# ttanida/rgrg

Measured on AMD Instinct MI355X. Metric: images/sec full 29-region report gen, 512x512 CXR, greedy max_len=128, higher is better.
Workload: dtype bf16; 1 GPU; full_model.generate() batch=32/GPU, 29 regions, greedy max_len=128, bf16 autocast: 16-bit detector, 16-bit decode GEMMs + K/V cache, hipGraph-captured decode step (BASELINE configs[2]); global_batch=32, parallelism=single GPU, weights=seeded random init (rgrg_amd.synth, profile bench), hipGraph_decode=True

## Files before the change

include/rgrg_hip.h:

```cpp
#ifndef RGRG_HIP_H_
#define RGRG_HIP_H_

#include <stdint.h>

#ifdef __cplusplus
extern "C" {
#endif

#define RGRG_OK 0
#define RGRG_EINVAL (-1)
#define RGRG_EHIP (-2)
#define RGRG_ESTATE (-3)

#define RGRG_ACT_NONE 0
#define RGRG_ACT_RELU 1
#define RGRG_ACT_GELU_NEW 2

const char* rgrg_last_error(void);
int rgrg_abi_version(void);
int rgrg_device_arch(int dev, char* buf, int buflen);

int rgrg_linear_f32(const float* A, const float* W, const float* scale, const float* shift, const float* R,
                    float* Y, int M, int N, int K, int ldy, int act, int splitk, float* ws, void* stream);
int rgrg_conv2d_nhwc_f32(const float* X, const float* W, const float* scale, const float* shift, const float* R,
                         float* Y, int B, int H, int Wd, int Cin, int Cout, int KH, int KW, int stride, int pad,
                         int act, int splitk, float* ws, void* stream);

int rgrg_stem_conv7x7_f32(const float* X, const float* Wt, const float* scale, const float* shift, float* Y,
                          int B, int H, int Wd, void* stream);
int rgrg_maxpool3x3s2_nhwc_f32(const float* X, float* Y, int B, int H, int Wd, int C, void* stream);

int rgrg_rpn_proposals_f32(const float* head_out, const float* anchors, float* proposals, int32_t* counts,
                           int32_t* offsets, int B, int HW, int A, int pre_nms, int post_nms, float nms_thresh,
                           float min_size, float img_w, float img_h, void* stream);

int rgrg_roi_align_avgpool_f32(const float* feat, const float* proposals, const int32_t* offsets, float* out,
                               float* pooled, int B, int FH, int FW, int C, int max_props, int R_total,
                               float spatial_scale, void* stream);
int rgrg_roi_align_avgpool_bf16maps(const float* feat, const float* proposals, const int32_t* offsets, uint16_t* out16,
                                    float* pooled, int B, int FH, int FW, int C, int max_props, int R_total,
                                    float spatial_scale, int fp16, void* stream);

int rgrg_top1_per_class_f32(const float* pred, int ldp, const float* proposals, const int32_t* offsets,
                            const float* pooled, uint8_t* class_detected, float* top_scores, float* top_boxes,
                            float* top_feats, int B, int C, int max_props, float img_w, float img_h, void* stream);

int rgrg_bce_with_logits_masked_f32(const float* logits, const uint8_t* mask, const uint8_t* target, float pos_weight,
                                    int n, float* loss, void* stream);
int rgrg_preprocess_u8_f32(const uint8_t* src, int h, int w, int src_stride, int new_h, int new_w, float mean, float std,
                           float* dst, void* stream);
int rgrg_select_regions_f32(const float* logits, const uint8_t* class_detected, float thr, uint8_t* selected,
                            int32_t* sel_rows, int32_t* n_selected, int n, void* stream);
int rgrg_gather_rows_f32(const float* src, const int32_t* rows, float* dst, int n_rows, int D, void* stream);

typedef struct rgrg_decoder_layer_weights {
    const float *ln1_g, *ln1_b, *ln2_g, *ln2_b;
    const float *c_attn_w, *c_attn_b;
    const float *attn_proj_w, *attn_proj_b;
    const float *c_fc_w, *c_fc_b;
    const float *mlp_proj_w, *mlp_proj_b;
} rgrg_decoder_layer_weights;

typedef struct rgrg_decoder_weights {
    int n_layer, d_model, n_head, vocab;
    const float* wte;
    const float *lnf_g, *lnf_b;
    const float *fst0_w, *fst0_b, *fst2_w, *fst2_b;
    const float *ukv_w, *ukv_b;
    const rgrg_decoder_layer_weights* layers;
} rgrg_decoder_weights;

typedef struct rgrg_decoder rgrg_decoder;

int rgrg_decoder_create(const rgrg_decoder_weights* w, int max_seqs, int max_len, rgrg_decoder** out);
int rgrg_decoder_create_with_cache(const rgrg_decoder_weights* w, int max_seqs, int max_len, void* kv_cache, size_t kv_cache_bytes,
                                   rgrg_decoder** out);
size_t rgrg_decoder_kv_cache_bytes(int n_layer, int max_seqs, int max_len);
void rgrg_decoder_destroy(rgrg_decoder* d);
int rgrg_decoder_generate(rgrg_decoder* d, const float* feats, int S, int max_length, int64_t* out_ids,
                          int out_ld, int* out_len, int use_graph, void* stream);
int rgrg_decoder_sample(rgrg_decoder* d, const float* feats, int S, int max_length, float temperature, int top_k, float top_p,
                        uint64_t seed, int64_t* out_ids, int out_ld, float* out_logprobs, int* out_len, int use_graph,
                        void* stream);
int rgrg_sample_logits_f32(const float* logits, int64_t ld, int S, int V, float temperature, int top_k, float top_p,
                           uint64_t seed, int step, int row0, int* out_tok, float* out_logprob, void* stream);
int rgrg_decoder_beam_search(rgrg_decoder* d, const float* feats, int S, int num_beams, int max_length,
                             int early_stopping, float length_penalty, int num_return_sequences, int64_t* out_ids,
                             int out_ld, int* out_len, void* stream);
int rgrg_decoder_set_precision(rgrg_decoder* d, int mode);
int rgrg_decoder_set_kv_format(rgrg_decoder* d, int fmt);
int rgrg_decoder_kv_format_in_use(rgrg_decoder* d, int rows);
int rgrg_decoder_set_lm_positions(rgrg_decoder* d, const int64_t* pos, int64_t n);
int rgrg_decoder_lm_forward(rgrg_decoder* d, const float* feats, const int64_t* input_ids, const float* attention_mask,
                            int S, int T, float* logits_out, float* loss_out, void* stream);
int rgrg_decoder_lm_loss_grad(rgrg_decoder* d, const float* feats, const int64_t* input_ids, const float* attention_mask,
                              int S, int T, float loss_scale, float dropout_p, uint64_t dropout_seed, float* loss_out,
                              float* grad_ukv_w, float* grad_ukv_b, float* grad_fst0_w, float* grad_fst0_b, float* grad_fst2_w,
                              float* grad_fst2_b, void* stream);
int rgrg_decoder_time_train_gemms(rgrg_decoder* d, int S, int T, int iters, float* ms_per_step, double* flops_per_step,
                                  int* launches_per_step);
int rgrg_dropout_mask_f32(uint64_t seed, uint32_t stream_id, float p, int64_t n, int row_len, float* out, void* stream);
int rgrg_decoder_forward_cached(rgrg_decoder* d, const float* feats, const int64_t* input_ids, const int64_t* position_ids,
                                const float* attention_mask,
                                int S, int T, int past_len, float* logits_out, void* stream);
int rgrg_decoder_cache_plane(rgrg_decoder* d, int layer, int kv, void** ptr, int* max_seqs, int* slots, int* is_bf16);
int rgrg_decoder_take_id_error(rgrg_decoder* d, int* pending);
int rgrg_decoder_refresh_trainable(rgrg_decoder* d, void* stream);
int rgrg_transpose_pad_f32(const float* src, float* dst, int rows, int cols, int rows_padded, void* stream);
int rgrg_colsum_f32(const float* src, float* out, int rows, int cols, void* stream);
int rgrg_relu_backward_f32(float* d, const float* h, int64_t n, void* stream);
int rgrg_bce_with_logits_masked_backward_f32(const float* logits, const uint8_t* mask, const uint8_t* target, float pos_weight,
                                             int n, float scale, float* dlogits, int ld, void* stream);
int rgrg_adamw_step_f32(float* param, const float* grad, float* exp_avg, float* exp_avg_sq, int64_t n, float lr, float beta1,
                        float beta2, float eps, float weight_decay, int step, float grad_scale, void* stream);
int rgrg_adamw_multi_step_f32(const void* items, int n_items, float lr, float beta1, float beta2, float eps,
                              float weight_decay, int step, float grad_scale, void* stream);
int rgrg_f32_to_bf16(const float* src, uint16_t* dst, int64_t n, int fp16, void* stream);
int rgrg_bf16_to_f32(const uint16_t* src, float* dst, int64_t n, int fp16, void* stream);
int rgrg_conv2d_nhwc_bf16(const uint16_t* X16, const uint16_t* Wb, const float* shift, const uint16_t* R16, float* Y,
                          uint16_t* Y16, int B, int H, int Wd, int Cin, int Cout, int KH, int KW, int stride, int pad,
                          int act, int fp16, void* stream);
int rgrg_linear_bf16w_f32(const float* A, const uint16_t* Wb, const float* shift, const float* R, float* Y, int M,
                          int N, int K, int ldy, int act, int fp16, void* stream);
int rgrg_linear_bf16_f32(const uint16_t* A16, const uint16_t* Wb, const float* shift, const float* R, float* Y,
                         uint16_t* Y16, int M, int N, int K, int ldy, int act, int fp16, void* stream);
int rgrg_debug_linear_bf16_tile(const uint16_t* A16, const uint16_t* Wb, const float* shift, const float* R, float* Y,
                                int M, int N, int K, int ldy, int act, int tile, int lda, int ldw, int fp16, void* stream);
int rgrg_debug_linear_bf16_train(const uint16_t* A16, const uint16_t* Wb, const float* shift, const float* R, float* Y,
                                 uint16_t* Y16, uint16_t* Ypre16, const uint16_t* G16, int M, int N, int K, int ldy, int act,
                                 int tile, int fp16, void* stream);
int rgrg_debug_linear_bf16_argmax(const uint16_t* A16, const uint16_t* Wb, const float* shift, int M, int N, int K,
                                  float* cand_val, int* cand_idx, int fp16, void* stream);
int rgrg_debug_ln_fold16(const float* w, const float* gain, const float* beta, const float* bias, uint16_t* wb, float* colsum,
                         float* shift, int N, int K, int fp16, void* stream);
int rgrg_debug_linear_bf16_ln(const uint16_t* A16, const uint16_t* Wb, const float* shift, const float* R, float* Y,
                              uint16_t* Yb16, float* stats_out, const float* ln_stats, const float* ln_colsum, int M, int N,
                              int K, int ldy, int act, int fp16, void* stream);
int rgrg_debug_linear_bf16_ln_kv(const uint16_t* A16, const uint16_t* Wb, const float* shift, float* Y, const float* ln_stats,
                                 const float* ln_colsum, uint16_t* kcache, uint16_t* vcache, const int* step_dev, int M, int H,
                                 int T_slots, int K, int ldy, int fp16, void* stream);
int rgrg_debug_linear_bf16_ln_kp(const uint16_t* A16, const uint16_t* Wb, const float* shift, const float* R, float* Y,
                                 uint16_t* Y16, uint16_t* Yb16, float* stats_out, const float* ln_stats, const float* ln_colsum,
                                 int M, int N, int K, int ldy, int act, int fp16, int kp, void* stream);
int rgrg_debug_attn_decode(const float* qkv, int ld_qkv, void* kcache, void* vcache, const int* step_dev, float* out,
                           uint16_t* out16, int S, int H, int T_slots, const int* src, const float* kmask, int kv16, int fp16,
                           int ni, int frag_out, int max_workgroups, void* stream);
int rgrg_debug_attn_decode_qonly(const float* q, int ld_q, const void* kcache, const void* vcache, const int* step_dev, float* out,
                                 uint16_t* out16, int S, int H, int T_slots, int fp16, int max_workgroups, void* stream);
int rgrg_debug_attn_decode_kv8(const float* qkv, int ld_qkv, uint8_t* kcache, uint8_t* vcache, const int* step_dev, float* out,
                               uint16_t* out16, int S, int H, int T_slots, const int* src, const float* kmask, int fp16,
                               int max_workgroups, void* stream);
int rgrg_debug_attn_prefill(const float* qkv, const float* ukv, int ld_ukv, int kcol, const float* am, float* out, uint16_t* out16,
                            float* lse, int S, int H, int T, int variant, uint64_t seed, uint32_t stream_id, float p, int fp16,
                            void* stream);
int rgrg_debug_attn_backward_f32(const float* qkv, const float* ukv, int ld_ukv, int kcol, const float* am, const float* d_att,
                                 const float* att, const float* lse, float* delta, float* d_qkv, float* d_ukv, uint16_t* d_qkv16,
                                 int S, int H, int T, uint64_t seed, uint32_t stream_id, float p, int fp16, float ukv_scale,
                                 void* stream);
int rgrg_debug_attn_train16(int backward, const uint16_t* qkv16, const uint16_t* ukv16, int ld_ukv, int kcol, const float* am,
                            uint16_t* att16, float* lse, const uint16_t* d_att16, uint16_t* d_qkv16, float* d_ukv, int S, int H,
                            int T, uint64_t seed, uint32_t stream_id, float p, float ukv_scale, int fp16, void* stream);
int rgrg_box_match_f32(const float* gt, const int* gt_count, int G, const float* boxes, int64_t box_image_stride,
                       const int* box_count, int B, int N, float high, float low, int allow_low_quality, int* matched,
                       int* ws_best_per_gt, void* stream);
int rgrg_balanced_sample(const int* matched, const int64_t* gt_labels, int G, const int* box_count, const float* keys,
                         uint64_t seed, int stage, int B, int n, int batch, int max_pos, uint32_t* ws_keys, uint8_t* mask,
                         int* list, int* count, void* stream);
int rgrg_rpn_loss_sampled_f32(const float* rpn_out, int ld, int anchors_per_cell, const int* matched, const float* gt, int G,
                              const float* anchors, const uint8_t* mask, const int* list, const int* count, int B, int A,
                              int batch, float* out2, void* stream);
int rgrg_roi_add_gt_f32(const float* props, const int* counts, int P, const float* gt, const int* gt_count, int G, int B,
                        float* boxes, int* box_count, void* stream);
int rgrg_roi_gather_samples_f32(const float* boxes, const int* matched, const float* gt, const int64_t* gt_labels,
                                const int* gt_count, int G, const int* list, const int* count, int B, int N, int K, float wx,
                                float wy, float ww, float wh, float* props_s, int* offsets, int64_t* labels_flat,
                                float* reg_targets, void* stream);
int rgrg_fastrcnn_loss_f32(const float* pred, int ld, int num_classes, const int64_t* labels, const float* reg_targets, int N,
                           float* out2, void* stream);

int rgrg_decoder_copy_last_logits(rgrg_decoder* d, float* dst, int S, void* stream);
int rgrg_decoder_time_step_parts(rgrg_decoder* d, int S, int nkeys, int iters, int one_range, float* ms_gemm, float* ms_attn,
                                 double* gemm_flops, double* gemm_weight_bytes, double* kv_bytes, int* gemm_launches);
int rgrg_decoder_trace_step(rgrg_decoder* d, int S, int nkeys, int iters, float* recs, int max_recs, int* n_out);
int rgrg_decoder_attention_only(rgrg_decoder* d, int S, int nkeys, int iters, void* stream);
int rgrg_decoder_row_limit(rgrg_decoder* d);
int rgrg_debug_chain(int n, int mode, int blocks, float* us_per_kernel);

#ifdef __cplusplus
}
#endif
#endif
```

rgrg_amd/_hip.py:

```python
from __future__ import annotations

import ctypes as C
import os
from typing import Optional

from . import build as _build

c_float_p = C.c_void_p
_i, _f, _p = C.c_int, C.c_float, C.c_void_p

ACT_NONE, ACT_RELU, ACT_GELU_NEW = 0, 1, 2
ABI_VERSION = 25


class RgrgHipError(RuntimeError):
    pass


class DecoderLayerWeights(C.Structure):
    _fields_ = [(n, _p) for n in ("ln1_g", "ln1_b", "ln2_g", "ln2_b", "c_attn_w", "c_attn_b", "attn_proj_w",
                                  "attn_proj_b", "c_fc_w", "c_fc_b", "mlp_proj_w", "mlp_proj_b")]


class DecoderWeights(C.Structure):
    _fields_ = [("n_layer", _i), ("d_model", _i), ("n_head", _i), ("vocab", _i), ("wte", _p), ("lnf_g", _p),
                ("lnf_b", _p), ("fst0_w", _p), ("fst0_b", _p), ("fst2_w", _p), ("fst2_b", _p), ("ukv_w", _p),
                ("ukv_b", _p), ("layers", C.POINTER(DecoderLayerWeights))]


SIGNATURES = {
    "rgrg_last_error": (C.c_char_p, []),
    "rgrg_abi_version": (_i, []),
    "rgrg_device_arch": (_i, [_i, C.c_char_p, _i]),
    "rgrg_linear_f32": (_i, [_p, _p, _p, _p, _p, _p, _i, _i, _i, _i, _i, _i, _p, _p]),
    "rgrg_conv2d_nhwc_f32": (_i, [_p, _p, _p, _p, _p, _p, _i, _i, _i, _i, _i, _i, _i, _i, _i, _i, _i, _p, _p]),
    "rgrg_stem_conv7x7_f32": (_i, [_p, _p, _p, _p, _p, _i, _i, _i, _p]),
    "rgrg_maxpool3x3s2_nhwc_f32": (_i, [_p, _p, _i, _i, _i, _i, _p]),
    "rgrg_rpn_proposals_f32": (_i, [_p, _p, _p, _p, _p, _i, _i, _i, _i, _i, _f, _f, _f, _f, _p]),
    "rgrg_roi_align_avgpool_f32": (_i, [_p, _p, _p, _p, _p, _i, _i, _i, _i, _i, _i, _f, _p]),
    "rgrg_roi_align_avgpool_bf16maps": (_i, [_p, _p, _p, _p, _p, _i, _i, _i, _i, _i, _i, _f, _i, _p]),
    "rgrg_top1_per_class_f32": (_i, [_p, _i, _p, _p, _p, _p, _p, _p, _p, _i, _i, _i, _f, _f, _p]),
    "rgrg_select_regions_f32": (_i, [_p, _p, _f, _p, _p, _p, _i, _p]),
    "rgrg_bce_with_logits_masked_f32": (_i, [_p, _p, _p, C.c_float, _i, _p, _p]),
    "rgrg_preprocess_u8_f32": (_i, [_p, _i, _i, _i, _i, _i, C.c_float, C.c_float, _p, _p]),
    "rgrg_gather_rows_f32": (_i, [_p, _p, _p, _i, _i, _p]),
    "rgrg_decoder_create": (_i, [C.POINTER(DecoderWeights), _i, _i, C.POINTER(_p)]),
    "rgrg_decoder_create_with_cache": (_i, [C.POINTER(DecoderWeights), _i, _i, _p, C.c_size_t, C.POINTER(_p)]),
    "rgrg_decoder_kv_cache_bytes": (C.c_size_t, [_i, _i, _i]),
    "rgrg_decoder_destroy": (None, [_p]),
    "rgrg_decoder_generate": (_i, [_p, _p, _i, _i, _p, _i, C.POINTER(_i), _i, _p]),
    "rgrg_decoder_sample": (_i, [_p, _p, _i, _i, _f, _i, _f, C.c_uint64, _p, _i, _p, C.POINTER(_i), _i, _p]),
    "rgrg_sample_logits_f32": (_i, [_p, C.c_int64, _i, _i, _f, _i, _f, C.c_uint64, _i, _i, _p, _p, _p]),
    "rgrg_decoder_beam_search": (_i, [_p, _p, _i, _i, _i, _i, _f, _i, _p, _i, C.POINTER(_i), _p]),
    "rgrg_decoder_set_precision": (_i, [_p, _i]),
    "rgrg_decoder_set_kv_format": (_i, [_p, _i]),
    "rgrg_decoder_kv_format_in_use": (_i, [_p, _i]),
    "rgrg_decoder_lm_forward": (_i, [_p, _p, _p, _p, _i, _i, _p, _p, _p]),
    "rgrg_decoder_lm_loss_grad": (_i, [_p, _p, _p, _p, _i, _i, C.c_float, C.c_float, C.c_uint64, _p, _p, _p, _p, _p, _p, _p, _p]),
    "rgrg_dropout_mask_f32": (_i, [C.c_uint64, C.c_uint32, C.c_float, C.c_int64, _i, _p, _p]),
    "rgrg_decoder_refresh_trainable": (_i, [_p, _p]),
    "rgrg_decoder_take_id_error": (_i, [_p, C.POINTER(_i)]),
    "rgrg_decoder_forward_cached": (_i, [_p, _p, _p, _p, _p, _i, _i, _i, _p, _p]),
    "rgrg_decoder_cache_plane": (_i, [_p, _i, _i, C.POINTER(C.c_void_p), C.POINTER(_i), C.POINTER(_i), C.POINTER(_i)]),
    "rgrg_transpose_pad_f32": (_i, [_p, _p, _i, _i, _i, _p]),
    "rgrg_colsum_f32": (_i, [_p, _p, _i, _i, _p]),
    "rgrg_relu_backward_f32": (_i, [_p, _p, C.c_int64, _p]),
    "rgrg_bce_with_logits_masked_backward_f32": (_i, [_p, _p, _p, C.c_float, _i, C.c_float, _p, _i, _p]),
    "rgrg_adamw_step_f32": (_i, [_p, _p, _p, _p, C.c_int64, C.c_float, C.c_float, C.c_float, C.c_float, C.c_float, _i, C.c_float, _p]),
    "rgrg_adamw_multi_step_f32": (_i, [_p, _i, C.c_float, C.c_float, C.c_float, C.c_float, C.c_float, _i, C.c_float, _p]),
    "rgrg_f32_to_bf16": (_i, [_p, _p, C.c_int64, _i, _p]),
    "rgrg_bf16_to_f32": (_i, [_p, _p, C.c_int64, _i, _p]),
    "rgrg_conv2d_nhwc_bf16": (_i, [_p, _p, _p, _p, _p, _p, _i, _i, _i, _i, _i, _i, _i, _i, _i, _i, _i, _p]),
    "rgrg_linear_bf16w_f32": (_i, [_p, _p, _p, _p, _p, _i, _i, _i, _i, _i, _i, _p]),
    "rgrg_linear_bf16_f32": (_i, [_p, _p, _p, _p, _p, _p, _i, _i, _i, _i, _i, _i, _p]),
    "rgrg_debug_linear_bf16_tile": (_i, [_p, _p, _p, _p, _p, _i, _i, _i, _i, _i, _i, _i, _i, _i, _p]),
    "rgrg_debug_linear_bf16_train": (_i, [_p, _p, _p, _p, _p, _p, _p, _p, _i, _i, _i, _i, _i, _i, _i, _p]),
    "rgrg_debug_linear_bf16_argmax": (_i, [_p, _p, _p, _i, _i, _i, _p, _p, _i, _p]),
    "rgrg_debug_ln_fold16": (_i, [_p, _p, _p, _p, _p, _p, _p, _i, _i, _i, _p]),
    "rgrg_debug_linear_bf16_ln": (_i, [_p, _p, _p, _p, _p, _p, _p, _p, _p, _i, _i, _i, _i, _i, _i, _p]),
    "rgrg_debug_linear_bf16_ln_kp": (_i, [_p, _p, _p, _p, _p, _p, _p, _p, _p, _p, _i, _i, _i, _i, _i, _i, _i, _p]),
    "rgrg_debug_attn_decode": (_i, [_p, _i, _p, _p, _p, _p, _p, _i, _i, _i, _p, _p, _i, _i, _i, _i, _i, _p]),
    "rgrg_debug_linear_bf16_ln_kv": (_i, [_p, _p, _p, _p, _p, _p, _p, _p, _p, _i, _i, _i, _i, _i, _i, _p]),
    "rgrg_debug_attn_decode_qonly": (_i, [_p, _i, _p, _p, _p, _p, _p, _i, _i, _i, _i, _i, _p]),
    "rgrg_debug_attn_decode_kv8": (_i, [_p, _i, _p, _p, _p, _p, _p, _i, _i, _i, _p, _p, _i, _i, _p]),
    "rgrg_debug_attn_prefill": (_i, [_p, _p, _i, _i, _p, _p, _p, _p, _i, _i, _i, _i, C.c_uint64, C.c_uint32, _f, _i, _p]),
    "rgrg_debug_attn_backward_f32": (_i, [_p, _p, _i, _i, _p, _p, _p, _p, _p, _p, _p, _p, _i, _i, _i, C.c_uint64, C.c_uint32, _f,
                                          _i, _f, _p]),
    "rgrg_debug_attn_train16": (_i, [_i, _p, _p, _i, _i, _p, _p, _p, _p, _p, _p, _i, _i, _i, C.c_uint64, C.c_uint32, _f, _f, _i, _p]),
    "rgrg_decoder_copy_last_logits": (_i, [_p, _p, _i, _p]),
    "rgrg_box_match_f32": (_i, [_p, _p, _i, _p, C.c_int64, _p, _i, _i, _f, _f, _i, _p, _p, _p]),
    "rgrg_balanced_sample": (_i, [_p, _p, _i, _p, _p, C.c_uint64, _i, _i, _i, _i, _i, _p, _p, _p, _p, _p]),
    "rgrg_rpn_loss_sampled_f32": (_i, [_p, _i, _i, _p, _p, _i, _p, _p, _p, _p, _i, _i, _i, _p, _p]),
    "rgrg_roi_add_gt_f32": (_i, [_p, _p, _i, _p, _p, _i, _i, _p, _p, _p]),
    "rgrg_roi_gather_samples_f32": (_i, [_p, _p, _p, _p, _p, _i, _p, _p, _i, _i, _i, _f, _f, _f, _f, _p, _p, _p, _p, _p]),
    "rgrg_fastrcnn_loss_f32": (_i, [_p, _i, _i, _p, _p, _i, _p, _p]),
    "rgrg_decoder_trace_step": (_i, [_p, _i, _i, _i, _p, _i, C.POINTER(_i)]),
    "rgrg_decoder_attention_only": (_i, [_p, _i, _i, _i, _p]),
    "rgrg_decoder_row_limit": (_i, [_p]),
    "rgrg_decoder_set_lm_positions": (_i, [_p, _p, C.c_int64]),
    "rgrg_decoder_time_step_parts": (_i, [_p, _i, _i, _i, _i, C.POINTER(_f), C.POINTER(_f), C.POINTER(C.c_double),
                                          C.POINTER(C.c_double), C.POINTER(C.c_double), C.POINTER(_i)]),
    "rgrg_decoder_time_train_gemms": (_i, [_p, _i, _i, _i, C.POINTER(_f), C.POINTER(C.c_double), C.POINTER(_i)]),
    "rgrg_debug_chain": (_i, [_i, _i, _i, C.POINTER(_f)]),
}

_lib: Optional[C.CDLL] = None


def library_path() -> str:
    return _build.LIB_PATH


def load() -> C.CDLL:
    global _lib
    if _lib is not None:
        return _lib
    path = library_path()
    if _build.is_stale():
        try:
            _build.build_library()
        except Exception as e:
            if not os.path.exists(path):
                raise RgrgHipError(f"librgrg_hip.so is missing and could not be built: {e}") from e
    try:
        lib = C.CDLL(path)
    except OSError as e:
        raise RgrgHipError(f"cannot load {path}: {e} (the RGRG HIP path has no CPU fallback)") from e
    for name, (res, args) in SIGNATURES.items():
        fn = getattr(lib, name)
        fn.restype = res
        fn.argtypes = args
    got = lib.rgrg_abi_version()
    if got != ABI_VERSION:
        raise RgrgHipError(f"{path} has ABI version {got}, this package expects {ABI_VERSION}: rebuild it "
                           "(python -m rgrg_amd.build)")
    _lib = lib
    return lib


def autocast_mode() -> int:
    import torch
    if not torch.is_autocast_enabled("cuda"):
        return 0
    dt = torch.get_autocast_dtype("cuda")
    return 1 if dt == torch.bfloat16 else (2 if dt == torch.float16 else 0)


def check(rc: int, what: str = "") -> None:
    if rc != 0:
        msg = load().rgrg_last_error()
        raise RgrgHipError(f"{what} failed (code {rc}): {msg.decode() if msg else '?'}")


def ptr(t) -> Optional[int]:
    if t is None:
        return None
    assert t.is_contiguous(), "rgrg_hip expects dense tensors"
    return t.data_ptr()
```

rgrg_amd/csrc/decoder.hip:

```cpp
#include <math.h>
#include <stdlib.h>

#include <algorithm>
#include <type_traits>
#include <cmath>
#include <vector>

#include "decoder_internal.h"

namespace rgrg {

int skinny_max_rows() {
    static int v = -1;
    if (v < 0) { const char* e = getenv("RGRG_SKINNY_MAX_ROWS"); v = e ? atoi(e) : SKINNY_MAX_ROWS;
        if (v > SKINNY_MAX_ROWS) v = SKINNY_MAX_ROWS; if (v < 32) v = 32; }
    return v;
}

__global__ __launch_bounds__(256) void pack_weights_kernel(const float* __restrict__ W, float* __restrict__ P, int N,
                                                           int K, int NT) {
    const size_t total = (size_t)NT * (K / 8) * 64;
    for (size_t o = (size_t)blockIdx.x * blockDim.x + threadIdx.x; o < total; o += (size_t)gridDim.x * blockDim.x) {
        const int l = (int)(o & 63);
        const size_t t = o >> 6;
// ... 77 lines not shown
#pragma unroll
            for (int j = 0; j < 4; ++j) c16 = __builtin_amdgcn_mfma_f32_32x32x2f32(x[j], w[c][j], c16, 0, 0, 0);
        }
#pragma unroll
        for (int r = 0; r < 16; ++r) acc[mt][r] = c16[r];
    }
    float* red = smem;
#pragma unroll
    for (int mt = 0; mt < MT; ++mt) {
        __syncthreads();
#pragma unroll
        for (int r = 0; r < 16; ++r) red[(wave * 16 + r) * 64 + lane] = acc[mt][r];
        __syncthreads();
        const int row0 = mt * 32;
#pragma unroll
        for (int q = 0; q < 2; ++q) {
            const int idx = tid + 512 * q;
            const int r = idx >> 6, l = idx & 63;
            float v = red[r * 64 + l];
#pragma unroll
            for (int w2 = 1; w2 < SK_WAVES; ++w2) v += red[(w2 * 16 + r) * 64 + l];
            const int lrow = (r & 3) + 8 * (r >> 2) + 4 * (l >> 5);
            const int col = nt * 32 + (l & 31);
            if (a.KS == 1) skinny_store(a, row0 + lrow, col, v);
            else a.part[(((size_t)mt * a.KS + ks) * PAD_ROWS + lrow) * (a.NT * 32) + col] = v;
        }
    }
}

__global__ __launch_bounds__(512) void rgrg_skinny_gemm_f32_wide(const SkinnyArgs a) {
    extern __shared__ __attribute__((aligned(16))) float smem[];
    constexpr int PW = 16, KC = 8, KWG = PW * SK_WAVES * KC, LDX = KWG + 4, XQ = KWG / 64;
    float* red = smem + a.M * LDX;
    const int tid = threadIdx.x, lane = tid & 63, wave = tid >> 6;
    const int chunks = a.K / KC;
    {
        f32x4 xr[XQ];
#pragma unroll
        for (int q = 0; q < XQ; ++q) {
            const int idx = tid + 512 * q;
            const int row = idx / (KWG / 4), c4 = idx - row * (KWG / 4);
            xr[q] = *reinterpret_cast<const f32x4*>(a.X + (size_t)row * a.K + c4 * 4);
        }
#pragma unroll
        for (int q = 0; q < XQ; ++q) {
            const int idx = tid + 512 * q;
            const int row = idx / (KWG / 4), c4 = idx - row * (KWG / 4);
            if (row < a.M) *reinterpret_cast<f32x4*>(&smem[row * LDX + c4 * 4]) = xr[q];
        }
    }
    __syncthreads();
    const float* xa = &smem[(lane & 31) * LDX + wave * PW * KC + (lane >> 5) * 4];
    const f32x4* wbase = reinterpret_cast<const f32x4*>(a.P) + ((size_t)wave * PW) * 64 + lane;
    f32x4 wa[8], wb[8];
    auto load8 = [&](f32x4(&w)[8], int nt, int half) {
        const f32x4* wp = wbase + ((size_t)nt * chunks + half * 8) * 64;
#pragma unroll
        for (int c = 0; c < 8; ++c) w[c] = __builtin_nontemporal_load(wp + (size_t)c * 64);
    };
    int nt = blockIdx.x;
    if (nt < a.NT) { load8(wa, nt, 0); load8(wb, nt, 1); }
    for (; nt < a.NT; nt += gridDim.x) {
        const int nxt = nt + gridDim.x;
        f32x16 acc;
#pragma unroll
        for (int r = 0; r < 16; ++r) acc[r] = 0.f;
#pragma unroll
        for (int c = 0; c < 8; ++c) {
            const f32x4 x = *reinterpret_cast<const f32x4*>(xa + c * KC);
#pragma unroll
            for (int j = 0; j < 4; ++j) acc = __builtin_amdgcn_mfma_f32_32x32x2f32(x[j], wa[c][j], acc, 0, 0, 0);
        }
        if (nxt < a.NT) load8(wa, nxt, 0);
#pragma unroll
        for (int c = 0; c < 8; ++c) {
            const f32x4 x = *reinterpret_cast<const f32x4*>(xa + (8 + c) * KC);
#pragma unroll
            for (int j = 0; j < 4; ++j) acc = __builtin_amdgcn_mfma_f32_32x32x2f32(x[j], wb[c][j], acc, 0, 0, 0);
        }
        if (nxt < a.NT) load8(wb, nxt, 1);
        __syncthreads();
#pragma unroll
        for (int r = 0; r < 16; ++r) red[(wave * 16 + r) * 64 + lane] = acc[r];
        __syncthreads();
#pragma unroll
        for (int q = 0; q < 2; ++q) {
            const int idx = tid + 512 * q;
            const int r = idx >> 6, l = idx & 63;
            float v = red[r * 64 + l];
#pragma unroll
            for (int w2 = 1; w2 < SK_WAVES; ++w2) v += red[(w2 * 16 + r) * 64 + l];
            const int row = (r & 3) + 8 * (r >> 2) + 4 * (l >> 5);
            const int col = nt * 32 + (l & 31);
            skinny_store(a, row, col, v);
        }
    }
}


#include "skinny_direct.inc"

constexpr int WIDE_MAX_ROWS = 31;
constexpr size_t WIDE_LDS = (size_t)(WIDE_MAX_ROWS * (16 * SK_WAVES * 8 + 4) + SK_WAVES * 16 * 64) * sizeof(float);
static_assert(WIDE_LDS <= 160 * 1024, "wide skinny GEMM must fit the 160 KiB LDS");

template <int PW, int MT>
static int launch_skinny(const SkinnyArgs& a, hipStream_t st) {
    constexpr size_t lds_x = (size_t)32 * (PW * SK_WAVES * 8 + 4) * sizeof(float);
    constexpr size_t lds_r = (size_t)SK_WAVES * 16 * 64 * sizeof(float);
    constexpr size_t lds = lds_x > lds_r ? lds_x : lds_r;
    hipLaunchKernelGGL((rgrg_skinny_gemm_f32<PW, MT>), dim3(a.NT, a.KS), dim3(64 * SK_WAVES), lds, st, a);
    RGRG_LAUNCH_CHECK();
    return RGRG_OK;
}

template <int PW>
static int launch_skinny_mt(const SkinnyArgs& a, hipStream_t st) {
    const int mt = (a.M + PAD_ROWS - 1) / PAD_ROWS;
    if (mt <= 1) return launch_skinny<PW, 1>(a, st);
    if (mt == 2) return launch_skinny<PW, 2>(a, st);
    if (mt == 3) return launch_skinny<PW, 3>(a, st);
    if (mt == 4) return launch_skinny<PW, 4>(a, st);
    set_error("skinny GEMM: %d rows exceed 4 row tiles", a.M);
    return RGRG_EINVAL;
}

static int launch_skinny_any(const SkinnyArgs& a, hipStream_t st) {
    const int pw = a.K / (8 * a.KS * SK_WAVES);
    if (pw == 16 && a.KS == 1 && a.NT > 512 && a.M <= WIDE_MAX_ROWS) {
        hipLaunchKernelGGL(rgrg_skinny_gemm_f32_wide, dim3(256), dim3(64 * SK_WAVES), WIDE_LDS, st, a);
        RGRG_LAUNCH_CHECK();
        return RGRG_OK;
    }
    if (pw == 4) return launch_skinny_mt<4>(a, st);
    if (pw == 8) return launch_skinny_mt<8>(a, st);
    if (pw == 16) return launch_skinny_mt<16>(a, st);
    set_error("skinny GEMM: unsupported shape K=%d KS=%d (chunks per wave %d)", a.K, a.KS, pw);
    return RGRG_EINVAL;
}

__global__ __launch_bounds__(256) void skinny_reduce_kernel(const SkinnyArgs a) {
    const int ldp = a.NT * 32;
    const int total = a.M * a.N;
    for (int i = blockIdx.x * blockDim.x + threadIdx.x; i < total; i += gridDim.x * blockDim.x) {
        const int row = i / a.N, col = i - row * a.N;
        float v = 0.f;
        const float* pt = a.part + ((size_t)(row >> 5) * a.KS * PAD_ROWS + (row & 31)) * ldp + col;
        for (int ks = 0; ks < a.KS; ++ks) v += pt[(size_t)ks * PAD_ROWS * ldp];
        skinny_store(a, row, col, v);
    }
}


__global__ __launch_bounds__(256) void embed_ln_kernel(const float* __restrict__ wte, const long long* __restrict__ ids,
                                                       int ld_ids, const int* __restrict__ step, const float* __restrict__ g,
                                                       const float* __restrict__ b, float* __restrict__ x,
                                                       float* __restrict__ xn, int D, const int* __restrict__ tok_override,
                                                       unsigned short* __restrict__ xn16, int f16, const int* __restrict__ pos_override,
                                                       float* __restrict__ stats) {
    __shared__ float sh[4];
    const int s = blockIdx.x, tid = threadIdx.x;
    const int t = pos_override ? pos_override[s] : *step;
    const long long tok = tok_override ? (long long)tok_override[s] : ids[(size_t)s * ld_ids + *step];
    const f32x4 v = reinterpret_cast<const f32x4*>(wte + (size_t)tok * D)[tid] + reinterpret_cast<const f32x4*>(wte + (size_t)t * D)[tid];
    reinterpret_cast<f32x4*>(x + (size_t)s * D)[tid] = v;
    if (stats) {
        store_16x4(xn16 + (size_t)s * D + 4 * tid, v, f16);
        const float s1 = block_sum_256((v[0] + v[1]) + (v[2] + v[3]), sh);
        const float s2 = block_sum_256((v[0] * v[0] + v[1] * v[1]) + (v[2] * v[2] + v[3] * v[3]), sh);
        if (tid < 16) reinterpret_cast<float2*>(stats)[(size_t)s * 16 + tid] = tid ? make_float2(0.f, 0.f) : make_float2(s1, s2);
        return;
    }
    const f32x4 o = ln_row(v, g, b, sh, D);
    if (xn16) store_16x4(xn16 + (size_t)s * D + 4 * tid, o, f16);
    else reinterpret_cast<f32x4*>(xn + (size_t)s * D)[tid] = o;
}

__global__ __launch_bounds__(256) void ln_rows_kernel(const float* __restrict__ x, const float* __restrict__ g,
                                                      const float* __restrict__ b, float* __restrict__ xn, int D,
                                                      unsigned short* __restrict__ xn16, int f16, int rows) {
    const int lane = threadIdx.x & 63, row = blockIdx.x * 4 + (threadIdx.x >> 6);
    if (row >= rows) return;
    const f32x4* xr = reinterpret_cast<const f32x4*>(x + (size_t)row * D);
    f32x4 v[4], gg[4], bb[4];
#pragma unroll
    for (int j = 0; j < 4; ++j) v[j] = xr[j * 64 + lane];
#pragma unroll
    for (int j = 0; j < 4; ++j) {
        gg[j] = reinterpret_cast<const f32x4*>(g)[j * 64 + lane];
        bb[j] = reinterpret_cast<const f32x4*>(b)[j * 64 + lane];
    }
    __builtin_amdgcn_sched_barrier(0);
    float s = 0.f;
#pragma unroll
    for (int j = 0; j < 4; ++j) s += (v[j][0] + v[j][1]) + (v[j][2] + v[j][3]);
    const float mean = wave_sum_dpp(s) / (float)D;
    float q = 0.f;
#pragma unroll
    for (int j = 0; j < 4; ++j) {
#pragma unroll
        for (int e = 0; e < 4; ++e) { v[j][e] -= mean; q += v[j][e] * v[j][e]; }
    }
    const float rstd = 1.0f / sqrtf(wave_sum_dpp(q) / (float)D + LN_EPS);
#pragma unroll
    for (int j = 0; j < 4; ++j) {
        f32x4 o;
#pragma unroll
        for (int e = 0; e < 4; ++e) o[e] = v[j][e] * rstd * gg[j][e] + bb[j][e];
        if (xn16) store_16x4(xn16 + (size_t)row * D + 4 * (j * 64 + lane), o, f16);
        else reinterpret_cast<f32x4*>(xn + (size_t)row * D)[j * 64 + lane] = o;
    }
}
int launch_ln_rows(const float* x, const float* g, const float* b, float* xn, int D, unsigned short* xn16, int f16, int rows,
                   hipStream_t st) {
    hipLaunchKernelGGL(ln_rows_kernel, dim3((rows + 3) / 4), dim3(256), 0, st, x, g, b, xn, D, xn16, f16, rows);
    RGRG_LAUNCH_CHECK();
    return RGRG_OK;
}


__device__ __forceinline__ float group16_sum_dpp(float v) {
    v += dpp_get<0xB1, 0xf>(v);
    v += dpp_get<0x4E, 0xf>(v);
    v += dpp_get<0x141, 0xf>(v);
    v += dpp_get<0x140, 0xf>(v);
    return v;
}

template <bool HAS_SRC, int NI, bool HAS_MASK = false>
__device__ __forceinline__ void attn_chunk(const float* __restrict__ kc, const float* __restrict__ vc, const int* __restrict__ srow, int s,
                                           int hd, int H, int T, int base, int nkeys, int slot, int wave, int g, int d4,
                                           const f32x4& q4, const f32x4& k4, const f32x4& v4, float& m, float& l, f32x4& acc,
                                           const float* __restrict__ kmask = nullptr) {
    int rowi[NI];
#pragma unroll
    for (int i = 0; i < NI; ++i) rowi[i] = HAS_SRC ? srow[min(base + (i * 4 + wave) * 4 + g, nkeys - 1)] : s;
    f32x4 kk[NI], vv[NI];
    float mk[NI];
#pragma unroll
    for (int i = 0; i < NI; ++i) {
        const int jc = min(base + (i * 4 + wave) * 4 + g, nkeys - 1);
        const size_t off = (((size_t)rowi[i] * H + hd) * T + jc) * 64 + d4 * 4;
        kk[i] = *reinterpret_cast<const f32x4*>(kc + off);
        vv[i] = *reinterpret_cast<const f32x4*>(vc + off);
        mk[i] = HAS_MASK ? kmask[(size_t)s * T + jc] : 0.f;
    }
    __builtin_amdgcn_sched_barrier(0);
    {
#pragma clang fp contract(off)
    float sc[NI];
#pragma unroll
    for (int i = 0; i < NI; ++i) {
        const int j = base + (i * 4 + wave) * 4 + g;
        if (j == slot) { kk[i] = k4; vv[i] = v4; }
        const float dot = group16_sum_dpp(fmaf(q4[0], kk[i][0], q4[1] * kk[i][1]) + fmaf(q4[2], kk[i][2], q4[3] * kk[i][3]));
        sc[i] = HAS_MASK ? dot / 8.0f + mk[i] : dot / 8.0f;
    }
    float ex[NI];
    bool up[NI];
    float mp = m;
#pragma unroll
    for (int i = 0; i < NI; ++i) {
        const bool valid = base + (i * 4 + wave) * 4 + g < nkeys;
        up[i] = valid && sc[i] > mp;
        ex[i] = valid ? expf(-fabsf(sc[i] - mp)) : 0.f;
        mp = up[i] ? sc[i] : mp;
    }
#pragma unroll
    for (int i = 0; i < NI; ++i) {
        const bool valid = base + (i * 4 + wave) * 4 + g < nkeys;
        const float scale = up[i] ? ex[i] : 1.f;
        const float p = up[i] ? 1.f : ex[i];
        l = fmaf(l, scale, p);
#pragma unroll
        for (int e = 0; e < 4; ++e) acc[e] = fmaf(p, valid ? vv[i][e] : 0.f, acc[e] * scale);
    }
    m = mp;
    }
}

template <bool HAS_SRC, int ATT_NI, bool HAS_MASK = false>
__global__ __launch_bounds__(256) void attn_decode_kernel(const float* __restrict__ qkv, int ld_qkv,
                                                          float* __restrict__ kc, float* __restrict__ vc,
                                                          const int* __restrict__ step, float* __restrict__ out,
                                                          int S, int H, int T, const int* __restrict__ src, int frag_out,
                                                          const float* __restrict__ kmask = nullptr) {
    __shared__ float pm[16], pl[16];
    __shared__ __attribute__((aligned(16))) float pacc[16][64];
    const int lane = threadIdx.x & 63, wave = threadIdx.x >> 6;
    const int s = blockIdx.x / H, hd = blockIdx.x - s * H;
    const int t = *step, nkeys = t + 2, slot = t + 1;
    const int g = lane >> 4, d4 = lane & 15;
    const float* row = qkv + (size_t)s * ld_qkv;
    const int D = H * 64;
    const int* srow = HAS_SRC ? src + (size_t)s * T : nullptr;
    constexpr int ATT_CHUNK = 16 * ATT_NI;
    const f32x4 q4 = *reinterpret_cast<const f32x4*>(row + hd * 64 + d4 * 4);
    const f32x4 k4 = *reinterpret_cast<const f32x4*>(row + D + hd * 64 + d4 * 4);
    const f32x4 v4 = *reinterpret_cast<const f32x4*>(row + 2 * D + hd * 64 + d4 * 4);
    float m = -INFINITY, l = 0.f;
    f32x4 acc = {0.f, 0.f, 0.f, 0.f};
#define ATT_CHUNK_CALL(NI_, BASE_) attn_chunk<HAS_SRC, NI_, HAS_MASK>(kc, vc, srow, s, hd, H, T, BASE_, nkeys, slot, wave, g, d4, q4, k4, v4, m, l, acc, kmask)
    if constexpr (ATT_NI == 9) {
        int base = 0;
        for (; nkeys - base > ATT_CHUNK; base += ATT_CHUNK) ATT_CHUNK_CALL(9, base);
        switch ((nkeys - base + 15) >> 4) {
            case 1: ATT_CHUNK_CALL(1, base); break;
            case 2: ATT_CHUNK_CALL(2, base); break;
            case 3: ATT_CHUNK_CALL(3, base); break;
            case 4: ATT_CHUNK_CALL(4, base); break;
            case 5: ATT_CHUNK_CALL(5, base); break;
            case 6: ATT_CHUNK_CALL(6, base); break;
            case 7: ATT_CHUNK_CALL(7, base); break;
            case 8: ATT_CHUNK_CALL(8, base); break;
            default: ATT_CHUNK_CALL(9, base); break;
        }
    } else {
        for (int base = 0; base < nkeys; base += ATT_CHUNK) ATT_CHUNK_CALL(ATT_NI, base);
    }
#undef ATT_CHUNK_CALL
    if (wave == 0 && g == 0) {
        *reinterpret_cast<f32x4*>(kc + (((size_t)s * H + hd) * T + slot) * 64 + d4 * 4) = k4;
        *reinterpret_cast<f32x4*>(vc + (((size_t)s * H + hd) * T + slot) * 64 + d4 * 4) = v4;
    }
    const int grp = wave * 4 + g;
    if (d4 == 0) { pm[grp] = m; pl[grp] = l; }
    *reinterpret_cast<f32x4*>(&pacc[grp][d4 * 4]) = acc;
    __syncthreads();
// ... 67 lines not shown
            vn16 = kv16_pack_round<F16>(r.v0, r.v1);
        }
    }
    float sc[NI];
    float cmax = -INFINITY;
#pragma unroll
    for (int i = 0; i < NI; ++i) {
        const int j = base + i * 8 + g;
        if constexpr (!QONLY) {
            if (j == slot) { kk[i] = kn16; vv[i] = vn16; }
        }
        float dot = 0.f;
#pragma unroll
        for (int e = 0; e < 4; ++e)
            dot += q[2 * e] * pair_lo<F16>(kk[i][e]) + q[2 * e + 1] * pair_hi<F16>(kk[i][e]);
        dot += dpp_get<0xB1, 0xf>(dot);
        dot += dpp_get<0x4E, 0xf>(dot);
        dot += dpp_get<0x141, 0xf>(dot);
        sc[i] = j < nkeys ? dot / 8.0f : -INFINITY;
        cmax = fmaxf(cmax, sc[i]);
    }
    const float m_new = fmaxf(m, cmax);
    const float scale = (m == -INFINITY) ? 0.f : expf(m - m_new);
    const bool any = m_new != -INFINITY;
    l *= scale;
#pragma unroll
    for (int e = 0; e < 8; ++e) acc[e] *= scale;
#pragma unroll
    for (int i = 0; i < NI; ++i) {
        const int j = base + i * 8 + g;
        const float pj = (j < nkeys && any) ? expf(sc[i] - m_new) : 0.f;
        l += pj;
#pragma unroll
        for (int e = 0; e < 4; ++e) {
            const unsigned u = j < nkeys ? vv[i][e] : 0u;
            acc[2 * e] += pj * pair_lo<F16>(u);
            acc[2 * e + 1] += pj * pair_hi<F16>(u);
        }
    }
    m = m_new;
}

template <bool HAS_SRC, bool F16, bool QONLY = false>
__global__ __launch_bounds__(256) void attn_decode_kv16_wave_kernel(const float* __restrict__ qkv, int ld_qkv,
                                                                    u16* __restrict__ kc, u16* __restrict__ vc,
                                                                    const int* __restrict__ step, float* __restrict__ out,
                                                                    int S, int H, int T, const int* __restrict__ src,
                                                                    u16* __restrict__ out16) {
    const int lane = threadIdx.x & 63;
    const int t = *step, nkeys = t + 2, slot = t + 1;
    const int g = lane >> 3, d8 = lane & 7;
    const int D = H * 64;
    const __amdgpu_buffer_rsrc_t rk = dx_rsrc(kc), rv = dx_rsrc(vc);
    for (int item = blockIdx.x * 4 + (threadIdx.x >> 6); item < S * H; item += gridDim.x * 4) {
    const int s = item / H, hd = item - s * H;
    const float* row = qkv + (size_t)s * ld_qkv;
    const int* srow = HAS_SRC ? src + (size_t)s * T : nullptr;
    Kv16Row r;
    r.q0 = *reinterpret_cast<const f32x4*>(row + hd * 64 + d8 * 8);
    r.q1 = *reinterpret_cast<const f32x4*>(row + hd * 64 + d8 * 8 + 4);
    if constexpr (!QONLY) {
        r.k0 = *reinterpret_cast<const f32x4*>(row + D + hd * 64 + d8 * 8);
        r.k1 = *reinterpret_cast<const f32x4*>(row + D + hd * 64 + d8 * 8 + 4);
        r.v0 = *reinterpret_cast<const f32x4*>(row + 2 * D + hd * 64 + d8 * 8);
        r.v1 = *reinterpret_cast<const f32x4*>(row + 2 * D + hd * 64 + d8 * 8 + 4);
    }
    float m = -INFINITY, l = 0.f, acc[8], q[8];
    u32x4 kn16, vn16;
#pragma unroll
    for (int e = 0; e < 8; ++e) acc[e] = 0.f;
#define KV16_CHUNK(NI_, FIRST_, BASE_) \
    kv16_wave_chunk<NI_, HAS_SRC, FIRST_, F16, QONLY>(rk, rv, srow, s, hd, H, T, BASE_, nkeys, slot, g, d8, r, q, kn16, vn16, m, l, acc)
#define KV16_TAIL(FIRST_, BASE_, REM_)                                                                   \
    switch (((REM_) + 7) >> 3) {                                                                         \
        case 1: KV16_CHUNK(1, FIRST_, BASE_); break;                                                     \
        case 2: KV16_CHUNK(2, FIRST_, BASE_); break;                                                     \
        case 3: KV16_CHUNK(3, FIRST_, BASE_); break;                                                     \
        case 4: KV16_CHUNK(4, FIRST_, BASE_); break;                                                     \
        case 5: KV16_CHUNK(5, FIRST_, BASE_); break;                                                     \
        case 6: KV16_CHUNK(6, FIRST_, BASE_); break;                                                     \
        case 7: KV16_CHUNK(7, FIRST_, BASE_); break;                                                     \
        case 8: KV16_CHUNK(8, FIRST_, BASE_); break;                                                     \
        default: KV16_CHUNK(9, FIRST_, BASE_); break;                                                    \
    }
    if (nkeys > 72) {
        KV16_CHUNK(9, true, 0);
        int base = 72;
        for (; nkeys - base > 72; base += 72) KV16_CHUNK(9, false, base);
        KV16_TAIL(false, base, nkeys - base)
    } else {
        KV16_TAIL(true, 0, nkeys)
    }
#undef KV16_TAIL
#undef KV16_CHUNK
    if constexpr (!QONLY) {
        if (g == 0) {
            const size_t o = (((size_t)s * H + hd) * T + slot) * 64 + d8 * 8;
            *reinterpret_cast<u32x4*>(kc + o) = kn16;
            *reinterpret_cast<u32x4*>(vc + o) = vn16;
        }
    }
    float M = fmaxf(m, dpp_get<0x128, 0xf>(m));
    M = fmaxf(M, __shfl_xor(M, 16, 64));
    M = fmaxf(M, __shfl_xor(M, 32, 64));
    const float wgt = (m == -INFINITY) ? 0.f : expf(m - M);
    l *= wgt;
    l += dpp_get<0x128, 0xf>(l);
    l += __shfl_xor(l, 16, 64);
    l += __shfl_xor(l, 32, 64);
#pragma unroll
    for (int e = 0; e < 8; ++e) {
        float o = acc[e] * wgt;
        o += dpp_get<0x128, 0xf>(o);
        o += __shfl_xor(o, 16, 64);
        o += __shfl_xor(o, 32, 64);
        acc[e] = o / l;
    }
    if (g == 0) {
        const size_t o = (size_t)s * D + hd * 64 + d8 * 8;
        if (out16) {
            u32x4 pk;
#pragma unroll
            for (int i = 0; i < 4; ++i) pk[i] = to16<F16>(acc[2 * i]) | (to16<F16>(acc[2 * i + 1]) << 16);
            *reinterpret_cast<u32x4*>(out16 + o) = pk;
        } else {
            *reinterpret_cast<f32x4*>(out + o) = f32x4{acc[0], acc[1], acc[2], acc[3]};
            *reinterpret_cast<f32x4*>(out + o + 4) = f32x4{acc[4], acc[5], acc[6], acc[7]};
        }
    }
    }
}

template <typename KV>
__global__ __launch_bounds__(256) void kv_slot0_kernel(const float* __restrict__ ukv, int ld, KV* __restrict__ kv_all,
                                                       size_t layer_stride, size_t kv_stride, int S, int H, int T,
                                                       int L, int row_mul, int f16) {
    const int D = H * 64;
    const size_t total = (size_t)L * 2 * S * D;
    for (size_t i = (size_t)blockIdx.x * blockDim.x + threadIdx.x; i < total; i += (size_t)gridDim.x * blockDim.x) {
        const int d = (int)(i % D);
        size_t r = i / D;
        const int s = (int)(r % S);
        r /= S;
        const int kv = (int)(r & 1), l = (int)(r >> 1);
        const int hd = d >> 6, e = d & 63;
        const float val = ukv[(size_t)s * ld + ((size_t)l * 2 + kv) * D + d];
        const size_t o = (size_t)l * layer_stride + (size_t)kv * kv_stride + (((size_t)s * row_mul * H + hd) * T) * 64 + e;
        if constexpr (sizeof(KV) == 1) kv_all[o] = (KV)f32_to_e4m3_bits(val);
        else if constexpr (sizeof(KV) == 2) kv_all[o] = (KV)to16_rt(val, f16);
        else kv_all[o] = val;
    }
}

constexpr int ARGMAX_U = 13;
__global__ __launch_bounds__(256) void argmax_update_kernel(const float* __restrict__ cand_val, const int* __restrict__ cand_idx,
                                                            int NT, long long* __restrict__ ids, int ld_ids,
                                                            int* __restrict__ finished, int* __restrict__ step,
                                                            int* __restrict__ done_len, int* __restrict__ sync, int S) {
    __shared__ float bv[4];
    __shared__ int bi[4];
    const int row = blockIdx.x, tid = threadIdx.x, lane = tid & 63, wave = tid >> 6;
    const int t = *step;
    const float* cv = cand_val + (size_t)row * NT;
    const int* cx = cand_idx + (size_t)row * NT;
    float v[ARGMAX_U];
    int ci[ARGMAX_U];
#pragma unroll
    for (int u = 0; u < ARGMAX_U; ++u) {
        const int i = min(tid + 256 * u, NT - 1);
        v[u] = cv[i];
        ci[u] = cx[i];
    }
    float best = -INFINITY;
    int idx = 0x7fffffff;
#pragma unroll
    for (int u = 0; u < ARGMAX_U; ++u)
        if (tid + 256 * u < NT && (v[u] > best || (v[u] == best && ci[u] < idx))) { best = v[u]; idx = ci[u]; }
    for (int i = tid + 256 * ARGMAX_U; i < NT; i += 256) {
        const float w = cv[i];
        const int wi = cx[i];
        if (w > best || (w == best && wi < idx)) { best = w; idx = wi; }
    }
    for (int o = 32; o > 0; o >>= 1) {
        const float ov = __shfl_xor(best, o, 64);
        const int oi = __shfl_xor(idx, o, 64);
        if (ov > best || (ov == best && oi < idx)) { best = ov; idx = oi; }
    }
    if (lane == 0) { bv[wave] = best; bi[wave] = idx; }
    __syncthreads();
    if (tid == 0) {
        for (int w = 1; w < 4; ++w)
            if (bv[w] > best || (bv[w] == best && bi[w] < idx)) { best = bv[w]; idx = bi[w]; }
        const StepBook bk{ids, ld_ids, finished, step, done_len, sync, S};
        record_step_token(bk, row, t, idx == 0x7fffffff ? 0 : idx);
    }
}

__global__ __launch_bounds__(256) void logits_candidates_kernel(const float* __restrict__ logits, int ld, int V, int NT,
                                                                float* __restrict__ cand_val, int* __restrict__ cand_idx) {
    const int row = blockIdx.y, lane = threadIdx.x & 63, wave = threadIdx.x >> 6;
    const float* x = logits + (size_t)row * ld;
    const int sub = lane & 7, tw = lane >> 3;
    constexpr int UN = 4;
    for (int t0 = (blockIdx.x * 4 + wave) * 8 * UN; t0 < NT; t0 += gridDim.x * 4 * 8 * UN) {
        f32x4 v[UN];
#pragma unroll
        for (int u = 0; u < UN; ++u) {
            const int nt = min(t0 + u * 8 + tw, NT - 1);
            v[u] = *reinterpret_cast<const f32x4*>(x + nt * 32 + sub * 4);
        }
#pragma unroll
        for (int u = 0; u < UN; ++u) {
            const int nt = t0 + u * 8 + tw;
            const int c0 = min(nt, NT - 1) * 32 + sub * 4;
            float bv = -INFINITY;
            int bi = c0;
#pragma unroll
            for (int e = 0; e < 4; ++e) {
                const float val = (c0 + e < V) ? v[u][e] : -INFINITY;
                if (val > bv) { bv = val; bi = c0 + e; }
            }
#define CAND_STEP(CTRL)                                                                                     \
    {                                                                                                       \
        const float ov = dpp_get<CTRL, 0xf>(bv);                                                            \
        const int oi = __builtin_amdgcn_update_dpp(0, bi, CTRL, 0xf, 0xf, false);                           \
        if (ov > bv || (ov == bv && oi < bi)) { bv = ov; bi = oi; }                                         \
    }
            CAND_STEP(0xB1) CAND_STEP(0x4E) CAND_STEP(0x141)
#undef CAND_STEP
            if (sub == 0 && nt < NT) {
                cand_val[(size_t)row * NT + nt] = bv;
                cand_idx[(size_t)row * NT + nt] = bi;
            }
        }
    }
}

__global__ __launch_bounds__(256) void decode_reset_kernel(long long* __restrict__ ids, int ld_ids, int* __restrict__ finished,
                                                           int* __restrict__ step, int* __restrict__ done_len,
                                                           int* __restrict__ sync, int S, int L) {
    const size_t total = (size_t)S * L;
    for (size_t i = (size_t)blockIdx.x * blockDim.x + threadIdx.x; i < total; i += (size_t)gridDim.x * blockDim.x)
        ids[(i / L) * ld_ids + (i % L)] = (i % L) == 0 ? BOS_ID : PAD_ID;
    if (blockIdx.x == 0) {
        for (int s = threadIdx.x; s < S; s += 256) finished[s] = 0;
        if (threadIdx.x == 0) { *step = 0; *done_len = 0; }
        if (threadIdx.x < 2) sync[threadIdx.x] = 0;
    }
}

__global__ __launch_bounds__(256) void ln_fold16_kernel(const float* __restrict__ w, const float* __restrict__ gain,
                                                        const float* __restrict__ beta, const float* __restrict__ b,
                                                        unsigned short* __restrict__ wb, float* __restrict__ cs,
                                                        float* __restrict__ c2, int N, int K, int f16) {
    const int lane = threadIdx.x & 63, n = blockIdx.x * 4 + (threadIdx.x >> 6);
    if (n >= N) return;
    float a = 0.f, c = 0.f;
    for (int k = lane; k < K; k += 64) {
        const float wv = w[(size_t)n * K + k];
        float gw = gain[k] * wv;
        asm("" : "+v"(gw));
        const unsigned short r = (unsigned short)to16_rt(gw, f16);
        wb[(size_t)n * K + k] = r;
        a += from16_rt(r, f16);
        c += beta[k] * wv;
    }
    a = wave_sum(a);
    c = wave_sum(c);
    if (lane == 0) { cs[n] = a; c2[n] = (b ? b[n] : 0.f) + c; }
}

int dmalloc(rgrg_decoder* d, void** p, size_t bytes, bool zero) {
    RGRG_HIP(hipMalloc(p, bytes));
    d->allocs.push_back(*p);
    if (zero) RGRG_HIP(hipMemset(*p, 0, bytes));
    return RGRG_OK;
}

static int pick_ks(int NT, int chunks) {
    int ks = 1;
    if (NT >= 64) return ks;
    while (NT * ks < 256 && chunks % (ks * 2 * SK_WAVES * 4) == 0) ks *= 2;
    return ks;
}

static int make_lin(rgrg_decoder* d, Lin& l, const float* w, const float* b, int N, int K, bool pack,
                    bool direct = false, const float* ln_g = nullptr, const float* ln_b = nullptr) {
    l.w = w; l.b = b; l.N = N; l.K = K;
    if (direct) {
        if (!(K == DK_SLICE || (K == 4 * DK_SLICE && !ln_g && N == DK_SLICE))) { set_error("decoder: N=%d K=%d unsupported by the fused plan", N, K); return RGRG_EINVAL; }
        l.direct = true; l.ntile = 16; l.KS = K / DK_SLICE; l.NT = (N + 15) / 16; l.lnf = ln_g != nullptr;
        int rc = dmalloc(d, (void**)&l.packed, (size_t)l.NT * 16 * K * sizeof(float), false);
        if (rc) return rc;
        hipLaunchKernelGGL(pack_weights16_scaled_kernel, dim3(2048), dim3(256), 0, d->stream, w, ln_g, l.packed, N, K, l.NT);
        RGRG_LAUNCH_CHECK();
        if (l.lnf) {
            if ((rc = dmalloc(d, (void**)&l.c1, (size_t)N * sizeof(float), false)) ||
                (rc = dmalloc(d, (void**)&l.c2, (size_t)N * sizeof(float), false)))
                return rc;
            hipLaunchKernelGGL(ln_fold_vectors_kernel, dim3((N + 3) / 4), dim3(256), 0, d->stream, w, ln_g, ln_b, b, l.c1, l.c2, N, K);
            RGRG_LAUNCH_CHECK();
        }
        return RGRG_OK;
    }
    l.ntile = 32;
    l.KS = pick_ks((N + 31) / 32, K / 8);
    l.NT = (N + l.ntile - 1) / l.ntile;
    const int kc = 8;
    const int pw = K / (kc * l.KS * SK_WAVES);
    const bool ok = (K % (kc * l.KS * SK_WAVES) == 0) && (pw == 4 || pw == 8 || pw == 16);
    if (!ok) {
        set_error("decoder: no skinny GEMM instance for N=%d K=%d (ntile %d, KS %d, %d chunks per wave)", N, K, l.ntile, l.KS, pw);
        return RGRG_EINVAL;
    }
    if (pack) {
        const size_t bytes = (size_t)l.NT * l.ntile * K * sizeof(float);
        int rc = dmalloc(d, (void**)&l.packed, bytes, false);
        if (rc) return rc;
        hipLaunchKernelGGL(pack_weights_kernel, dim3(2048), dim3(256), 0, d->stream, w, l.packed, N, K, l.NT);
        RGRG_LAUNCH_CHECK();
    }
    return RGRG_OK;
}

template <int PW, int MT>
static int skinny_attr1() {
    constexpr size_t lds_x = (size_t)32 * (PW * SK_WAVES * 8 + 4) * sizeof(float);
    RGRG_HIP(hipFuncSetAttribute(reinterpret_cast<const void*>(&rgrg_skinny_gemm_f32<PW, MT>),
                                 hipFuncAttributeMaxDynamicSharedMemorySize, (int)(lds_x > 65536 ? lds_x : 65536)));
    return RGRG_OK;
}
template <int PW>
static int skinny_attr() {
    int rc;
    if ((rc = skinny_attr1<PW, 1>())) return rc;
    if ((rc = skinny_attr1<PW, 2>())) return rc;
    if ((rc = skinny_attr1<PW, 3>())) return rc;
    return skinny_attr1<PW, 4>();
}
static int init_skinny_attrs() {
    int rc;
    RGRG_HIP(hipFuncSetAttribute(reinterpret_cast<const void*>(&rgrg_lm_head_wave_f32<DX_COMBINE4>),
                                 hipFuncAttributeMaxDynamicSharedMemorySize, (int)LMH_LDS));
    if ((rc = skinny_attr<4>())) return rc;
    if ((rc = skinny_attr<8>())) return rc;
    RGRG_HIP(hipFuncSetAttribute(reinterpret_cast<const void*>(&rgrg_skinny_gemm_f32_wide),
                                 hipFuncAttributeMaxDynamicSharedMemorySize, (int)WIDE_LDS));
    return skinny_attr<16>();
// ... 113 lines not shown
        const dim3 wgrid(a.max_wgs > 0 ? std::min(wgs, a.max_wgs) : wgs), wblk(256);
        if (a.q_only && (a.fmt == KV_E4M3 || a.src)) {
            set_error("decode attention: the q-only variant exists for the 16-bit K/V cache without an ancestor table (%s)",
                      a.src ? "beam search" : "e4m3 K/V cache");
            return RGRG_EINVAL;
        }
        if (a.fmt == KV_E4M3)
            return launch_attn_decode_kv8(a.qkv, a.ld_qkv, static_cast<uint8_t*>(a.kc), static_cast<uint8_t*>(a.vc), a.step, a.out, a.out16,
                                          a.S, a.H, a.T, a.src, a.f16, (int)wgrid.x, a.st);
#define KV16_LAUNCH(...) hipLaunchKernelGGL((attn_decode_kv16_wave_kernel<__VA_ARGS__>), wgrid, wblk, 0, a.st, a.qkv, a.ld_qkv, \
                                                  static_cast<u16*>(a.kc), static_cast<u16*>(a.vc), a.step, a.out, a.S, a.H, a.T, a.src, a.out16)
        if (a.q_only) { if (a.f16) KV16_LAUNCH(false, true, true); else KV16_LAUNCH(false, false, true); }
        else if (a.src) { if (a.f16) KV16_LAUNCH(true, true); else KV16_LAUNCH(true, false); }
        else { if (a.f16) KV16_LAUNCH(false, true); else KV16_LAUNCH(false, false); }
#undef KV16_LAUNCH
    } else {
        if (a.q_only) { set_error("decode attention: the q-only variant exists for the 16-bit K/V cache only"); return RGRG_EINVAL; }
        const dim3 grid(a.S * a.H), blk(256);
        const int ni = a.ni ? a.ni : (a.S * a.H <= 4096 ? 9 : 2);
        if (ni != 9 && ni != 2) { set_error("decode attention: %d keys per group, the kernel is built for 9 and 2", ni); return RGRG_EINVAL; }
#define ATT_LAUNCH(SRC_, NI_, MASK_) hipLaunchKernelGGL((attn_decode_kernel<SRC_, NI_, MASK_>), grid, blk, 0, a.st, a.qkv, a.ld_qkv, static_cast<float*>(a.kc), \
                                                       static_cast<float*>(a.vc), a.step, a.out, a.S, a.H, a.T, a.src, a.frag_out, a.kmask)
        if (a.kmask) {
            if (ni == 9) ATT_LAUNCH(false, 9, true); else ATT_LAUNCH(false, 2, true);
        } else if (ni == 9) { if (a.src) ATT_LAUNCH(true, 9, false); else ATT_LAUNCH(false, 9, false); }
        else { if (a.src) ATT_LAUNCH(true, 2, false); else ATT_LAUNCH(false, 2, false); }
#undef ATT_LAUNCH
    }
    RGRG_LAUNCH_CHECK();
    return RGRG_OK;
}

static int launch_attention(rgrg_decoder* d, int l, int S, const int* src, unsigned short* att16, int frag_out = 0, int r0 = 0,
                            bool q_only = false) {
    const int D = d->D;
    AttnDecodeLaunch a{};
    a.q_only = q_only;
    a.ld_qkv = 3 * D; a.step = d->step; a.S = S; a.H = d->H; a.T = d->T; a.src = src; a.kmask = d->key_mask_cur;
    a.frag_out = frag_out; a.st = d->stream; a.plane_elems = d->kv_kv_stride;
    a.fmt = kv_format(d, S);
    if (a.fmt != KV_F32) {
        static const int cap = [] { const char* e = getenv("RGRG_ATTN_WGS_PER_CU"); return e ? atoi(e) : 0; }();
        const size_t esz = a.fmt == KV_E4M3 ? 1 : sizeof(u16);
        unsigned char* kcr = reinterpret_cast<unsigned char*>(d->kv) + ((size_t)l * d->kv_layer_stride + (size_t)r0 * d->H * d->T * 64) * esz;
        a.f16 = d->f16(); a.max_wgs = cap > 0 ? cap * 256 : 0;
        a.qkv = d->qkv + (size_t)r0 * 3 * D; a.kc = kcr; a.vc = kcr + d->kv_kv_stride * esz;
        a.out = d->att + (size_t)r0 * D; a.out16 = att16;
    } else {
        float* kc = d->kv + (size_t)l * d->kv_layer_stride;
        a.qkv = d->qkv; a.kc = kc; a.vc = kc + d->kv_kv_stride; a.out = d->att;
    }
    return launch_attn_decode(a);
}

static int direct_linear(rgrg_decoder* d, const Lin& l, DirectArgs a, int mode, int M, bool count, bool cand = false) {
    if (!l.direct) { set_error("direct_linear: layer was not packed for the fused plan"); return RGRG_EINVAL; }
    if (l.lnf && mode == DX_PLAIN && !a.Xf) { set_error("direct_linear: missing operand"); return RGRG_EINVAL; }
    a.P = l.packed; a.bias = l.lnf ? l.c2 : l.b; a.c1 = l.c1;
    a.M = M; a.K = l.K; a.N = l.N; a.NT = l.NT; a.KS = l.KS;
    if (l.KS > 1) a.part_out = d->part;
    if (cand) { a.cand_val = d->cand_val; a.cand_idx = d->cand_idx; }
    const int mt = (M + PAD_ROWS - 1) / PAD_ROWS;
    const int w16 = (d->bf16_gemms && d->w16_fused && mt > 1 && l.packed16 && l.packed16_f16 == d->f16() && (!l.lnf || l.c1_16)) ? (d->f16() ? 2 : 1) : 0;
    if (w16) { a.P = reinterpret_cast<const float*>(l.packed16); if (l.lnf) a.c1 = l.c1_16; }
    const dim3 grid(l.NT, l.KS), blk(64 * SK_WAVES);
    hipStream_t st = d->stream;
    if (l.lnf && mode == DX_COMBINE4 && l.NT > 512 && mt == 1 && l.K == DK_SLICE) {
        hipLaunchKernelGGL((rgrg_lm_head_wave_f32<DX_COMBINE4>), dim3(256), blk, LMH_LDS, st, a);
    } else if (!l.lnf && mode == DX_PLAIN && l.KS == 1 && mt == 1 && l.NT <= 64 && M > 16 && !cand) {
        hipLaunchKernelGGL(rgrg_skinny_direct_half_f32, dim3(l.NT, 2), blk, 0, st, a);
    } else {
#define DX_LAUNCH(MT_, MODE_, LNF_)                                                                                          \
    do {                                                                                                                      \
        if constexpr (MT_ > 1) {                                                                                              \
            if (w16 == 1) { hipLaunchKernelGGL((rgrg_skinny_direct_f32<MT_, MODE_, LNF_, 1>), grid, blk, 0, st, a); break; }  \
            if (w16 == 2) { hipLaunchKernelGGL((rgrg_skinny_direct_f32<MT_, MODE_, LNF_, 2>), grid, blk, 0, st, a); break; }  \
        }                                                                                                                     \
        hipLaunchKernelGGL((rgrg_skinny_direct_f32<MT_, MODE_, LNF_>), grid, blk, 0, st, a);                                  \
    } while (0)
#define DX_MODES(MT_)                                                                        \
    do {                                                                                     \
        if (!l.lnf && mode == DX_PLAIN) DX_LAUNCH(MT_, DX_PLAIN, false);                     \
        else if (l.lnf && mode == DX_PLAIN) DX_LAUNCH(MT_, DX_PLAIN, true);                  \
        else if (l.lnf && mode == DX_COMBINE4) DX_LAUNCH(MT_, DX_COMBINE4, true);            \
        else if (l.lnf && mode == DX_EMBED) DX_LAUNCH(MT_, DX_EMBED, true);                  \
        else if (l.lnf && mode == DX_EMBED_TOK) DX_LAUNCH(MT_, DX_EMBED_TOK, true);          \
        else if (l.lnf && mode == DX_EMBED_TOKPOS) DX_LAUNCH(MT_, DX_EMBED_TOKPOS, true);    \
        else { set_error("direct_linear: unsupported mode %d (lnf %d)", mode, (int)l.lnf); return RGRG_EINVAL; } \
    } while (0)
        if (mt == 1) DX_MODES(1);
        else if (mt == 2) DX_MODES(2);
        else if (mt == 3) DX_MODES(3);
        else if (mt == 4) DX_MODES(4);
        else { set_error("direct_linear: %d rows exceed 4 row tiles", M); return RGRG_EINVAL; }
#undef DX_MODES
#undef DX_LAUNCH
    }
    RGRG_LAUNCH_CHECK();
    if (count) {
        d->gemm_bytes_per_step += (size_t)l.N * l.K * (w16 ? 2 : sizeof(float));
        d->gemm_flops_per_step += 2.0 * M * l.N * l.K;
        d->gemm_launches_per_step += 1;
    }
    return RGRG_OK;
}

static int enqueue_layer_gemms(rgrg_decoder* d, int l, int S, bool count, const int* tok_override, const float* cur, float* nxt,
                               int part) {
    const LayerW& w = d->layers[l];
    const int D = d->D;
    int rc;
    if (part == 0) {
        DirectArgs a{};
        a.xout = nxt; a.Y = d->qkv; a.ldy = 3 * D; a.act = RGRG_ACT_NONE;
        int mode;
        if (l == 0) {
            a.wte = d->wte; a.ids = d->ids; a.ld_ids = d->max_len; a.step = d->step; a.tok_override = tok_override;
            a.pos_override = d->pos_override_cur;
            mode = tok_override ? (d->pos_override_cur ? DX_EMBED_TOKPOS : DX_EMBED_TOK) : DX_EMBED;
        } else {
            a.Xf = cur; a.part = d->part;
            mode = DX_COMBINE4;
        }
        return direct_linear(d, w.c_attn, a, mode, S, count);
    }
    DirectArgs p{};
    p.Xf = d->att; p.Rf = nxt; p.Yf = nxt; p.act = RGRG_ACT_NONE;
    p.zero_acc = d->part;
    if ((rc = direct_linear(d, w.attn_proj, p, DX_PLAIN, S, count))) return rc;
    DirectArgs f{};
    f.Xf = nxt; f.Yf = d->ff; f.act = RGRG_ACT_GELU_NEW;
    if ((rc = direct_linear(d, w.c_fc, f, DX_PLAIN, S, count))) return rc;
    DirectArgs m{};
    m.Xf = d->ff; m.act = RGRG_ACT_NONE;
    return direct_linear(d, w.mlp_proj, m, DX_PLAIN, S, count);
}

static int enqueue_step_fused(rgrg_decoder* d, int S, bool count, const int* tok_override, const int* src, bool beam) {
    if (count) { d->gemm_bytes_per_step = 0; d->gemm_flops_per_step = 0.0; d->gemm_launches_per_step = 0; }
    hipStream_t st = d->stream;
    int rc;
    float* cur = d->x;
    float* nxt = d->x2;
    for (int l = 0; l < d->n_layer; ++l) {
        if ((rc = enqueue_layer_gemms(d, l, S, count, tok_override, cur, nxt, 0))) return rc;
        if ((rc = launch_attention(d, l, S, src, nullptr, 1))) return rc;
        if ((rc = enqueue_layer_gemms(d, l, S, count, tok_override, cur, nxt, 1))) return rc;
        float* tmp = cur; cur = nxt; nxt = tmp;
    }
    DirectArgs h{};
    h.Xf = cur; h.part = d->part; h.Y = d->logits; h.ldy = d->ld_logits; h.act = RGRG_ACT_NONE;
    if ((rc = direct_linear(d, d->lm_head, h, DX_COMBINE4, S, count, !beam))) return rc;
    if (beam) return RGRG_OK;
    hipLaunchKernelGGL(argmax_update_kernel, dim3(S), dim3(256), 0, st, d->cand_val, d->cand_idx, d->lm_head.NT, d->ids,
                       d->max_len, d->finished, d->step, d->done_len, d->sync, S);
    RGRG_LAUNCH_CHECK();
    return RGRG_OK;
}

static int range_bounds(int S, int want, int (&bounds)[MAX_CHAINS + 1]) {
    int nr = want < 1 ? 1 : (want > MAX_CHAINS ? MAX_CHAINS : want);
    const int tiles = (S + 63) / 64;
    for (; nr > 1; --nr) {
        int least = S;
        for (int i = 0; i <= nr; ++i) {
            bounds[i] = std::min(S, ((tiles * i + nr - 1) / nr) * 64);
            if (i) least = std::min(least, bounds[i] - bounds[i - 1]);
        }
        if (least > SKINNY_MAX_ROWS) break;
    }
    if (nr <= 1) { nr = 1; bounds[0] = 0; bounds[1] = S; }
    return nr;
}
template <class F>
static int run_row_ranges(rgrg_decoder* d, int S, int chains, F&& fn) {
    int bounds[MAX_CHAINS + 1];
    const int nr = range_bounds(S, chains < 0 ? -chains : chains, bounds);
    if (nr <= 1) return fn(0, S);
    if (chains > 0) {
        RGRG_HIP(hipEventRecord(d->ev_fork, d->stream));
        for (int i = 1; i < nr; ++i) RGRG_HIP(hipStreamWaitEvent(d->streams_x[i - 1], d->ev_fork, 0));
    }
    int rc = RGRG_OK;
    for (int i = 0; i < nr && !rc; ++i) {
        if (bounds[i + 1] <= bounds[i]) continue;
        if (chains > 0 && i > 0) std::swap(d->stream, d->streams_x[i - 1]);
        rc = fn(bounds[i], bounds[i + 1] - bounds[i]);
        if (chains > 0 && i > 0) std::swap(d->stream, d->streams_x[i - 1]);
    }
    if (chains > 0)
        for (int i = 1; i < nr; ++i) {
            RGRG_HIP(hipEventRecord(d->ev_join[i - 1], d->streams_x[i - 1]));
            RGRG_HIP(hipStreamWaitEvent(d->stream, d->ev_join[i - 1], 0));
        }
    return rc;
}
static int step_chains(const rgrg_decoder* d, int S, bool greedy, bool fold) {
    return (greedy && fold && S >= 512 && (d->chains < 0 || d->streams_x[0])) ? d->chains : 1;
}

static int trace_mark(rgrg_decoder* d, int r0, int tag) {
    if (!d->trace) return RGRG_OK;
    hipEvent_t e;
    RGRG_HIP(hipEventCreate(&e));
    RGRG_HIP(hipEventRecord(e, d->stream));
    d->trace->push_back({e, r0, tag});
    return RGRG_OK;
}

static bool step_ln_fold(const rgrg_decoder* d, int S) {
    return kv_is_bf16(d, S) && d->xn16 && d->ln_fold && d->ln_stat && d->layers[0].c_attn.wb_ln && d->D == 1024;
}
static bool step_qkv_cache(const rgrg_decoder* d, int S, bool plain) {
    const KvFormat f = kv_format(d, S);
    return d->qkv_cache && plain && step_ln_fold(d, S) && (f == KV_BF16 || f == KV_F16) && d->kp_gemms != 1 && d->kp_gemms != 3 && !d->key_mask_cur;
}
static GemmLnFold cons_kv_cache(const rgrg_decoder* d, const GemmLnFold& cons, int l, int r0) {
    GemmLnFold f = cons;
    u16* kcr = reinterpret_cast<u16*>(d->kv) + (size_t)l * d->kv_layer_stride + (size_t)r0 * d->H * d->T * 64;
    f.kv_k = kcr; f.kv_v = kcr + d->kv_kv_stride; f.kv_step = d->step; f.kv_H = d->H; f.kv_T = d->T;
    return f;
}

int enqueue_step(rgrg_decoder* d, int S, bool count, const int* tok_override, const int* src, bool beam) {
    if (S <= decode_row_limit(d)) return enqueue_step_fused(d, S, count, tok_override, src, beam);
    if (count) { d->gemm_bytes_per_step = 0; d->gemm_flops_per_step = 0.0; d->gemm_launches_per_step = 0; }
    d->step_rows = S;
    hipStream_t st = d->stream;
    const int D = d->D;
    int rc;
    unsigned short* xn16 = (kv_is_bf16(d, S) && d->xn16) ? d->xn16 : nullptr;
    unsigned short* att16 = xn16 ? d->att16 : nullptr;
    unsigned short* ff16 = xn16 ? d->ff16 : nullptr;
    const bool fold = step_ln_fold(d, S);
    const bool qc = step_qkv_cache(d, S, !tok_override && !src);
    static const float cons_tag = 0.f;
    GemmLnFold prod{}, cons{};
    prod.Yb16 = xn16; prod.stats_out = d->ln_stat;
    cons.ln_stats = d->ln_stat; cons.ln_colsum = &cons_tag;
    const GemmLnFold* pf = fold ? &prod : nullptr;
    const GemmLnFold* cf = fold ? &cons : nullptr;
    auto run_rows = [&](int r0, int rows) -> int {
        hipStream_t rs = d->stream;
        const size_t o = (size_t)r0 * D;
        float* x = d->x + o; float* xn = d->xn + o;
        unsigned short* xn16r = xn16 ? xn16 + o : nullptr;
        unsigned short* att16r = att16 ? att16 + o : nullptr;
        unsigned short* ff16r = ff16 ? ff16 + 4 * o : nullptr;
        float* statr = d->ln_stat ? d->ln_stat + (size_t)r0 * 32 : nullptr;
        GemmLnFold prod_r = prod, cons_r = cons;
        prod_r.Yb16 = xn16r; prod_r.stats_out = statr; cons_r.ln_stats = statr;
        const GemmLnFold* pfr = fold ? &prod_r : nullptr;
        const GemmLnFold* cfr = fold ? &cons_r : nullptr;
        hipLaunchKernelGGL(embed_ln_kernel, dim3(rows), dim3(256), 0, rs, d->wte, d->ids + (size_t)r0 * d->max_len, d->max_len, d->step,
                           d->layers[0].ln1_g, d->layers[0].ln1_b, x, xn, D, tok_override ? tok_override + r0 : nullptr, xn16r, d->f16(),
                           d->pos_override_cur ? d->pos_override_cur + r0 : nullptr, fold ? statr : (float*)nullptr);
        RGRG_LAUNCH_CHECK();
        int rc2;
        if ((rc2 = trace_mark(d, r0, 1000))) return rc2;
        for (int l = 0; l < d->n_layer; ++l) {
            const LayerW& w = d->layers[l];
            const float* ng = (l + 1 < d->n_layer) ? d->layers[l + 1].ln1_g : d->lnf_g;
            const float* nb = (l + 1 < d->n_layer) ? d->layers[l + 1].ln1_b : d->lnf_b;
            const GemmLnFold cons_kv = qc ? cons_kv_cache(d, cons_r, l, r0) : cons_r;
            if ((rc2 = linear(d, w.c_attn, xn, nullptr, d->qkv + 3 * o, rows, 3 * D, RGRG_ACT_NONE, count, xn16r, nullptr, qc ? &cons_kv : cfr))) return rc2;
            if ((rc2 = trace_mark(d, r0, l * 8 + 0))) return rc2;
            if ((rc2 = launch_attention(d, l, rows, src ? src + (size_t)r0 * d->T : nullptr, att16r, 0, r0, qc))) return rc2;
            if ((rc2 = trace_mark(d, r0, l * 8 + 1))) return rc2;
            if ((rc2 = linear(d, w.attn_proj, d->att + o, x, x, rows, D, RGRG_ACT_NONE, count, att16r, nullptr, pfr))) return rc2;
            if ((rc2 = trace_mark(d, r0, l * 8 + 2))) return rc2;
            if (!fold) {
                if ((rc2 = launch_ln_rows(x, w.ln2_g, w.ln2_b, xn, D, xn16r, d->f16(), rows, rs))) return rc2;
            }
            if ((rc2 = linear(d, w.c_fc, xn, nullptr, d->ff + 4 * o, rows, 4 * D, RGRG_ACT_GELU_NEW, count, xn16r, ff16r, cfr))) return rc2;
            if ((rc2 = trace_mark(d, r0, l * 8 + 3))) return rc2;
            if ((rc2 = linear(d, w.mlp_proj, d->ff + 4 * o, x, x, rows, D, RGRG_ACT_NONE, count, ff16r, nullptr, pfr))) return rc2;
            if ((rc2 = trace_mark(d, r0, l * 8 + 4))) return rc2;
            if (!fold || l + 1 == d->n_layer) {
                if ((rc2 = launch_ln_rows(x, ng, nb, xn, D, xn16r, d->f16(), rows, rs))) return rc2;
                if ((rc2 = trace_mark(d, r0, 1001))) return rc2;
            }
        }
        return RGRG_OK;
    };
    if ((rc = run_row_ranges(d, S, step_chains(d, S, !beam && !tok_override && !src, fold), run_rows))) return rc;
    if (!beam && xn16 && lm_head_cand_path(d, S)) {
        GemmLnFold ce{};
        ce.cand_val = d->cand_val; ce.cand_idx = d->cand_idx;
        if ((rc = linear(d, d->lm_head, d->xn, nullptr, nullptr, S, d->ld_logits, RGRG_ACT_NONE, count, xn16, nullptr, &ce))) return rc;
        if ((rc = trace_mark(d, 0, 1002))) return rc;
        hipLaunchKernelGGL(argmax_update_kernel, dim3(S), dim3(256), 0, st, d->cand_val, d->cand_idx, (d->lm_head.N + 255) / 256, d->ids,
                           d->max_len, d->finished, d->step, d->done_len, d->sync, S);
        RGRG_LAUNCH_CHECK();
        return trace_mark(d, 0, 1003);
    }
    if ((rc = linear(d, d->lm_head, d->xn, nullptr, d->logits, S, d->ld_logits, RGRG_ACT_NONE, count, xn16))) return rc;
    if (beam) return RGRG_OK;
    const int cand_nt = (d->V + 31) / 32;
    hipLaunchKernelGGL(logits_candidates_kernel, dim3(4, S), dim3(256), 0, st, d->logits, d->ld_logits, d->V,
                       cand_nt, d->cand_val, d->cand_idx);
    RGRG_LAUNCH_CHECK();
    hipLaunchKernelGGL(argmax_update_kernel, dim3(S), dim3(256), 0, st, d->cand_val, d->cand_idx, cand_nt, d->ids,
                       d->max_len, d->finished, d->step, d->done_len, d->sync, S);
    RGRG_LAUNCH_CHECK();
    return RGRG_OK;
}

int enqueue_prefill(rgrg_decoder* d, const float* feats, int S, int row_mul) {
    hipStream_t st = d->stream;
    const int D = d->D;
    hipLaunchKernelGGL(decode_reset_kernel, dim3(64), dim3(256), 0, st, d->ids, d->max_len, d->finished, d->step,
                       d->done_len, d->sync, S, d->max_len);
    RGRG_LAUNCH_CHECK();
    RGRG_HIP(hipMemcpyAsync(d->feats, feats, (size_t)S * D * sizeof(float), hipMemcpyDeviceToDevice, st));
    int rc;
    if ((rc = linear(d, d->fst0, d->feats, nullptr, d->h1, S, D, RGRG_ACT_RELU, false))) return rc;
    if ((rc = linear(d, d->fst2, d->h1, nullptr, d->img, S, D, RGRG_ACT_NONE, false))) return rc;
    if ((rc = linear(d, d->ukv, d->img, nullptr, d->ukv_out, S, d->ld_ukv, RGRG_ACT_NONE, false))) return rc;
    const KvFormat fmt = kv_format(d, S * row_mul);
    if (fmt == KV_E4M3)
        hipLaunchKernelGGL(kv_slot0_kernel<uint8_t>, dim3(1024), dim3(256), 0, st, d->ukv_out, d->ld_ukv,
                           reinterpret_cast<uint8_t*>(d->kv), d->kv_layer_stride, d->kv_kv_stride, S, d->H, d->T, d->n_layer, row_mul, 0);
    else if (fmt != KV_F32)
        hipLaunchKernelGGL(kv_slot0_kernel<u16>, dim3(1024), dim3(256), 0, st, d->ukv_out, d->ld_ukv,
                           reinterpret_cast<u16*>(d->kv), d->kv_layer_stride, d->kv_kv_stride, S, d->H, d->T, d->n_layer, row_mul, d->f16());
    else
        hipLaunchKernelGGL(kv_slot0_kernel<float>, dim3(1024), dim3(256), 0, st, d->ukv_out, d->ld_ukv, d->kv,
                           d->kv_layer_stride, d->kv_kv_stride, S, d->H, d->T, d->n_layer, row_mul, 0);
    RGRG_LAUNCH_CHECK();
    return RGRG_OK;
}

}

using namespace rgrg;

extern "C" size_t rgrg_decoder_kv_cache_bytes(int n_layer, int max_seqs, int max_len) {
    return (size_t)n_layer * 2 * (size_t)max_seqs * 16 * (size_t)(max_len + 1) * 64 * sizeof(float);
}

extern "C" int rgrg_decoder_create(const rgrg_decoder_weights* w, int max_seqs, int max_len, rgrg_decoder** out) {
    return rgrg_decoder_create_with_cache(w, max_seqs, max_len, nullptr, 0, out);
}

extern "C" int rgrg_decoder_create_with_cache(const rgrg_decoder_weights* w, int max_seqs, int max_len, void* kv_cache, size_t kv_cache_bytes,
                                              rgrg_decoder** out) {
    RGRG_CHECK_ARG(w && out && max_seqs > 0 && max_seqs < 65536 && max_len >= 2 && max_len <= 1024);
    RGRG_CHECK_ARG(w->d_model == 1024 && w->n_head == 16 && w->n_layer > 0 && w->vocab > 0 && w->layers);
    int rc = init_gemm_attrs();
    if (rc) return rc;
    if ((rc = init_skinny_attrs())) return rc;
    RGRG_HIP(hipDeviceSynchronize());
    rgrg_decoder* d = new rgrg_decoder();
    d->n_layer = w->n_layer; d->D = w->d_model; d->H = w->n_head; d->V = w->vocab;
    d->max_seqs = max_seqs; d->max_len = max_len; d->T = max_len + 1;
    d->rows = ((max_seqs + PAD_ROWS - 1) / PAD_ROWS) * PAD_ROWS;
    d->wte = w->wte; d->lnf_g = w->lnf_g; d->lnf_b = w->lnf_b;
    const int D = d->D;
#define TRY(x) do { rc = (x); if (rc) { rgrg_decoder_destroy(d); return rc; } } while (0)
    if (hipStreamCreateWithFlags(&d->stream, hipStreamNonBlocking) != hipSuccess ||
        hipEventCreateWithFlags(&d->ev_in, hipEventDisableTiming) != hipSuccess) {
        set_error("decoder: stream/event creation failed");
        delete d;
        return RGRG_EHIP;
    }
    if (const char* e = getenv("RGRG_GEMM_KP")) d->kp_gemms = atoi(e);
    if (const char* e = getenv("RGRG_W16_FUSED")) d->w16_fused = atoi(e) != 0;
    if (const char* e = getenv("RGRG_QKV_CACHE")) d->qkv_cache = atoi(e) != 0;
    if (const char* e = getenv("RGRG_DECODE_CHAINS")) {
        const int v = atoi(e);
        d->chains = (v >= -MAX_CHAINS && v <= MAX_CHAINS && v != 0 && v != -1) ? v : 1;
    }
    if (d->chains > 1) {
        bool ok = hipEventCreateWithFlags(&d->ev_fork, hipEventDisableTiming) == hipSuccess;
        for (int i = 0; ok && i < d->chains - 1; ++i)
            ok = hipStreamCreateWithFlags(&d->streams_x[i], hipStreamNonBlocking) == hipSuccess &&
                 hipEventCreateWithFlags(&d->ev_join[i], hipEventDisableTiming) == hipSuccess;
        if (!ok) {
            set_error("decoder: stream/event creation failed");
            rgrg_decoder_destroy(d);
            return RGRG_EHIP;
        }
    }
    if (hipHostMalloc((void**)&d->h_id_error, sizeof(int), 0) == hipSuccess) *d->h_id_error = 0;
    if (hipHostMalloc((void**)&d->h_done, 3 * sizeof(int), 0) != hipSuccess ||
        hipEventCreateWithFlags(&d->ev_poll[0], hipEventDisableTiming) != hipSuccess ||
        hipEventCreateWithFlags(&d->ev_poll[1], hipEventDisableTiming) != hipSuccess) {
        set_error("decoder: hipHostMalloc failed");
        delete d;
        return RGRG_EHIP;
    }
    TRY(make_lin(d, d->fst0, w->fst0_w, w->fst0_b, D, D, true));
    TRY(make_lin(d, d->fst2, w->fst2_w, w->fst2_b, D, D, true));
    TRY(make_lin(d, d->ukv, w->ukv_w, w->ukv_b, w->n_layer * 2 * D, D, true));
    TRY(make_lin(d, d->lm_head, w->wte, nullptr, w->vocab, D, true, true, w->lnf_g, w->lnf_b));
    d->layers.resize(w->n_layer);
    for (int l = 0; l < w->n_layer; ++l) {
        const rgrg_decoder_layer_weights& s = w->layers[l];
        LayerW& t = d->layers[l];
        t.ln1_g = s.ln1_g; t.ln1_b = s.ln1_b; t.ln2_g = s.ln2_g; t.ln2_b = s.ln2_b;
        TRY(make_lin(d, t.c_attn, s.c_attn_w, s.c_attn_b, 3 * D, D, true, true, s.ln1_g, s.ln1_b));
        TRY(make_lin(d, t.attn_proj, s.attn_proj_w, s.attn_proj_b, D, D, true, true));
        TRY(make_lin(d, t.c_fc, s.c_fc_w, s.c_fc_b, 4 * D, D, true, true, s.ln2_g, s.ln2_b));
        TRY(make_lin(d, t.mlp_proj, s.mlp_proj_w, s.mlp_proj_b, D, 4 * D, true, true));
    }
    const size_t R = d->rows;
    d->ld_logits = d->lm_head.NT * d->lm_head.ntile;
    d->ld_ukv = d->ukv.N;
    TRY(dmalloc(d, (void**)&d->feats, R * D * 4, true));
    TRY(dmalloc(d, (void**)&d->h1, R * D * 4, true));
    TRY(dmalloc(d, (void**)&d->img, R * D * 4, true));
    TRY(dmalloc(d, (void**)&d->ukv_out, R * d->ld_ukv * 4, true));
    TRY(dmalloc(d, (void**)&d->x, R * D * 4, true));
    TRY(dmalloc(d, (void**)&d->x2, R * D * 4, true));
    TRY(dmalloc(d, (void**)&d->xn, R * D * 4, true));
    TRY(dmalloc(d, (void**)&d->qkv, R * 3 * D * 4, true));
    TRY(dmalloc(d, (void**)&d->att, R * D * 4, true));
    TRY(dmalloc(d, (void**)&d->ff, R * 4 * D * 4, true));
    TRY(dmalloc(d, (void**)&d->logits, R * d->ld_logits * 4, true));
    TRY(dmalloc(d, (void**)&d->part, (size_t)(SKINNY_MAX_ROWS / PAD_ROWS) * 8 * PAD_ROWS * D * 4, true));
    d->kv_kv_stride = (size_t)d->max_seqs * d->H * d->T * 64;
    d->kv_layer_stride = 2 * d->kv_kv_stride;
    if (kv_cache) {
        if (kv_cache_bytes < (size_t)d->n_layer * d->kv_layer_stride * 4) {
            set_error("decoder: the caller's K/V cache holds %zu bytes, %zu needed", kv_cache_bytes, (size_t)d->n_layer * d->kv_layer_stride * 4);
            rgrg_decoder_destroy(d);
            return RGRG_EINVAL;
        }
        d->kv = static_cast<float*>(kv_cache);
    } else {
        TRY(dmalloc(d, (void**)&d->kv, (size_t)d->n_layer * d->kv_layer_stride * 4, true));
    }
    TRY(dmalloc(d, (void**)&d->ids, R * max_len * sizeof(long long), true));
    TRY(dmalloc(d, (void**)&d->next, R * 4, true));
    TRY(dmalloc(d, (void**)&d->finished, R * 4, true));
    TRY(dmalloc(d, (void**)&d->step, 4, true));
    TRY(dmalloc(d, (void**)&d->done_len, 4, true));
    TRY(dmalloc(d, (void**)&d->sync, 64, true));
    TRY(dmalloc(d, (void**)&d->id_error, 8, true));
    TRY(dmalloc(d, (void**)&d->cand_val, R * d->lm_head.NT * 4, true));
    TRY(dmalloc(d, (void**)&d->cand_idx, R * d->lm_head.NT * 4, true));
    TRY(dmalloc(d, (void**)&d->src_a, R * d->T * 4, true));
    TRY(dmalloc(d, (void**)&d->src_b, R * d->T * 4, true));
    TRY(dmalloc(d, (void**)&d->beam_tok, R * 4, true));
    TRY(dmalloc(d, (void**)&d->row_pos, R * 4, true));
    TRY(dmalloc(d, (void**)&d->beam_parent, R * 4, true));
    TRY(dmalloc(d, (void**)&d->beam_scores, R * 4, true));
    TRY(dmalloc(d, (void**)&d->row_max, R * 4, true));
    TRY(dmalloc(d, (void**)&d->row_logsum, R * 4, true));
    TRY(dmalloc(d, (void**)&d->top_val, R * BEAM_K * 4, true));
    TRY(dmalloc(d, (void**)&d->top_tok, R * BEAM_K * 4, true));
    TRY(dmalloc(d, (void**)&d->cand_score, R * BEAM_K * 4, true));
    TRY(dmalloc(d, (void**)&d->cand_tok, R * BEAM_K * 4, true));
    TRY(dmalloc(d, (void**)&d->cand_beam, R * BEAM_K * 4, true));
    d->gemm_ws_floats = (d->max_seqs > 32) ? (size_t)16 * R * 4 * D : 0;
    d->gemm_ws = nullptr;
    if (d->gemm_ws_floats) TRY(dmalloc(d, (void**)&d->gemm_ws, d->gemm_ws_floats * 4, false));
#undef TRY
    if (hipDeviceSynchronize() != hipSuccess) {
        set_error("decoder: weight packing failed");
        rgrg_decoder_destroy(d);
        return RGRG_EHIP;
    }
    *out = d;
    return RGRG_OK;
}

extern "C" void rgrg_decoder_destroy(rgrg_decoder* d) {
    if (!d) return;
    for (auto& g : d->graphs) (void)hipGraphExecDestroy(g.exec);
    for (void* p : d->allocs) (void)hipFree(p);
    d->tf.free();
    d->tr.free();
    if (d->tr.a16_scratch) (void)hipFree(d->tr.a16_scratch);
    if (d->h_done) (void)hipHostFree(d->h_done);
    for (hipEvent_t e : d->ev_poll)
        if (e) (void)hipEventDestroy(e);
    if (d->h_id_error) (void)hipHostFree(d->h_id_error);
    if (d->ev_in) (void)hipEventDestroy(d->ev_in);
    if (d->ev_fork) (void)hipEventDestroy(d->ev_fork);
    for (int i = 0; i < MAX_CHAINS - 1; ++i) {
        if (d->ev_join[i]) (void)hipEventDestroy(d->ev_join[i]);
        if (d->streams_x[i]) (void)hipStreamDestroy(d->streams_x[i]);
    }
    if (d->stream) (void)hipStreamDestroy(d->stream);
    delete d;
}

namespace rgrg {
int decode_begin(rgrg_decoder* d, void* stream) {
    RGRG_HIP(hipEventRecord(d->ev_in, as_stream(stream)));
    RGRG_HIP(hipStreamWaitEvent(d->stream, d->ev_in, 0));
    d->logits_valid = false;
    return RGRG_OK;
}
int run_decode_loop(rgrg_decoder* d, const float* feats, int S, int limit, int graph_key, int (*step)(rgrg_decoder*, int, bool),
                    int use_graph, int64_t* out_ids, int out_ld, float* out_logprobs, int* out_len) {
    int rc = enqueue_prefill(d, feats, S);
    if (rc) return rc;

    hipGraphExec_t exec = nullptr;
    if (use_graph) {
        for (auto& g : d->graphs)
            if (g.S == S && g.key2 == graph_key) exec = g.exec;
        if (!exec) {
            hipGraph_t graph = nullptr;
            RGRG_HIP(hipStreamBeginCapture(d->stream, hipStreamCaptureModeThreadLocal));
            rc = step(d, S, true);
            hipError_t e = hipStreamEndCapture(d->stream, &graph);
            if (rc) return rc;
            if (e != hipSuccess) { set_error("hipStreamEndCapture: %s", hipGetErrorString(e)); return RGRG_EHIP; }
            RGRG_HIP(hipGraphInstantiate(&exec, graph, nullptr, nullptr, 0));
            (void)hipGraphDestroy(graph);
            d->graphs.push_back({S, exec, graph_key, 0});
        }
    }
    const int steps = limit - 1;
    int done = 0;
    int polls = 0;
    d->h_done[1] = d->h_done[2] = 0;
    for (int t = 0; t < steps; ++t) {
        if (exec) {
            RGRG_HIP(hipGraphLaunch(exec, d->stream));
        } else {
            rc = step(d, S, t == 0);
            if (rc) return rc;
        }
        if ((t & 15) == 15 && t + 1 < steps) {
            if (polls > 0) {
                const int prev = (polls - 1) & 1;
                RGRG_HIP(hipEventSynchronize(d->ev_poll[prev]));
                if (d->h_done[1 + prev]) break;
            }
            const int cur = polls & 1;
            RGRG_HIP(hipMemcpyAsync(d->h_done + 1 + cur, d->done_len, sizeof(int), hipMemcpyDeviceToHost, d->stream));
            RGRG_HIP(hipEventRecord(d->ev_poll[cur], d->stream));
            ++polls;
        }
    }
    RGRG_HIP(hipMemcpyAsync(d->h_done, d->done_len, sizeof(int), hipMemcpyDeviceToHost, d->stream));
    RGRG_HIP(hipMemcpy2DAsync(out_ids, (size_t)out_ld * sizeof(int64_t), d->ids, (size_t)d->max_len * sizeof(long long),
                              (size_t)limit * sizeof(int64_t), S, hipMemcpyDeviceToDevice, d->stream));
    if (out_logprobs)
        RGRG_HIP(hipMemcpy2DAsync(out_logprobs, (size_t)out_ld * sizeof(float), d->sample_lp, (size_t)d->max_len * sizeof(float),
                                  (size_t)limit * sizeof(float), S, hipMemcpyDeviceToDevice, d->stream));
    RGRG_HIP(hipStreamSynchronize(d->stream));
    done = *d->h_done;
    *out_len = (done > 0 && done < limit) ? done : limit;
    d->logits_valid = true;
    return RGRG_OK;
}
}

static int greedy_step(rgrg_decoder* d, int S, bool count) { return enqueue_step(d, S, count); }

extern "C" int rgrg_decoder_generate(rgrg_decoder* d, const float* feats, int S, int max_length, int64_t* out_ids,
                                     int out_ld, int* out_len, int use_graph, void* stream) {
    RGRG_CHECK_ARG(d && feats && out_ids && out_len && S > 0 && S <= d->max_seqs);
    int limit = (max_length > 0) ? max_length : d->max_len;
    RGRG_CHECK_ARG(limit >= 2 && limit <= d->max_len && out_ld >= limit);
    int rc = decode_begin(d, stream);
    if (rc) return rc;
    if ((rc = run_decode_loop(d, feats, S, limit, 0, greedy_step, use_graph, out_ids, out_ld, nullptr, out_len))) return rc;
    d->logits_stale_rows = lm_head_cand_path(d, S) ? S : 0;
    return RGRG_OK;
}

namespace rgrg {
__global__ __launch_bounds__(256) void key_mask_kernel(const float* __restrict__ am, int L, int S, int T, float* __restrict__ kmask) {
    const int i = blockIdx.x * 256 + threadIdx.x;
    if (i >= S * T) return;
    const int s = i / T, j = i - s * T;
    kmask[i] = (j >= 1 && j <= L) ? (1.0f - am[(size_t)s * L + (j - 1)]) * -10000.0f : 0.f;
}
__global__ void set_int_kernel(int* p, int v) {
    if (threadIdx.x == 0 && blockIdx.x == 0) *p = v;
}
__global__ __launch_bounds__(256) void forward_cached_tokens_kernel(const long long* __restrict__ ids, const long long* __restrict__ pos_ids,
                                                                    int T, int j, int S, int V, int* __restrict__ tok,
                                                                    int* __restrict__ row_pos, int* __restrict__ step, int position) {
    const int s = blockIdx.x * 256 + threadIdx.x;
    if (s < S) {
        const long long t = ids[(size_t)s * T + j];
        tok[s] = (int)(t < 0 ? 0 : (t >= V ? V - 1 : t));
        if (pos_ids) {
            const long long q = pos_ids[(size_t)s * T + j];
            row_pos[s] = (int)(q < 0 ? 0 : (q >= V ? V - 1 : q));
        }
    }
    if (s == 0) *step = position;
}
}

extern "C" int rgrg_decoder_forward_cached(rgrg_decoder* d, const float* feats, const int64_t* input_ids, const int64_t* position_ids,
                                           const float* attention_mask, int S, int T, int past_len, float* logits_out, void* stream) {
    RGRG_CHECK_ARG(d && input_ids && logits_out && S > 0 && S <= d->max_seqs && T >= 1 && past_len >= 0);
    RGRG_CHECK_ARG(past_len == 0 || feats == nullptr);
    RGRG_CHECK_ARG(past_len + T <= d->max_len);
    if (attention_mask && kv_is_bf16(d, S)) {
        set_error("rgrg_decoder_forward_cached: attention_mask is not supported in precision mode %d for %d sequences (more than the "
                  "%d rows of the fp32-cache path): call rgrg_decoder_set_precision(d, 0) first", d->bf16_gemms, S, decode_row_limit(d));
        return RGRG_EINVAL;
    }
    hipStream_t caller = as_stream(stream), st = d->stream;
    RGRG_HIP(hipEventRecord(d->ev_in, caller));
    RGRG_HIP(hipStreamWaitEvent(st, d->ev_in, 0));
    int rc;
    d->logits_stale_rows = 0;
    d->logits_valid = false;
    if (past_len == 0 && feats && (rc = enqueue_prefill(d, feats, S))) return rc;
    if (attention_mask) {
        if (!d->key_mask && (rc = dmalloc(d, (void**)&d->key_mask, (size_t)d->rows * d->T * sizeof(float), true))) return rc;
        hipLaunchKernelGGL(key_mask_kernel, dim3((S * d->T + 255) / 256), dim3(256), 0, st, attention_mask, past_len + T, S, d->T, d->key_mask);
        RGRG_LAUNCH_CHECK();
    }
    for (int j = 0; j < T; ++j) {
        hipLaunchKernelGGL(forward_cached_tokens_kernel, dim3((S + 255) / 256), dim3(256), 0, st,
                           reinterpret_cast<const long long*>(input_ids), reinterpret_cast<const long long*>(position_ids), T, j, S, d->V,
                           d->beam_tok, d->row_pos, d->step, past_len + j);
        RGRG_LAUNCH_CHECK();
        d->pos_override_cur = position_ids ? d->row_pos : nullptr;
        d->key_mask_cur = attention_mask ? d->key_mask : nullptr;
        rc = enqueue_step(d, S, false, d->beam_tok, nullptr, true);
        d->pos_override_cur = nullptr;
        d->key_mask_cur = nullptr;
        if (rc) return rc;
        RGRG_HIP(hipMemcpy2DAsync(logits_out + (size_t)j * d->V, (size_t)T * d->V * sizeof(float), d->logits,
                                  (size_t)d->ld_logits * sizeof(float), (size_t)d->V * sizeof(float), S, hipMemcpyDeviceToDevice, st));
    }
    hipLaunchKernelGGL(set_int_kernel, dim3(1), dim3(64), 0, st, d->step, past_len + T);
    RGRG_LAUNCH_CHECK();
    RGRG_HIP(hipEventRecord(d->ev_in, st));
    RGRG_HIP(hipStreamWaitEvent(caller, d->ev_in, 0));
    d->logits_valid = true;
    return RGRG_OK;
}

extern "C" int rgrg_decoder_cache_plane(rgrg_decoder* d, int layer, int kv, void** ptr, int* max_seqs, int* slots, int* is_bf16) {
    RGRG_CHECK_ARG(d && ptr && layer >= 0 && layer < d->n_layer && (kv == 0 || kv == 1));
    *ptr = d->kv + (size_t)layer * d->kv_layer_stride + (size_t)kv * d->kv_kv_stride;
    if (max_seqs) *max_seqs = d->max_seqs;
    if (slots) *slots = d->T;
    if (is_bf16) *is_bf16 = 0;
    return RGRG_OK;
}

extern "C" int rgrg_decoder_take_id_error(rgrg_decoder* d, int* pending) {
    RGRG_CHECK_ARG(d && pending);
    RGRG_HIP(hipStreamSynchronize(d->stream));
    *pending = (d->h_id_error && *d->h_id_error) ? 1 : 0;
    if (*pending) {
        *d->h_id_error = 0;
        RGRG_HIP(hipMemsetAsync(d->id_error, 0, 2 * sizeof(int), d->stream));
    }
    return RGRG_OK;
}

extern "C" int rgrg_decoder_refresh_trainable(rgrg_decoder* d, void* stream) {
    RGRG_CHECK_ARG(d);
    hipStream_t caller = as_stream(stream), st = d->stream;
    RGRG_HIP(hipEventRecord(d->ev_in, caller));
    RGRG_HIP(hipStreamWaitEvent(st, d->ev_in, 0));
    Lin* ls[] = {&d->fst0, &d->fst2, &d->ukv};
    for (Lin* l : ls) {
        if (l->packed) {
            hipLaunchKernelGGL(pack_weights_kernel, dim3(2048), dim3(256), 0, st, l->w, l->packed, l->N, l->K, l->NT);
            RGRG_LAUNCH_CHECK();
        }
        if (l->wT) {
            int rc = launch_transpose_pad(l->w, l->wT, l->N, l->K, pad256(l->N), st);
            if (rc) return rc;
        }
    }
    RGRG_HIP(hipEventRecord(d->ev_in, st));
    RGRG_HIP(hipStreamWaitEvent(caller, d->ev_in, 0));
    return RGRG_OK;
}

extern "C" int rgrg_debug_attn_decode(const float* qkv, int ld_qkv, void* kcache, void* vcache, const int* step_dev, float* out,
                                      uint16_t* out16, int S, int H, int T_slots, const int* src, const float* kmask, int kv16,
                                      int fp16, int ni, int frag_out, int max_workgroups, void* stream) {
    RGRG_CHECK_ARG(qkv && kcache && vcache && step_dev && S > 0 && H > 0 && T_slots >= 2 && ld_qkv >= 3 * H * 64);
    RGRG_CHECK_ARG(out || (kv16 && out16));
    RGRG_CHECK_ARG(kv16 || (!out16 && max_workgroups == 0));
    RGRG_CHECK_ARG(!kv16 || (ni == 0 && frag_out == 0));
    AttnDecodeLaunch a{};
    a.qkv = qkv; a.ld_qkv = ld_qkv; a.kc = kcache; a.vc = vcache; a.plane_elems = (size_t)S * H * T_slots * 64;
    a.step = step_dev; a.out = out; a.out16 = out16; a.S = S; a.H = H; a.T = T_slots; a.src = src; a.kmask = kmask;
    a.fmt = kv16 ? (fp16 ? KV_F16 : KV_BF16) : KV_F32; a.f16 = fp16 ? 1 : 0; a.ni = ni; a.frag_out = frag_out ? 1 : 0; a.max_wgs = max_workgroups;
    a.st = as_stream(stream);
    return launch_attn_decode(a);
}

extern "C" int rgrg_debug_attn_decode_qonly(const float* q, int ld_q, const void* kcache, const void* vcache, const int* step_dev, float* out,
                                            uint16_t* out16, int S, int H, int T_slots, int fp16, int max_workgroups, void* stream) {
    RGRG_CHECK_ARG(q && kcache && vcache && step_dev && S > 0 && H > 0 && T_slots >= 2 && ld_q >= H * 64 && (out || out16));
    AttnDecodeLaunch a{};
    a.qkv = q; a.ld_qkv = ld_q; a.kc = const_cast<void*>(kcache); a.vc = const_cast<void*>(vcache);
    a.plane_elems = (size_t)S * H * T_slots * 64; a.step = step_dev; a.out = out; a.out16 = out16; a.S = S; a.H = H; a.T = T_slots;
    a.fmt = fp16 ? KV_F16 : KV_BF16; a.f16 = fp16 ? 1 : 0; a.max_wgs = max_workgroups; a.st = as_stream(stream); a.q_only = true;
    return launch_attn_decode(a);
}

extern "C" int rgrg_debug_attn_decode_kv8(const float* qkv, int ld_qkv, uint8_t* kcache, uint8_t* vcache, const int* step_dev, float* out,
                                          uint16_t* out16, int S, int H, int T_slots, const int* src, const float* kmask, int fp16,
                                          int max_workgroups, void* stream) {
    RGRG_CHECK_ARG(qkv && kcache && vcache && step_dev && S > 0 && H > 0 && T_slots >= 2 && ld_qkv >= 3 * H * 64 && (out || out16));
    AttnDecodeLaunch a{};
    a.qkv = qkv; a.ld_qkv = ld_qkv; a.kc = kcache; a.vc = vcache; a.plane_elems = (size_t)S * H * T_slots * 64;
    a.step = step_dev; a.out = out; a.out16 = out16; a.S = S; a.H = H; a.T = T_slots; a.src = src; a.kmask = kmask;
    a.fmt = KV_E4M3; a.f16 = fp16 ? 1 : 0; a.max_wgs = max_workgroups; a.st = as_stream(stream);
    return launch_attn_decode(a);
}

extern "C" int rgrg_debug_ln_fold16(const float* w, const float* gain, const float* beta, const float* bias, uint16_t* wb,
                                    float* colsum, float* shift, int N, int K, int fp16, void* stream) {
    RGRG_CHECK_ARG(w && gain && beta && wb && colsum && shift && N > 0 && K > 0);
    hipLaunchKernelGGL(ln_fold16_kernel, dim3((N + 3) / 4), dim3(256), 0, as_stream(stream), w, gain, beta, bias, wb, colsum, shift, N, K,
                       fp16 ? 1 : 0);
    RGRG_LAUNCH_CHECK();
    return RGRG_OK;
}

static int set_precision_impl(rgrg_decoder* d, int mode);
extern "C" int rgrg_decoder_set_precision(rgrg_decoder* d, int mode) {
    RGRG_CHECK_ARG(d && mode >= 0 && mode <= 2);
    if (mode == d->bf16_gemms) return RGRG_OK;
    const int prev = d->bf16_gemms;
    const int rc = set_precision_impl(d, mode);
    if (rc) {
        auto stale = [](Lin& l) { l.wb_f16 = -1; l.wb_ln_f16 = -1; l.wTb_f16 = -1; };
        stale(d->lm_head); stale(d->ukv); stale(d->fst2);
        for (auto& w : d->layers) { stale(w.c_attn); stale(w.attn_proj); stale(w.c_fc); stale(w.mlp_proj); }
        d->bf16_gemms = 0;
        (void)prev;
        for (auto& g : d->graphs) (void)hipGraphExecDestroy(g.exec);
        d->graphs.clear();
    }
    return rc;
}
static int set_precision_impl(rgrg_decoder* d, int mode) {
    d->logits_valid = false;
    const int prev = d->bf16_gemms;
    d->bf16_gemms = mode;
    if (mode) {
        int rc = init_gemm_bf16_attrs();
        if (rc) { d->bf16_gemms = prev; return rc; }
        auto mk = [&](Lin& l) -> int {
            if (l.wb && l.wb_f16 == d->f16()) return RGRG_OK;
            if (!l.wb) {
                int r = dmalloc(d, &l.wb, (size_t)l.N * l.K * 2, false);
                if (r) return r;
            }
            l.wb_f16 = d->f16();
            return convert_f32_to_bf16(l.w, l.wb, (size_t)l.N * l.K, d->stream, d->f16());
        };
        int rc2;
        RGRG_HIP(hipStreamSynchronize(d->stream));
        if (!d->xn16) {
            if ((rc2 = dmalloc(d, (void**)&d->xn16, (size_t)d->rows * d->D * 2, false)) ||
                (rc2 = dmalloc(d, (void**)&d->att16, (size_t)d->rows * d->D * 2, false)) ||
                (rc2 = dmalloc(d, (void**)&d->ff16, (size_t)d->rows * 4 * d->D * 2, false)))
                return rc2;
        }
        if ((rc2 = mk(d->lm_head))) return rc2;
        for (auto& w : d->layers) {
            if ((rc2 = mk(w.c_attn)) || (rc2 = mk(w.attn_proj)) || (rc2 = mk(w.c_fc)) || (rc2 = mk(w.mlp_proj))) return rc2;
        }
        if (d->w16_fused && d->rows > PAD_ROWS) {
            auto mk16 = [&](Lin& l) -> int {
                if (!l.direct || !l.packed || (l.packed16 && l.packed16_f16 == d->f16())) return RGRG_OK;
                const size_t n = (size_t)l.NT * 16 * l.K;
                int r;
                if (!l.packed16 && (r = dmalloc(d, &l.packed16, n * 2, false))) return r;
                if (l.lnf && !l.c1_16 && (r = dmalloc(d, (void**)&l.c1_16, (size_t)l.NT * 16 * sizeof(float), false))) return r;
                if ((r = convert_f32_to_bf16(l.packed, l.packed16, n, d->stream, d->f16()))) return r;
                if (l.lnf)
                    hipLaunchKernelGGL(packed16_colsum_kernel, dim3(l.NT), dim3(64), 0, d->stream, (const unsigned short*)l.packed16, l.c1_16, l.NT * 16, l.K,
                                       d->f16());
                l.packed16_f16 = d->f16();
                return RGRG_OK;
            };
            if ((rc2 = mk16(d->lm_head))) return rc2;
            for (auto& w : d->layers) {
                if ((rc2 = mk16(w.c_attn)) || (rc2 = mk16(w.attn_proj)) || (rc2 = mk16(w.c_fc)) || (rc2 = mk16(w.mlp_proj))) return rc2;
            }
        }
        if (const char* e = getenv("RGRG_LN_FOLD")) d->ln_fold = atoi(e) != 0;
        if (d->ln_fold && d->D == 1024) {
            auto mkln = [&](Lin& l, const float* g, const float* be) -> int {
                if (l.wb_ln && l.wb_ln_f16 == d->f16()) return RGRG_OK;
                int r;
                if (!l.wb_ln && ((r = dmalloc(d, &l.wb_ln, (size_t)l.N * l.K * 2, false)) ||
                                 (r = dmalloc(d, (void**)&l.cs16, (size_t)l.N * sizeof(float), false)) ||
                                 (r = dmalloc(d, (void**)&l.c2_16, (size_t)l.N * sizeof(float), false))))
                    return r;
                l.wb_ln_f16 = d->f16();
                hipLaunchKernelGGL(ln_fold16_kernel, dim3((l.N + 3) / 4), dim3(256), 0, d->stream, l.w, g, be, l.b,
                                   reinterpret_cast<unsigned short*>(l.wb_ln), l.cs16, l.c2_16, l.N, l.K, d->f16());
                RGRG_LAUNCH_CHECK();
                return RGRG_OK;
            };
            if (!d->ln_stat && (rc2 = dmalloc(d, (void**)&d->ln_stat, (size_t)d->rows * 32 * sizeof(float), true))) return rc2;
            if (!d->sk_ws) {
                const size_t tiles = (size_t)((d->rows + 63) / 64) * (d->D / 64);
                const size_t small_rows = (size_t)((std::min(d->rows, 256) + 127) / 128) * 2;
                const size_t slabs = std::max(tiles * 4, small_rows * (size_t)(4 * d->D / 64) * 2), tickets = std::max(tiles, small_rows * (size_t)(4 * d->D / 64));
                if ((rc2 = dmalloc(d, (void**)&d->sk_ws, slabs * 4096 * sizeof(float), false)) ||
                    (rc2 = dmalloc(d, (void**)&d->sk_cnt, tickets * sizeof(unsigned), true)))
                    return rc2;
                const char* e1 = getenv("RGRG_SK_MLP");
                const char* e2 = getenv("RGRG_SK_ATTN");
                d->sk_mlp = e1 ? atoi(e1) : -1;
                d->sk_attn = e2 ? atoi(e2) : -1;
                if (d->sk_mlp == 0) d->sk_mlp = 1;
                if (d->sk_attn == 0) d->sk_attn = 1;
                if (d->sk_mlp > 4) d->sk_mlp = 4;
                if (d->sk_attn > 4) d->sk_attn = 4;
            }
            for (auto& w : d->layers) {
                if ((rc2 = mkln(w.c_attn, w.ln1_g, w.ln1_b)) || (rc2 = mkln(w.c_fc, w.ln2_g, w.ln2_b))) return rc2;
            }
        }
        RGRG_HIP(hipStreamSynchronize(d->stream));
    }
    for (auto& g : d->graphs) (void)hipGraphExecDestroy(g.exec);
    d->graphs.clear();
    return RGRG_OK;
}

extern "C" int rgrg_decoder_set_kv_format(rgrg_decoder* d, int fmt) {
    RGRG_CHECK_ARG(d && (fmt == 0 || fmt == 1));
    if (fmt == d->kv8) return RGRG_OK;
    RGRG_HIP(hipStreamSynchronize(d->stream));
    d->kv8 = fmt;
    d->logits_valid = false;
    for (auto& g : d->graphs) (void)hipGraphExecDestroy(g.exec);
    d->graphs.clear();
    return RGRG_OK;
}

extern "C" int rgrg_decoder_kv_format_in_use(rgrg_decoder* d, int rows) { return d && rows > 0 ? (int)kv_format(d, rows) : -1; }

extern "C" int rgrg_decoder_copy_last_logits(rgrg_decoder* d, float* dst, int S, void* stream) {
    RGRG_CHECK_ARG(d && dst && S > 0 && S <= d->max_seqs);
    if (!d->logits_valid) {
        set_error("decoder: no logits of a completed step to copy - the last generate / beam / cached call failed, or a timing hook or a "
                  "precision change has reused the decoder's work space since");
        return RGRG_EINVAL;
    }
    if (d->logits_stale_rows > 0) {
        const int rows = d->logits_stale_rows;
        RGRG_CHECK_ARG(S <= rows);
        int rc = linear(d, d->lm_head, d->xn, nullptr, d->logits, rows, d->ld_logits, RGRG_ACT_NONE, false, d->xn16);
        if (rc) return rc;
        RGRG_HIP(hipStreamSynchronize(d->stream));
        d->logits_stale_rows = 0;
    }
    RGRG_HIP(hipMemcpy2DAsync(dst, (size_t)d->V * 4, d->logits, (size_t)d->ld_logits * 4, (size_t)d->V * 4, S,
                              hipMemcpyDeviceToDevice, as_stream(stream)));
    RGRG_HIP(hipStreamSynchronize(as_stream(stream)));
    return RGRG_OK;
}

extern "C" int rgrg_decoder_row_limit(rgrg_decoder* d) { return d ? decode_row_limit(d) : -1; }

extern "C" int rgrg_decoder_attention_only(rgrg_decoder* d, int S, int nkeys, int iters, void* stream) {
    RGRG_CHECK_ARG(d && S > decode_row_limit(d) && S <= d->rows && nkeys >= 2 && nkeys <= d->T && iters > 0);
    hipStream_t keep = d->stream;
    d->stream = as_stream(stream);
    hipLaunchKernelGGL(set_int_kernel, dim3(1), dim3(64), 0, d->stream, d->step, nkeys - 2);
    int rc = RGRG_OK;
    unsigned short* att16 = (kv_is_bf16(d, S) && d->xn16) ? d->att16 : nullptr;
    const bool qc = step_qkv_cache(d, S, true);
    for (int it = 0; it < iters && !rc; ++it)
        for (int l = 0; l < d->n_layer && !rc; ++l) rc = launch_attention(d, l, S, nullptr, att16, 0, 0, qc);
    hipLaunchKernelGGL(set_int_kernel, dim3(1), dim3(64), 0, d->stream, d->step, 0);
    d->stream = keep;
    return rc;
}

extern "C" int rgrg_decoder_trace_step(rgrg_decoder* d, int S, int nkeys, int iters, float* recs, int max_recs, int* n_out) {
    RGRG_CHECK_ARG(d && S > decode_row_limit(d) && S <= d->rows && nkeys >= 2 && nkeys <= d->T && recs && n_out && iters >= 0);
    d->logits_valid = false;
    std::vector<rgrg_decoder::TraceMark> marks;
    hipEvent_t base;
    RGRG_HIP(hipEventCreate(&base));
    int rc = RGRG_OK;
    for (int it = 0; it <= iters && !rc; ++it) {
        hipLaunchKernelGGL(set_int_kernel, dim3(1), dim3(64), 0, d->stream, d->step, nkeys - 2);
        if (it == iters) { d->trace = &marks; RGRG_HIP(hipEventRecord(base, d->stream)); }
        rc = enqueue_step(d, S, false);
    }
    d->trace = nullptr;
    (void)hipStreamSynchronize(d->stream);
    int n = 0;
    for (auto& m : marks) {
        float ms = 0.f;
        if (!rc && n < max_recs && hipEventElapsedTime(&ms, base, m.ev) == hipSuccess) {
            recs[3 * n] = (float)m.r0; recs[3 * n + 1] = (float)m.tag; recs[3 * n + 2] = ms;
            ++n;
        }
        (void)hipEventDestroy(m.ev);
    }
    (void)hipEventDestroy(base);
    hipLaunchKernelGGL(set_int_kernel, dim3(1), dim3(64), 0, d->stream, d->step, 0);
    (void)hipStreamSynchronize(d->stream);
    *n_out = n;
    return rc;
}

extern "C" int rgrg_decoder_time_step_parts(rgrg_decoder* d, int S, int nkeys, int iters, int one_range, float* ms_gemm, float* ms_attn,
                                            double* gemm_flops, double* gemm_weight_bytes, double* kv_bytes,
                                            int* gemm_launches) {
    RGRG_CHECK_ARG(d && S > 0 && S <= d->max_seqs && nkeys >= 2 && nkeys <= d->T && iters > 0 && ms_gemm && ms_attn);
// ... 104 lines not shown
```

rgrg_amd/csrc/decoder_internal.h:

```cpp
#pragma once
#include <vector>

#include "internal.h"

namespace rgrg {

constexpr int MAX_CHAINS = 4;
constexpr int PAD_ROWS = 32;
constexpr int SKINNY_MAX_ROWS = 128;
constexpr int BOS_ID = 50256, EOS_ID = 50256, PAD_ID = 50256;
constexpr int BEAM_K = 32;
enum KvFormat { KV_F32 = 0, KV_BF16 = 1, KV_F16 = 2, KV_E4M3 = 3 };
constexpr int KV8_CHUNK_KEYS = 144;

struct StepBook {
    long long* ids;
    int ld_ids;
    int *finished, *step, *done_len, *sync;
    int S;
};
#ifdef __HIPCC__
__device__ __forceinline__ int record_step_token(const StepBook& bk, int row, int t, int tok, bool* was_finished = nullptr) {
    int fin = bk.finished[row];
    if (was_finished) *was_finished = fin != 0;
    if (fin) tok = PAD_ID;
    bk.ids[(size_t)row * bk.ld_ids + t + 1] = tok;
    if (tok == EOS_ID) fin = 1;
    bk.finished[row] = fin;
    const unsigned mine = fin ? 0u : 0x10000u;
    const unsigned old = atomicAdd(reinterpret_cast<unsigned*>(bk.sync), 1u + mine);
    if ((old & 0xffffu) == (unsigned)(bk.S - 1)) {
        const unsigned unfinished = (old >> 16) + (mine >> 16);
        if (unfinished == 0 && *bk.done_len == 0) *bk.done_len = t + 2;
        *bk.step = t + 1;
        bk.sync[0] = 0;
    }
    return tok;
}
#endif

struct Lin {
    const float* w = nullptr;
    const float* b = nullptr;
    float* packed = nullptr;
    void* wb = nullptr;
    float* wT = nullptr;
    void* wTb = nullptr;
    int wb_f16 = 0, wTb_f16 = 0;
    void* wb_ln = nullptr;
    float *cs16 = nullptr, *c2_16 = nullptr;
    int wb_ln_f16 = -1;
    int N = 0, K = 0, NT = 0, KS = 1, ntile = 32;
    bool direct = false, lnf = false;
    float *c1 = nullptr, *c2 = nullptr;
    void* packed16 = nullptr;
    float* c1_16 = nullptr;
    int packed16_f16 = -1;
};

struct LayerW {
    const float *ln1_g, *ln1_b, *ln2_g, *ln2_b;
    Lin c_attn, attn_proj, c_fc, mlp_proj;
};

struct GraphEntry {
    int S;
    hipGraphExec_t exec;
    int key2 = 0, key3 = 0;
};

}

struct rgrg_decoder {
    int n_layer, D, H, V, max_seqs, rows, T, max_len;
    const float* wte;
    const float *lnf_g, *lnf_b;
    rgrg::Lin fst0, fst2, ukv, lm_head;
    std::vector<rgrg::LayerW> layers;
    float *feats, *h1, *img, *ukv_out, *x, *x2, *xn, *qkv, *att, *ff, *logits, *part, *kv, *cand_val, *gemm_ws;
    size_t gemm_ws_floats;
    int* cand_idx;
    size_t kv_layer_stride, kv_kv_stride;
    int ld_logits, ld_ukv;
    long long* ids;
    int *next, *finished, *step, *done_len, *sync;
    int *src_a, *src_b, *beam_tok, *beam_parent, *cand_tok, *cand_beam, *top_tok;
    float *beam_scores, *row_max, *row_logsum, *top_val, *cand_score;
    float *wide_val = nullptr, *wide_score = nullptr;
    int* wide_tok = nullptr;
    size_t wide_cap = 0;
    void* sample_prm = nullptr;
    float* sample_lp = nullptr;
    int* h_done;
    hipEvent_t ev_poll[2] = {nullptr, nullptr};
    int* id_error = nullptr;
    int* h_id_error = nullptr;
    hipStream_t stream;
    hipEvent_t ev_in;
    std::vector<rgrg::GraphEntry> graphs;
    std::vector<void*> allocs;
    size_t gemm_bytes_per_step = 0;
    double gemm_flops_per_step = 0.0;
    struct TfWork {
        float *x = nullptr, *xn = nullptr, *qkv = nullptr, *att = nullptr, *ff = nullptr, *logits = nullptr, *ws = nullptr,
              *row_loss = nullptr;
        int* row_valid = nullptr;
        size_t rows = 0, ws_floats = 0;
        const long long* pos = nullptr;
        int pos_rows = 1;
        void free() {
            float** fs[] = {&x, &xn, &qkv, &att, &ff, &logits, &ws, &row_loss};
            for (float** f : fs) { if (*f) (void)hipFree(*f); *f = nullptr; }
            if (row_valid) (void)hipFree(row_valid);
            row_valid = nullptr;
            rows = 0;
            ws_floats = 0;
        }
    } tf;
    struct TrWork {
        float *xs = nullptr, *qkv = nullptr, *ffpre = nullptr, *ff = nullptr, *dx = nullptr, *dbig = nullptr, *dxn = nullptr,
              *logits = nullptr, *dukv = nullptr, *t1 = nullptr, *t2 = nullptr, *dimg = nullptr, *dh1 = nullptr, *row_lse = nullptr,
              *att = nullptr, *lse = nullptr, *delta = nullptr;
        int* count = nullptr;
        size_t rows = 0, seqs = 0;
        unsigned short *xn16 = nullptr, *att16 = nullptr, *ff16 = nullptr, *ffpre16 = nullptr, *dx16 = nullptr, *dff16 = nullptr,
                       *dqkv16 = nullptr, *dl16 = nullptr;
        unsigned short *qkv16 = nullptr, *datt16 = nullptr, *ukv16 = nullptr;
        bool a16 = false;
        bool h16 = false;
        size_t chunk = 0;
        bool seen_a16 = false, seen_a32 = false, seen_h16 = false, seen_h32 = false, seen_h16_a32 = false;
        bool have_wT = false;
        void* a16_scratch = nullptr;
        size_t a16_bytes = 0;
        void free() {
            float** fs[] = {&xs, &qkv, &ffpre, &ff, &dx, &dbig, &dxn, &logits, &dukv, &t1, &t2, &dimg, &dh1, &row_lse, &att, &lse, &delta};
            for (float** f : fs) { if (*f) (void)hipFree(*f); *f = nullptr; }
            if (count) (void)hipFree(count);
            count = nullptr;
            unsigned short** hs[] = {&xn16, &att16, &ff16, &ffpre16, &dx16, &dff16, &dqkv16, &dl16, &qkv16, &datt16, &ukv16};
            for (unsigned short** h : hs) { if (*h) (void)hipFree(*h); *h = nullptr; }
            rows = seqs = 0;
            chunk = 0;
        }
    } tr;
    int bf16_gemms = 0;
    int f16() const { return bf16_gemms == 2 ? 1 : 0; }
    unsigned short *xn16 = nullptr, *att16 = nullptr, *ff16 = nullptr;
    float* sk_ws = nullptr;
    unsigned* sk_cnt = nullptr;
    int sk_attn = 0, sk_mlp = 0;
    int step_rows = 0;
    float* ln_stat = nullptr;
    bool ln_fold = true;
    float* key_mask = nullptr;
    const float* key_mask_cur = nullptr;
    struct TraceMark { hipEvent_t ev; int r0; int tag; };
    std::vector<TraceMark>* trace = nullptr;
    bool w16_fused = true;
    bool qkv_cache = true;
    int kp_gemms = 2;
    int gemm_launches_per_step = 0;
    const int* pos_override_cur = nullptr;
    int* row_pos = nullptr;
    int logits_stale_rows = 0;
    bool logits_valid = false;
    hipStream_t streams_x[rgrg::MAX_CHAINS - 1] = {};
    hipEvent_t ev_fork = nullptr, ev_join[rgrg::MAX_CHAINS - 1] = {};
    int kv8 = 0;
    int chains = 4;
};

namespace rgrg {

inline int pad256(int n) { return (n + 255) / 256 * 256; }

int dmalloc(rgrg_decoder* d, void** p, size_t bytes, bool zero);
int skinny_max_rows();
int linear(rgrg_decoder* d, const Lin& l, const float* X, const float* R, float* Y, int M, int ldy, int act,
           bool count, const unsigned short* X16 = nullptr, unsigned short* Y16 = nullptr, const GemmLnFold* ln = nullptr);
int launch_ln_rows(const float* x, const float* g, const float* b, float* xn, int D, unsigned short* xn16, int f16, int rows,
                   hipStream_t st);
int enqueue_step(rgrg_decoder* d, int S, bool count, const int* tok_override = nullptr, const int* src = nullptr,
                 bool beam = false);
int enqueue_prefill(rgrg_decoder* d, const float* feats, int S, int row_mul = 1);
int decode_begin(rgrg_decoder* d, void* stream);
int launch_attn_decode_kv8(const float* qkv, int ld_qkv, uint8_t* kc, uint8_t* vc, const int* step, float* out, unsigned short* out16,
                           int S, int H, int T, const int* src, int f16, int workgroups, hipStream_t st);
int run_decode_loop(rgrg_decoder* d, const float* feats, int S, int limit, int graph_key, int (*step)(rgrg_decoder*, int, bool),
                    int use_graph, int64_t* out_ids, int out_ld, float* out_logprobs, int* out_len);

}
```

rgrg_amd/csrc/gemm_bf16.hip:

```cpp
#include "internal.h"

namespace rgrg {

typedef short bf16x8 __attribute__((ext_vector_type(8)));
typedef short bf16x4 __attribute__((ext_vector_type(4)));
typedef unsigned short u16;

struct GemmBf16Params {
    const float* A;
    const u16* A16;
    const u16* Wb;
    const float* shift;
    const float* R;
    float* Y;
    u16* Y16;
    int M, N, K, ldy, act;
    int lda = 0, ldw = 0;
    int cH = 0, cW = 0, cCin = 0, cKH = 0, cKW = 0, cStride = 1, cPad = 0, cOH = 0, cOW = 0;
    const u16* R16 = nullptr;
    int f16 = 0;
    u16* Yb16 = nullptr;
    float* stats_out = nullptr;
    const float* ln_stats = nullptr;
    const float* ln_colsum = nullptr;
    u16 *kv_k = nullptr, *kv_v = nullptr;
    const int* kv_step = nullptr;
    int kv_H = 0, kv_T = 0;
    u16* Ypre16 = nullptr;
    const u16* G16 = nullptr;
    int gm = 0;
    int ksplit = 0;
    float* sk_ws = nullptr;
    unsigned* sk_cnt = nullptr;
    float* cand_val = nullptr;
    int* cand_idx = nullptr;
    int dbg = 0;
};

constexpr float LN_EPS16 = 1e-5f;

constexpr int BK16 = 64;
constexpr int LDB = (BK16 * 2 + 16) / 2;

template <bool F16>
__device__ __forceinline__ f32x16 mfma16(const bf16x8& a, const bf16x8& b, const f32x16& c) {
    if constexpr (F16) return __builtin_amdgcn_mfma_f32_32x32x16_f16(__builtin_bit_cast(f16x8, a), __builtin_bit_cast(f16x8, b), c, 0, 0, 0);
    else return __builtin_amdgcn_mfma_f32_32x32x16_bf16(a, b, c, 0, 0, 0);
}

template <int BM, int BN, int THREADS, bool A16, bool F16>
__global__ __launch_bounds__(THREADS) void gemm_bf16w_kernel(const GemmBf16Params p, const int mtiles, const int ntiles) {
    constexpr int WAVES = THREADS / 64, WN = WAVES / 2;
    constexpr int TM = BM / 2, TN = BN / WN;
    constexpr int MI = TM / 32, NI = TN / 32;
    constexpr int AL = BM * 8 / THREADS, BL = BN * 8 / THREADS;
    constexpr int RSTEP = THREADS / 8;
    constexpr int NS = 4;
    extern __shared__ __attribute__((aligned(16))) u16 smem16[];
    u16* As = smem16;
    u16* Bs = smem16 + 2 * BM * LDB;
    const int tid = threadIdx.x, lane = tid & 63, wave = tid >> 6;
    const int wm = wave / WN, wn = wave % WN;
    const int total = mtiles * ntiles;
    int t = blockIdx.x;
    if ((total & 7) == 0) t = (t & 7) * (total >> 3) + (t >> 3);
    const int tn = t / mtiles, tm = t - tn * mtiles;
    const int m0 = tm * BM, n0 = tn * BN;
    const int kchunk = tid & 7, lrow = tid >> 3;
    const int nk = p.K / BK16;

    const float* aptr[AL];
    const u16* aptr16[AL];
    const u16* bptr[BL];
#pragma unroll
    for (int i = 0; i < AL; ++i) {
        const int m = min(m0 + lrow + RSTEP * i, p.M - 1);
        aptr[i] = A16 ? nullptr : p.A + (size_t)m * p.K + kchunk * 4;
        aptr16[i] = A16 ? p.A16 + (size_t)m * p.K + kchunk * 8 : nullptr;
    }
#pragma unroll
    for (int i = 0; i < BL; ++i) {
        const int n = min(n0 + lrow + RSTEP * i, p.N - 1);
        bptr[i] = p.Wb + (size_t)n * p.K + kchunk * 8;
    }

    f32x4 ra[NS][AL][2];
    bf16x8 ra16[NS][AL];
    bf16x8 rb[NS][BL];
#define RGRG_LOAD_TILE(S, KT)                                                                    \
    {                                                                                            \
        const int koff = (KT) * BK16;                                                            \
        _Pragma("unroll") for (int i = 0; i < AL; ++i) {                                         \
            if constexpr (A16) {                                                                 \
                ra16[S][i] = *reinterpret_cast<const bf16x8*>(aptr16[i] + koff);                 \
            } else {                                                                             \
                ra[S][i][0] = *reinterpret_cast<const f32x4*>(aptr[i] + koff);                   \
                ra[S][i][1] = *reinterpret_cast<const f32x4*>(aptr[i] + koff + 32);              \
            }                                                                                    \
        }                                                                                        \
        _Pragma("unroll") for (int i = 0; i < BL; ++i)                                           \
            rb[S][i] = *reinterpret_cast<const bf16x8*>(bptr[i] + koff);                         \
    }
#define RGRG_STORE_ITEM(S, BUF, I)                                                               \
    {                                                                                            \
        if ((I) < AL) {                                                                          \
            constexpr int i = (I) < AL ? (I) : 0;                                                \
            if constexpr (A16) {                                                                 \
                *reinterpret_cast<bf16x8*>(&As[((BUF) * BM + lrow + RSTEP * i) * LDB + kchunk * 8]) = ra16[S][i]; \
            } else {                                                                             \
                bf16x4 lo, hi;                                                                   \
                _Pragma("unroll") for (int e = 0; e < 4; ++e) {                                  \
                    lo[e] = (short)to16<F16>(ra[S][i][0][e]);                                    \
                    hi[e] = (short)to16<F16>(ra[S][i][1][e]);                                    \
                }                                                                                \
                u16* dst = &As[((BUF) * BM + lrow + RSTEP * i) * LDB + kchunk * 4];              \
                *reinterpret_cast<bf16x4*>(dst) = lo;                                            \
                *reinterpret_cast<bf16x4*>(dst + 32) = hi;                                       \
            }                                                                                    \
        } else {                                                                                 \
            constexpr int i = (I) >= AL ? (I) - AL : 0;                                          \
            *reinterpret_cast<bf16x8*>(&Bs[((BUF) * BN + lrow + RSTEP * i) * LDB + kchunk * 8]) = rb[S][i]; \
        }                                                                                        \
    }
#define RGRG_STORE_TILE(S, BUF) \
    { RGRG_STORE_ITEM(S, BUF, 0) RGRG_STORE_ITEM(S, BUF, 1) RGRG_STORE_ITEM(S, BUF, 2) RGRG_STORE_ITEM(S, BUF, 3) }
    static_assert(AL + BL == BK16 / 16, "one staging item per 16-wide K step");

    f32x16 acc[MI][NI];
#pragma unroll
    for (int mi = 0; mi < MI; ++mi)
#pragma unroll
        for (int ni = 0; ni < NI; ++ni)
#pragma unroll
            for (int r = 0; r < 16; ++r) acc[mi][ni][r] = 0.f;

#pragma unroll
    for (int s = 0; s < NS; ++s) RGRG_LOAD_TILE(s, s)
    __builtin_amdgcn_sched_barrier(0);
    RGRG_STORE_TILE(0, 0)
    __syncthreads();

    const int frow = lane & 31, fk = (lane >> 5) * 8;
    for (int kt0 = 0; kt0 < nk; kt0 += NS) {
#pragma unroll
        for (int s = 0; s < NS; ++s) {
            const int kt = kt0 + s;
            {
                const int buf = kt & 1;
                RGRG_LOAD_TILE(s, min(kt + NS, nk - 1))
                __builtin_amdgcn_sched_barrier(0);
                const u16* Ab = &As[(buf * BM + wm * TM + frow) * LDB + fk];
                const u16* Bb = &Bs[(buf * BN + wn * TN + frow) * LDB + fk];
                bf16x8 a[2][MI], b[2][NI];
#pragma unroll
                for (int mi = 0; mi < MI; ++mi) a[0][mi] = *reinterpret_cast<const bf16x8*>(Ab + mi * 32 * LDB);
#pragma unroll
                for (int ni = 0; ni < NI; ++ni) b[0][ni] = *reinterpret_cast<const bf16x8*>(Bb + ni * 32 * LDB);
#define RGRG_KSTEP(KS)                                                                                       \
    {                                                                                                        \
        if ((KS) + 1 < BK16 / 16) {                                                                          \
            _Pragma("unroll") for (int mi = 0; mi < MI; ++mi) a[((KS) + 1) & 1][mi] =                        \
                *reinterpret_cast<const bf16x8*>(Ab + mi * 32 * LDB + ((KS) + 1) * 16);                      \
            _Pragma("unroll") for (int ni = 0; ni < NI; ++ni) b[((KS) + 1) & 1][ni] =                        \
                *reinterpret_cast<const bf16x8*>(Bb + ni * 32 * LDB + ((KS) + 1) * 16);                      \
        }                                                                                                    \
        _Pragma("unroll") for (int mi = 0; mi < MI; ++mi) _Pragma("unroll") for (int ni = 0; ni < NI; ++ni)  \
            acc[mi][ni] = mfma16<F16>(a[(KS) & 1][mi], b[(KS) & 1][ni], acc[mi][ni]);                        \
        RGRG_STORE_ITEM((s + 1) % NS, buf ^ 1, KS)                                                           \
    }
                RGRG_KSTEP(0) RGRG_KSTEP(1) RGRG_KSTEP(2) RGRG_KSTEP(3)
#undef RGRG_KSTEP
                __syncthreads();
            }
        }
    }
#undef RGRG_LOAD_TILE
#undef RGRG_STORE_TILE
#undef RGRG_STORE_ITEM
    const int ccol = lane & 31, crow4 = 4 * (lane >> 5);
#pragma unroll
    for (int mi = 0; mi < MI; ++mi)
#pragma unroll
        for (int ni = 0; ni < NI; ++ni) {
            const int col = n0 + wn * TN + ni * 32 + ccol;
            const int colc = min(col, p.N - 1);
            const int rbase = m0 + wm * TM + mi * 32 + crow4;
            const float sh = p.shift ? p.shift[colc] : 0.f;
            float rv[16];
// ... 358 lines not shown
                        }
                    }
#pragma unroll
                    for (int r = 0; r < 16; ++r) vv[r] = apply_act_fast(acc[mi][ni][r] + sh + rv[r], p.act);
                }
            } else {
#pragma unroll
                for (int r = 0; r < 16; ++r) vv[r] = apply_act_fast(acc[mi][ni][r] + sh + rv[r], p.act);
            }
            bool to_cache = false;
            if constexpr (KVC) to_cache = n0 + wn * (BN / 2) + ni * 32 >= p.kv_H * 64;
            if (to_cache) {
                const int Dm = p.kv_H * 64, c = col - Dm, isv = c >= Dm ? 1 : 0, ch = c - isv * Dm;
                u16* plane = isv ? p.kv_v : p.kv_k;
                const size_t o0 = ((size_t)(ch >> 6) * p.kv_T + kv_slot) * 64 + (ch & 63);
                if (kv_slot < p.kv_T) {
#pragma unroll
                    for (int r = 0; r < 16; ++r) {
                        const int row = rbase + (r & 3) + 8 * (r >> 2);
                        if (row < p.M) plane[(size_t)row * p.kv_H * p.kv_T * 64 + o0] = (u16)to16<F16>(vv[r]);
                    }
                }
            } else if (col < p.N) {
#pragma unroll
                for (int r = 0; r < 16; ++r) {
                    const int dr = (r & 3) + 8 * (r >> 2);
                    const float v = vv[r];
                    if (rbase + dr < p.M) {
                        const size_t o = (size_t)rbase * p.ldy + col + (size_t)(dr * p.ldy);
                        if (p.Y16) p.Y16[o] = (u16)to16<F16>(v);
                        else if (p.N > 8192) __builtin_nontemporal_store(v, &p.Y[o]);
                        else p.Y[o] = v;
                        if constexpr (LNF == 1) p.Yb16[o] = (u16)to16<F16>(v);
                    }
                }
            }
            if constexpr (LNF == 1) {
                float a1[16], a2[16];
#pragma unroll
                for (int r = 0; r < 16; ++r) { a1[r] = vv[r]; a2[r] = vv[r] * vv[r]; }
#define RGRG_BFLY(H, BIT)                                                                         \
                {                                                                                         \
                    const bool up = (lane & (BIT)) != 0;                                                  \
                    _Pragma("unroll") for (int i = 0; i < (H); ++i) {                                     \
                        const float s1 = up ? a1[i] : a1[i + (H)], s2 = up ? a2[i] : a2[i + (H)];         \
                        const float k1 = up ? a1[i + (H)] : a1[i], k2 = up ? a2[i + (H)] : a2[i];         \
                        a1[i] = k1 + __shfl_xor(s1, (BIT), 64);                                           \
                        a2[i] = k2 + __shfl_xor(s2, (BIT), 64);                                           \
                    }                                                                                     \
                }
                RGRG_BFLY(8, 16) RGRG_BFLY(4, 8) RGRG_BFLY(2, 4) RGRG_BFLY(1, 2)
#undef RGRG_BFLY
                a1[0] += __shfl_xor(a1[0], 1, 64);
                a2[0] += __shfl_xor(a2[0], 1, 64);
                blk1[mi] += a1[0];
                blk2[mi] += a2[0];
            }
        }
    if constexpr (LNF == 1) {
        float2* xch = reinterpret_cast<float2*>(glds_smem + NST * STAGE);
        const int r = (lane >> 1) & 15, lrow = (r & 3) + 8 * (r >> 2) + 4 * (lane >> 5);
        if constexpr (NI == 1) {
            if (wn == 1 && !(lane & 1)) {
#pragma unroll
                for (int mi = 0; mi < MI; ++mi) xch[(wave * MI + mi) * 32 + lrow] = make_float2(blk1[mi], blk2[mi]);
            }
            __syncthreads();
        }
        if (!(lane & 1) && (NI == 2 || wn == 0)) {
#pragma unroll
            for (int mi = 0; mi < MI; ++mi) {
                float s1 = blk1[mi], s2 = blk2[mi];
                if constexpr (NI == 1) {
                    const float2 o = xch[((wave + 1) * MI + mi) * 32 + lrow];
                    s1 += o.x; s2 += o.y;
                }
                const int row = m0 + wm * (BM / 2) + mi * 32 + lrow;
                const int slot = NI == 2 ? (n0 + wn * 64) / 64 : n0 / 64;
                if (row < p.M) *reinterpret_cast<float2*>(p.stats_out + ((size_t)row * 16 + slot) * 2) = make_float2(s1, s2);
            }
        }
    }
}

template <int TAG>
__device__ __forceinline__ void pp_dma4(const u16* base, unsigned char* dst, const int (&v)[4], int soff) {
    const __amdgpu_buffer_rsrc_t r = bf16_rsrc(base);
#pragma unroll
    for (int j = 0; j < 4; ++j) __builtin_amdgcn_raw_ptr_buffer_load_lds(r, (lds_ptr_t)(dst + j * 8192), 16, v[j], soff, 0, 0);
}
template <int TAG>
__device__ __forceinline__ void pp_dma2(const u16* base, unsigned char* dst, int v0, int v1, int soff) {
    const __amdgpu_buffer_rsrc_t r = bf16_rsrc(base);
    __builtin_amdgcn_raw_ptr_buffer_load_lds(r, (lds_ptr_t)dst, 16, v0, soff, 0, 0);
    __builtin_amdgcn_raw_ptr_buffer_load_lds(r, (lds_ptr_t)(dst + 1024), 16, v1, soff, 0, 0);
}
template <bool F16>
__global__ __launch_bounds__(512) void gemm_bf16_pp_kernel(const GemmBf16Params p, const int mtiles, const int ntiles) {
    constexpr int BM = 256, BN = 256, BK = 64, MI = 4, NI = 2;
    constexpr int STAGE = (BM + BN) * 128, WOFF = BM * 128;
    constexpr int TAG = F16 ? 901 : 900;
    extern __shared__ __attribute__((aligned(16))) unsigned char pp_smem[];
    const int tid = threadIdx.x, lane = tid & 63;
    const int wave = __builtin_amdgcn_readfirstlane(tid >> 6);
    const int g = wave >> 2, wq = wave & 3;
    int t = blockIdx.x;
    {
        const int total = mtiles * ntiles, q = total >> 3, r = total & 7, x = t & 7, i = t >> 3;
        t = (x < r ? x * (q + 1) : r * (q + 1) + (x - r) * q) + i;
    }
    int tn, tm;
    if (p.gm <= 0 || p.gm >= mtiles) {
        tn = t / mtiles; tm = t - tn * mtiles;
    } else {
        const int gsz = p.gm * ntiles, gi = t / gsz, r = t - gi * gsz;
        const int rows = min(p.gm, mtiles - gi * p.gm);
        tn = r / rows; tm = gi * p.gm + (r - tn * rows);
    }
    const int m0 = tm * BM, n0 = tn * BN;
    const int nk = p.K / BK;
    const int lda = p.lda ? p.lda : p.K, ldw = p.ldw ? p.ldw : p.K;
    const u16* abase = p.A16 + (size_t)m0 * lda;
    const u16* wbase = p.Wb + (size_t)n0 * ldw;
    const int lrow = lane >> 3, lch = lane & 7;
    auto src_off = [&](int row0, int limit, int ld) { const int row = row0 + lrow; return min(row, limit) * ld * 2 + ((lch ^ ((row >> 1) & 7)) << 4); };
    const int ra0 = (g == 0 ? 192 : 0) + wq * 16, ra1 = (g == 0 ? 128 : 64) + wq * 16;
    const int rw0 = (g == 0 ? 0 : 128) + wq * 16, rw1 = rw0 + 64;
    const int va00 = src_off(ra0, p.M - 1 - m0, lda), va01 = src_off(ra0 + 8, p.M - 1 - m0, lda);
    const int va10 = src_off(ra1, p.M - 1 - m0, lda), va11 = src_off(ra1 + 8, p.M - 1 - m0, lda);
    const int vw00 = src_off(rw0, p.N - 1 - n0, ldw), vw01 = src_off(rw0 + 8, p.N - 1 - n0, ldw);
    const int vw10 = src_off(rw1, p.N - 1 - n0, ldw), vw11 = src_off(rw1 + 8, p.N - 1 - n0, ldw);
    unsigned char* const da0 = pp_smem + ra0 * 128;
    unsigned char* const da1 = pp_smem + ra1 * 128;
    unsigned char* const dw0 = pp_smem + WOFF + rw0 * 128;
    unsigned char* const dw1 = pp_smem + WOFF + rw1 * 128;
    const int frow = lane & 31, fh = lane >> 5, fsw = (frow >> 1) & 7;
    int foff[4];
#pragma unroll
    for (int ks = 0; ks < 4; ++ks) foff[ks] = frow * 128 + (((2 * ks + fh) ^ fsw) << 4);
    const unsigned char* const fa_base = pp_smem + g * (128 * 128);
    const unsigned char* const fb_base = pp_smem + WOFF + wq * (64 * 128);

    f32x16 acc[MI][NI];
#pragma unroll
    for (int mi = 0; mi < MI; ++mi)
#pragma unroll
        for (int ni = 0; ni < NI; ++ni)
#pragma unroll
            for (int r = 0; r < 16; ++r) acc[mi][ni][r] = 0.f;
    bf16x8 fa[4][2], fb[4][NI];
    float esh[NI];
#pragma unroll
    for (int ni = 0; ni < NI; ++ni) esh[ni] = p.shift ? p.shift[min(n0 + wq * 64 + ni * 32 + (lane & 31), p.N - 1)] : 0.f;
    const int dbg = __builtin_amdgcn_readfirstlane(p.dbg);
    if (dbg) {
#pragma unroll
        for (int ks = 0; ks < 4; ++ks)
#pragma unroll
            for (int i = 0; i < 2; ++i) { fa[ks][i] = bf16x8{1, 2, 3, 4, 5, 6, 7, 8}; fb[ks][i] = bf16x8{8, 7, 6, 5, 4, 3, 2, 1}; }
    }

#define PP_READ_A(ST_, H_)                                                                                       \
    if (!(dbg & 1)) {                                                                                            \
        const unsigned char* sa_ = fa_base + (ST_) * STAGE + (H_) * (64 * 128);                                  \
        _Pragma("unroll") for (int ks = 0; ks < 4; ++ks)                                                         \
            _Pragma("unroll") for (int m2 = 0; m2 < 2; ++m2)                                                     \
                fa[ks][m2] = *reinterpret_cast<const bf16x8*>(sa_ + m2 * 4096 + foff[ks]);                       \
    }
#define PP_READ_W(ST_)                                                                                           \
    if (!(dbg & 1)) {                                                                                            \
        const unsigned char* sw_ = fb_base + (ST_) * STAGE;                                                      \
        _Pragma("unroll") for (int ks = 0; ks < 4; ++ks)                                                         \
            _Pragma("unroll") for (int ni = 0; ni < NI; ++ni)                                                    \
                fb[ks][ni] = *reinterpret_cast<const bf16x8*>(sw_ + ni * 4096 + foff[ks]);                       \
    }
#define PP_MUL(H_)                                                                                               \
    if (!(dbg & 4)) {                                                                                            \
        __builtin_amdgcn_s_setprio(1);                                                                           \
        _Pragma("unroll") for (int ks = 0; ks < 4; ++ks)                                                         \
            _Pragma("unroll") for (int m2 = 0; m2 < 2; ++m2)                                                     \
                _Pragma("unroll") for (int ni = 0; ni < NI; ++ni)                                                \
                    acc[(H_) * 2 + m2][ni] = mfma16<F16>(fa[ks][m2], fb[ks][ni], acc[(H_) * 2 + m2][ni]);        \
        __builtin_amdgcn_s_setprio(0);                                                                           \
    }
#define PP_BAR()                                  \
    {                                             \
        __builtin_amdgcn_sched_barrier(0);        \
        __builtin_amdgcn_s_barrier();             \
        __builtin_amdgcn_sched_barrier(0);        \
    }
#define PP_END_READ(FIRST_, DO_, TA_, WAIT_)                                                                                  \
    {                                                                                                                          \
        if ((DO_) && !(dbg & 2)) {                                                                                             \
            pp_dma2<TAG>(abase, ((FIRST_) ? da0 : da1) + ((TA_) & 1) * STAGE, (FIRST_) ? va00 : va10, (FIRST_) ? va01 : va11, (TA_) * (BK * 2)); \
            if (!(FIRST_)) {                                                                                                   \
                pp_dma2<TAG>(wbase, dw0 + ((TA_) & 1) * STAGE, vw00, vw01, (TA_) * (BK * 2));                                  \
                pp_dma2<TAG>(wbase, dw1 + ((TA_) & 1) * STAGE, vw10, vw11, (TA_) * (BK * 2));                                  \
            }                                                                                                                  \
        }                                                                                                                      \
        asm volatile("s_waitcnt lgkmcnt(0)" ::: "memory");                                                                     \
        if (dbg & 2) wait_vmcnt<0>(); else wait_vmcnt<WAIT_>();                                                                \
        PP_BAR()                                                                                                               \
    }

    {
        int vpa[4], vpw[4];
#pragma unroll
        for (int j = 0; j < 4; ++j) {
            vpa[j] = src_off((j * 8 + wave) * 8, p.M - 1 - m0, lda);
            vpw[j] = src_off((j * 8 + wave) * 8, p.N - 1 - n0, ldw);
        }
        unsigned char* const dst = pp_smem + wave * 1024;
        pp_dma4<TAG>(wbase, dst + WOFF, vpw, 0);
        pp_dma4<TAG>(abase, dst, vpa, 0);
        pp_dma4<TAG>(wbase, dst + STAGE + WOFF, vpw, BK * 2);
        pp_dma4<TAG>(abase, dst + STAGE, vpa, BK * 2);
    }
    wait_vmcnt<8>();
    PP_BAR()

#define PP_TILE_G0(D0_, W0_, D2_, W2_)                                              \
    {                                                                               \
        const int cur = kt & 1;                                                     \
        PP_READ_A(cur, 0) PP_READ_W(cur)                                            \
        PP_END_READ(true, D0_, kt + 1, W0_)                                         \
        PP_MUL(0)                                                                   \
        PP_BAR()                                                                    \
        PP_READ_A(cur, 1)                                                           \
        PP_END_READ(false, D2_, kt + 2, W2_)                                        \
        PP_MUL(1)                                                                   \
        PP_BAR()                                                                    \
    }
#define PP_TILE_G1(FIRSTKT_, D1_, W1_, D3_, W3_)                                    \
    {                                                                               \
        const int cur = kt & 1;                                                     \
        if (!(FIRSTKT_)) PP_MUL(1)                                                  \
        PP_BAR()                                                                    \
        PP_READ_A(cur, 0) PP_READ_W(cur)                                            \
        PP_END_READ(true, D1_, kt + 2, W1_)                                         \
        PP_MUL(0)                                                                   \
        PP_BAR()                                                                    \
        PP_READ_A(cur, 1)                                                           \
        PP_END_READ(false, D3_, kt + 2, W3_)                                        \
    }
    if (g == 0) {
        int kt = 0;
        PP_TILE_G0(0, 0, 1, 6)
        for (kt = 1; kt < nk - 2; ++kt) PP_TILE_G0(1, 8, 1, 8)
        PP_TILE_G0(1, 8, 0, 2)
        ++kt;
        PP_TILE_G0(0, 0, 0, 0)
    } else {
        int kt = 0;
        PP_TILE_G1(true, 1, 2, 1, 8)
        for (kt = 1; kt < nk - 2; ++kt) PP_TILE_G1(false, 1, 8, 1, 8)
        PP_TILE_G1(false, 0, 6, 0, 0)
        ++kt;
        PP_TILE_G1(false, 0, 0, 0, 0)
        PP_MUL(1)
    }
#undef PP_TILE_G0
#undef PP_TILE_G1
#undef PP_END_READ
#undef PP_MUL
#undef PP_READ_A
#undef PP_READ_W
#undef PP_BAR

    if (dbg & 8) {
        float z = 0.f;
#pragma unroll
        for (int mi = 0; mi < MI; ++mi)
#pragma unroll
            for (int ni = 0; ni < NI; ++ni)
#pragma unroll
                for (int r = 0; r < 16; ++r) z += acc[mi][ni][r];
        if (z == 12345.678f) p.Y[0] = z;
        return;
    }
    if (p.cand_val) {
        __syncthreads();
        float* cv = reinterpret_cast<float*>(pp_smem);
        int* ci = reinterpret_cast<int*>(pp_smem + 4096);
        const int ccol = lane & 31;
#pragma unroll
        for (int mi = 0; mi < MI; ++mi) {
            float bv[16];
            int bi[16];
            const int c0 = n0 + wq * 64 + ccol, c1 = c0 + 32;
#pragma unroll
            for (int r = 0; r < 16; ++r) {
                const float v0 = c0 < p.N ? acc[mi][0][r] + esh[0] : -INFINITY;
                const float v1 = c1 < p.N ? acc[mi][1][r] + esh[1] : -INFINITY;
                const bool hi = v1 > v0;
                bv[r] = hi ? v1 : v0;
                bi[r] = hi ? c1 : c0;
            }
#define PP_CAND_STEP(CNT_, XOR_)                                                                   \
    {                                                                                              \
        const bool up = (lane & (XOR_)) != 0;                                                      \
        _Pragma("unroll") for (int j = 0; j < (CNT_); ++j) {                                       \
            const float keep_v = up ? bv[j + (CNT_)] : bv[j], send_v = up ? bv[j] : bv[j + (CNT_)]; \
            const int keep_i = up ? bi[j + (CNT_)] : bi[j], send_i = up ? bi[j] : bi[j + (CNT_)];   \
            const float ov = __shfl_xor(send_v, (XOR_), 64);                                       \
            const int oi = __shfl_xor(send_i, (XOR_), 64);                                         \
            const bool take = ov > keep_v || (ov == keep_v && oi < keep_i);                        \
            bv[j] = take ? ov : keep_v;                                                            \
// ... 43 lines not shown
            float rv[16], vv[16];
#pragma unroll
            for (int r = 0; r < 16; ++r) rv[r] = 0.f;
            if (p.R) {
#pragma unroll
                for (int r = 0; r < 16; ++r) {
                    const int row = min(rbase + (r & 3) + 8 * (r >> 2), p.M - 1);
                    rv[r] = p.R[(size_t)row * p.ldy + colc];
                }
            }
            if (p.G16) {
#pragma unroll
                for (int r = 0; r < 16; ++r) {
                    const int row = min(rbase + (r & 3) + 8 * (r >> 2), p.M - 1);
                    rv[r] = from16<F16>(p.G16[(size_t)row * p.ldy + colc]);
                }
#pragma unroll
                for (int r = 0; r < 16; ++r) vv[r] = (acc[mi][ni][r] + sh) * gelu_new_grad_fast(rv[r]);
            } else {
                if (p.Ypre16 && col < p.N) {
#pragma unroll
                    for (int r = 0; r < 16; ++r) {
                        const int dr = (r & 3) + 8 * (r >> 2);
                        if (rbase + dr < p.M)
                            p.Ypre16[(size_t)rbase * p.ldy + col + (size_t)(dr * p.ldy)] = (u16)to16<F16>(acc[mi][ni][r] + sh + rv[r]);
                    }
                }
#pragma unroll
                for (int r = 0; r < 16; ++r) vv[r] = apply_act_fast(acc[mi][ni][r] + sh + rv[r], p.act);
            }
            if (col < p.N) {
#pragma unroll
                for (int r = 0; r < 16; ++r) {
                    const int dr = (r & 3) + 8 * (r >> 2);
                    if (rbase + dr < p.M) {
                        const size_t o = (size_t)rbase * p.ldy + col + (size_t)(dr * p.ldy);
                        if (p.Y16) p.Y16[o] = (u16)to16<F16>(vv[r]);
                        else if (p.N > 8192) __builtin_nontemporal_store(vv[r], &p.Y[o]);
                        else p.Y[o] = vv[r];
                    }
                }
            }
        }
}

__global__ __launch_bounds__(256) void f32_to_bf16_kernel(const float* __restrict__ src, u16* __restrict__ dst, size_t n, int f16) {
    for (size_t i = (size_t)blockIdx.x * blockDim.x + threadIdx.x; i < n; i += (size_t)gridDim.x * blockDim.x)
        dst[i] = (u16)to16_rt(src[i], f16);
}

template <int BM, int BN, int THREADS>
static int launch_bf16_cfg(const GemmBf16Params& p, hipStream_t st) {
    constexpr size_t lds = (size_t)(2 * BM + 2 * BN) * LDB * sizeof(u16);
    const int mtiles = (p.M + BM - 1) / BM, ntiles = (p.N + BN - 1) / BN;
#define RGRG_W_LAUNCH(A16_, F16_) hipLaunchKernelGGL((gemm_bf16w_kernel<BM, BN, THREADS, A16_, F16_>), dim3(mtiles * ntiles), dim3(THREADS), lds, st, p, mtiles, ntiles)
    if (p.A16) { if (p.f16) RGRG_W_LAUNCH(true, true); else RGRG_W_LAUNCH(true, false); }
    else { if (p.f16) RGRG_W_LAUNCH(false, true); else RGRG_W_LAUNCH(false, false); }
#undef RGRG_W_LAUNCH
    RGRG_LAUNCH_CHECK();
    return RGRG_OK;
}

template <int BM, int BN, int THREADS>
static int bf16_attr() {
    RGRG_HIP(hipFuncSetAttribute(reinterpret_cast<const void*>(&gemm_bf16w_kernel<BM, BN, THREADS, false, false>),
                                 hipFuncAttributeMaxDynamicSharedMemorySize, 81920));
    RGRG_HIP(hipFuncSetAttribute(reinterpret_cast<const void*>(&gemm_bf16w_kernel<BM, BN, THREADS, true, false>),
                                 hipFuncAttributeMaxDynamicSharedMemorySize, 81920));
    RGRG_HIP(hipFuncSetAttribute(reinterpret_cast<const void*>(&gemm_bf16w_kernel<BM, BN, THREADS, false, true>),
                                 hipFuncAttributeMaxDynamicSharedMemorySize, 81920));
    RGRG_HIP(hipFuncSetAttribute(reinterpret_cast<const void*>(&gemm_bf16w_kernel<BM, BN, THREADS, true, true>),
                                 hipFuncAttributeMaxDynamicSharedMemorySize, 81920));
    return RGRG_OK;
}

template <int BM, int BN, int NST>
static int glds_attr() {
    constexpr int lds = NST * (BM + BN) * 128 + BM * 16;
#define RGRG_G_ATTR(...) RGRG_HIP(hipFuncSetAttribute(reinterpret_cast<const void*>(&gemm_bf16_glds_kernel<BM, BN, NST, __VA_ARGS__>), hipFuncAttributeMaxDynamicSharedMemorySize, lds))
    RGRG_G_ATTR(false, false, 0); RGRG_G_ATTR(true, false, 0); RGRG_G_ATTR(false, true, 0); RGRG_G_ATTR(true, true, 0);
    RGRG_G_ATTR(false, false, 1); RGRG_G_ATTR(false, true, 1); RGRG_G_ATTR(false, false, 2); RGRG_G_ATTR(false, true, 2);
    RGRG_G_ATTR(false, false, 3); RGRG_G_ATTR(false, true, 3);
#undef RGRG_G_ATTR
    return RGRG_OK;
}
template <int BM, int BN>
static int glds_attrs() {
    int rc;
    if ((rc = glds_attr<BM, BN, 2>()) || (rc = glds_attr<BM, BN, 3>())) return rc;
    return glds_attr<BM, BN, 4>();
}

static int gemm_gm_override();
#include "gemm_kp.inc"

constexpr int PP_LDS = 2 * (256 + 256) * 128;

int init_gemm_bf16_attrs() {
    static bool done = false;
    if (done) return RGRG_OK;
    int rc;
    if ((rc = bf16_attr<128, 128, 512>()) || (rc = bf16_attr<64, 64, 256>())) return rc;
    if ((rc = glds_attrs<128, 128>()) || (rc = glds_attrs<64, 64>()) || (rc = glds_attrs<128, 64>()) || (rc = glds_attrs<64, 128>())) return rc;
    RGRG_HIP(hipFuncSetAttribute(reinterpret_cast<const void*>(&gemm_bf16_pp_kernel<false>), hipFuncAttributeMaxDynamicSharedMemorySize, PP_LDS));
    RGRG_HIP(hipFuncSetAttribute(reinterpret_cast<const void*>(&gemm_bf16_pp_kernel<true>), hipFuncAttributeMaxDynamicSharedMemorySize, PP_LDS));
    if ((rc = kp_attr<128, 128, 2>()) || (rc = kp_attr<64, 64, 4>()) || (rc = kp_attr<64, 64, 3>()) || (rc = kp_attr<128, 64, 3>()) || (rc = kp_attr<64, 128, 3>()) || (rc = kp_attr<64, 64, 2>()) || (rc = pr_attrs())) return rc;
    done = true;
    return RGRG_OK;
}

static int gemm_gm_override() {
    static const int v = [] { const char* e = getenv("RGRG_GEMM_GM"); return e ? atoi(e) : 0; }();
    return v;
}

template <int BM, int BN, int NST>
static int launch_glds_cfg(const GemmBf16Params& p0, hipStream_t st) {
    GemmBf16Params p = p0;
    const int mtiles = (p.M + BM - 1) / BM, ntiles = (p.N + BN - 1) / BN;
    if (p.gm == 0) {
        const int o = gemm_gm_override();
        p.gm = o < 0 ? 0 : o > 0 ? o : (mtiles > 16 ? 8 : 0);
    }
    const int ks = (!p.cCin && p.ksplit > 1 && p.sk_ws && p.sk_cnt && (p.K / 64) % p.ksplit == 0 && p.K / 64 / p.ksplit >= NST - 1) ? p.ksplit : 1;
    p.ksplit = ks;
#define RGRG_G_LAUNCH(CONV_, F16_, LNF_) hipLaunchKernelGGL((gemm_bf16_glds_kernel<BM, BN, NST, CONV_, F16_, LNF_>), dim3(mtiles * ntiles * ks), dim3(256), NST * (BM + BN) * 128 + BM * 16, st, p, mtiles, ntiles)
    if (p.cCin) { if (p.f16) RGRG_G_LAUNCH(true, true, 0); else RGRG_G_LAUNCH(true, false, 0); }
    else if (p.Yb16) { if (p.f16) RGRG_G_LAUNCH(false, true, 1); else RGRG_G_LAUNCH(false, false, 1); }
    else if (p.ln_colsum && p.kv_k) { if (p.f16) RGRG_G_LAUNCH(false, true, 3); else RGRG_G_LAUNCH(false, false, 3); }
    else if (p.ln_colsum) { if (p.f16) RGRG_G_LAUNCH(false, true, 2); else RGRG_G_LAUNCH(false, false, 2); }
    else { if (p.f16) RGRG_G_LAUNCH(false, true, 0); else RGRG_G_LAUNCH(false, false, 0); }
#undef RGRG_G_LAUNCH
    RGRG_LAUNCH_CHECK();
    return RGRG_OK;
}
template <int BM, int BN>
static int launch_glds_nst(const GemmBf16Params& p, int nst, hipStream_t st) {
    if (nst == 2) return launch_glds_cfg<BM, BN, 2>(p, st);
    if (nst == 3) return launch_glds_cfg<BM, BN, 3>(p, st);
    return launch_glds_cfg<BM, BN, 4>(p, st);
}

static bool pp_eligible(const GemmBf16Params& p) {
    return !p.cCin && !p.Yb16 && !p.ln_colsum && !p.R16 && p.K >= 256 && p.K % 64 == 0;
}
static int launch_pp(const GemmBf16Params& p0, hipStream_t st) {
    GemmBf16Params p = p0;
    const int mtiles = (p.M + 255) / 256, ntiles = (p.N + 255) / 256;
    if (p.gm == 0) {
        const int o = gemm_gm_override();
        p.gm = o < 0 ? 0 : o > 0 ? o : (mtiles > 8 ? 8 : 0);
    }
    { const char* e = getenv("RGRG_PP_DBG"); p.dbg = e ? atoi(e) : 0; }
    if (p.f16) hipLaunchKernelGGL(gemm_bf16_pp_kernel<true>, dim3(mtiles * ntiles), dim3(512), PP_LDS, st, p, mtiles, ntiles);
    else hipLaunchKernelGGL(gemm_bf16_pp_kernel<false>, dim3(mtiles * ntiles), dim3(512), PP_LDS, st, p, mtiles, ntiles);
    RGRG_LAUNCH_CHECK();
    return RGRG_OK;
}
static bool pp_enabled() {
    static const bool v = [] { const char* e = getenv("RGRG_GEMM_PP"); return !e || atoi(e) != 0; }();
    return v;
}

static bool pp_lm_head() {
    static const bool v = [] { const char* e = getenv("RGRG_GEMM_PP_LMHEAD"); return !e || atoi(e) != 0; }();
    return v;
}

static int launch_glds(const GemmBf16Params& p, int tile, hipStream_t st) {
    int shape = tile & 15, nst = tile >> 4;
    if (p.kv_k && shape >= 5) { set_error("bf16 GEMM: only the LDS-DMA kernel has the K/V-cache epilogue (tile %d)", tile); return RGRG_EINVAL; }
    switch (shape) {
        case 6: return launch_kp_cfg<128, 128, 2>(p, st);
        case 7: return launch_kp_cfg<64, 64, 4>(p, st);
        case 8: return launch_kp_cfg<128, 64, 3>(p, st);
        case 9: return launch_kp_cfg<64, 128, 3>(p, st);
        case 10: return launch_kp_cfg<64, 64, 3>(p, st);
        case 11: return launch_kp_auto(p, st);
        case 12: return launch_pr(p, st);
        case 13: return launch_kp_cfg<64, 64, 2>(p, st);
    }
    if (shape == 5) {
        if (!pp_eligible(p)) { set_error("bf16 GEMM: the 256 x 256 kernel does not take this variant"); return RGRG_EINVAL; }
        return launch_pp(p, st);
    }
    if (shape == 0 && pp_enabled() && pp_eligible(p)) {
        const long tiles_pp = (long)((p.M + 255) / 256) * ((p.N + 255) / 256);
        if (p.M >= 2048 && tiles_pp >= 192) return launch_pp(p, st);
        if (p.M >= 512 && p.N >= 32768 && tiles_pp >= 512 && pp_lm_head()) return launch_pp(p, st);
    }
    if (shape == 0 && p.ln_colsum && p.M <= 320) {
        static const int o = [] { const char* e = getenv("RGRG_CONS_TILE_SMALLM"); return e ? atoi(e) : 0; }();
        if (o) { shape = o & 15; nst = o >> 4; }
    }
    if (shape == 0) {
        const long tiles_big = (long)((p.M + 127) / 128) * ((p.N + 127) / 128);
        if (p.N <= 64) { shape = 3; nst = 2; }
        else if (tiles_big >= 512) { shape = 1; nst = 2; }
        else if (p.K >= 8192 && tiles_big >= 192) { shape = 1; nst = 2; }
        else if (p.K > 1024) { shape = 2; nst = 4; }
        else if (tiles_big >= 256) { shape = 3; nst = 3; }
        else if (tiles_big >= 128) { shape = 2; nst = 3; }
        else { shape = 2; nst = 4; }
    }
    if (nst == 0) nst = 4;
    if (p.K / 64 < nst - 1) nst = 2;
    switch (shape) {
        case 1: return launch_glds_nst<128, 128>(p, nst, st);
        case 2: return launch_glds_nst<64, 64>(p, nst, st);
        case 3: return launch_glds_nst<128, 64>(p, nst, st);
        case 4: return launch_glds_nst<64, 128>(p, nst, st);
    }
    set_error("bf16 GEMM: unknown tile configuration %d", tile);
    return RGRG_EINVAL;
}

bool gemm_bf16_cand_epilogue_ok(int M, int N, int K) {
    static const bool on = [] { const char* e = getenv("RGRG_LMHEAD_CAND"); return !e || atoi(e) != 0; }();
    const long tiles_pp = (long)((M + 255) / 256) * ((N + 255) / 256);
    return on && pp_enabled() && pp_lm_head() && M >= 512 && N >= 32768 && tiles_pp >= 512 && K >= 256 && K % 64 == 0;
}

int launch_gemm_bf16w_ex(const float* A, const void* A16, const void* Wb, const float* shift, const float* R, float* Y, void* Y16,
                         int M, int N, int K, int ldy, int act, hipStream_t st, int f16, const GemmLnFold* ln) {
    RGRG_CHECK_ARG((A || A16) && Wb && (Y || Y16 || (ln && ln->cand_val)) && M > 0 && N > 0 && K > 0 && K % (4 * BK16) == 0 && ldy >= N);
    GemmBf16Params p{A, reinterpret_cast<const u16*>(A16), reinterpret_cast<const u16*>(Wb), shift, R, Y,
                     reinterpret_cast<u16*>(Y16), M, N, K, ldy, act};
    p.f16 = f16 ? 1 : 0;
    if (ln && (ln->Ypre16 || ln->G16)) {
        RGRG_CHECK_ARG(A16 && (size_t)128 * K * 2 < ((size_t)1 << 31) && !ln->Yb16 && !ln->ln_colsum);
        RGRG_CHECK_ARG(!(ln->Ypre16 && ln->G16) && (!ln->G16 || (!R && act == RGRG_ACT_NONE)));
        p.Ypre16 = reinterpret_cast<u16*>(ln->Ypre16); p.G16 = reinterpret_cast<const u16*>(ln->G16);
    } else if (ln && (ln->Yb16 || ln->ln_colsum)) {
        RGRG_CHECK_ARG(A16 && (size_t)128 * K * 2 < ((size_t)1 << 31));
        RGRG_CHECK_ARG((ln->Yb16 != nullptr) != (ln->ln_colsum != nullptr));
        RGRG_CHECK_ARG(!ln->Yb16 || (Y && ln->stats_out && N == 1024));
        RGRG_CHECK_ARG(!ln->ln_colsum || (ln->ln_stats && K == 1024 && !R));
        p.Yb16 = reinterpret_cast<u16*>(ln->Yb16); p.stats_out = ln->stats_out;
        p.ln_stats = ln->ln_stats; p.ln_colsum = ln->ln_colsum;
        if (ln->kv_k) {
            RGRG_CHECK_ARG(ln->ln_colsum && ln->kv_v && ln->kv_step && ln->kv_H > 0 && ln->kv_T >= 2 && N == 3 * ln->kv_H * 64 && Y && !Y16 && !ln->kp &&
                           ln->ksplit <= 1 && act == RGRG_ACT_NONE);
            p.kv_k = reinterpret_cast<u16*>(ln->kv_k); p.kv_v = reinterpret_cast<u16*>(ln->kv_v);
            p.kv_step = ln->kv_step; p.kv_H = ln->kv_H; p.kv_T = ln->kv_T;
        }
    } else if (ln && ln->kv_k) {
        set_error("bf16 GEMM: the K/V-cache epilogue belongs to the folded-LayerNorm consumer");
        return RGRG_EINVAL;
    }
    if (ln && ln->ksplit > 1) { p.ksplit = ln->ksplit; p.sk_ws = ln->sk_ws; p.sk_cnt = ln->sk_cnt; }
    if (ln && ln->cand_val) {
        RGRG_CHECK_ARG(A16 && ln->cand_idx && !R && act == RGRG_ACT_NONE && !Y16 && !ln->Yb16 && !ln->ln_colsum && !ln->Ypre16 && !ln->G16);
        p.cand_val = ln->cand_val; p.cand_idx = ln->cand_idx;
        return launch_glds(p, 5, st);
    }
    if (ln && ln->kp && A16 && (size_t)128 * K * 2 < ((size_t)1 << 31) && kp_eligible(p, 4)) return launch_glds(p, 11, st);
    if (A16 && (size_t)128 * K * 2 < ((size_t)1 << 31)) return launch_glds(p, 0, st);
    const long tiles_big = (long)((M + 127) / 128) * ((N + 127) / 128);
    return tiles_big >= 192 ? launch_bf16_cfg<128, 128, 512>(p, st) : launch_bf16_cfg<64, 64, 256>(p, st);
}

int launch_gemm_bf16w(const float* A, const void* Wb, const float* shift, const float* R, float* Y, int M, int N, int K,
                      int ldy, int act, hipStream_t st, int f16) {
    return launch_gemm_bf16w_ex(A, nullptr, Wb, shift, R, Y, nullptr, M, N, K, ldy, act, st, f16, nullptr);
}

__global__ __launch_bounds__(256) void bf16_to_f32_kernel(const u16* __restrict__ src, float* __restrict__ dst, size_t n, int f16) {
    for (size_t i = (size_t)blockIdx.x * blockDim.x + threadIdx.x; i < n; i += (size_t)gridDim.x * blockDim.x)
        dst[i] = from16_rt(src[i], f16);
}

int convert_f32_to_bf16(const float* src, void* dst, size_t n, hipStream_t st, int f16) {
    const int blocks = (int)((n + 255) / 256 < 4096 ? (n + 255) / 256 : 4096);
    hipLaunchKernelGGL(f32_to_bf16_kernel, dim3(blocks), dim3(256), 0, st, src, reinterpret_cast<u16*>(dst), n, f16 ? 1 : 0);
    RGRG_LAUNCH_CHECK();
    return RGRG_OK;
}

}

using namespace rgrg;

extern "C" int rgrg_f32_to_bf16(const float* src, uint16_t* dst, int64_t n, int fp16, void* stream) {
    RGRG_CHECK_ARG(src && dst && n > 0);
    return convert_f32_to_bf16(src, dst, (size_t)n, as_stream(stream), fp16);
}

extern "C" int rgrg_bf16_to_f32(const uint16_t* src, float* dst, int64_t n, int fp16, void* stream) {
    RGRG_CHECK_ARG(src && dst && n > 0);
    const int blocks = (int)(((size_t)n + 255) / 256 < 4096 ? ((size_t)n + 255) / 256 : 4096);
    hipLaunchKernelGGL(bf16_to_f32_kernel, dim3(blocks), dim3(256), 0, as_stream(stream), src, dst, (size_t)n, fp16 ? 1 : 0);
    RGRG_LAUNCH_CHECK();
    return RGRG_OK;
}

extern "C" int rgrg_linear_bf16w_f32(const float* A, const uint16_t* Wb, const float* shift, const float* R, float* Y,
                                     int M, int N, int K, int ldy, int act, int fp16, void* stream) {
    int rc = init_gemm_bf16_attrs();
    if (rc) return rc;
    return launch_gemm_bf16w(A, Wb, shift, R, Y, M, N, K, ldy, act, as_stream(stream), fp16);
}

extern "C" int rgrg_linear_bf16_f32(const uint16_t* A16, const uint16_t* Wb, const float* shift, const float* R, float* Y,
                                    uint16_t* Y16, int M, int N, int K, int ldy, int act, int fp16, void* stream) {
    int rc = init_gemm_bf16_attrs();
    if (rc) return rc;
// ... 91 lines not shown
```

rgrg_amd/csrc/runtime.hip:

```cpp
#include <stdarg.h>
#include <string.h>

#include "common.h"

namespace rgrg {
static thread_local char g_err[512] = "";
void set_error(const char* fmt, ...) {
    va_list ap;
    va_start(ap, fmt);
    vsnprintf(g_err, sizeof(g_err), fmt, ap);
    va_end(ap);
}
}

extern "C" const char* rgrg_last_error(void) { return rgrg::g_err; }
extern "C" int rgrg_abi_version(void) { return 25; }
extern "C" int rgrg_device_arch(int dev, char* buf, int buflen) {
    RGRG_CHECK_ARG(buf && buflen > 1);
    hipDeviceProp_t prop;
    RGRG_HIP(hipGetDeviceProperties(&prop, dev));
    strncpy(buf, prop.gcnArchName, buflen - 1);
    buf[buflen - 1] = 0;
    return RGRG_OK;
}

#include <chrono>
namespace rgrg {
__global__ void chain_kernel(int* p, int n) {
    if (threadIdx.x == 0 && blockIdx.x == 0) p[0] += n;
}
}

extern "C" int rgrg_debug_chain(int n, int mode, int blocks, float* us_per_kernel) {
    RGRG_CHECK_ARG(n > 0 && us_per_kernel && blocks > 0);
    int* d = nullptr;
    RGRG_HIP(hipMalloc((void**)&d, 64));
    RGRG_HIP(hipMemset(d, 0, 64));
    hipStream_t st = nullptr;
    if (mode != 2) RGRG_HIP(hipStreamCreateWithFlags(&st, hipStreamNonBlocking));
    hipGraphExec_t exec = nullptr;
    if (mode == 1) {
        hipGraph_t g = nullptr;
        RGRG_HIP(hipStreamBeginCapture(st, hipStreamCaptureModeThreadLocal));
        for (int i = 0; i < n; ++i) hipLaunchKernelGGL(rgrg::chain_kernel, dim3(blocks), dim3(64), 0, st, d, 1);
        RGRG_HIP(hipStreamEndCapture(st, &g));
        RGRG_HIP(hipGraphInstantiate(&exec, g, nullptr, nullptr, 0));
        (void)hipGraphDestroy(g);
        RGRG_HIP(hipGraphLaunch(exec, st));
        RGRG_HIP(hipStreamSynchronize(st));
    } else {
        for (int i = 0; i < 16; ++i) hipLaunchKernelGGL(rgrg::chain_kernel, dim3(blocks), dim3(64), 0, st, d, 1);
        RGRG_HIP(hipStreamSynchronize(st));
    }
    auto t0 = std::chrono::steady_clock::now();
    if (mode == 1) {
        RGRG_HIP(hipGraphLaunch(exec, st));
    } else {
        for (int i = 0; i < n; ++i) hipLaunchKernelGGL(rgrg::chain_kernel, dim3(blocks), dim3(64), 0, st, d, 1);
    }
    RGRG_HIP(hipStreamSynchronize(st));
    auto t1 = std::chrono::steady_clock::now();
    *us_per_kernel = (float)(std::chrono::duration<double, std::micro>(t1 - t0).count() / n);
    if (exec) (void)hipGraphExecDestroy(exec);
    if (st) (void)hipStreamDestroy(st);
    (void)hipFree(d);
    return RGRG_OK;
}
```

Before: 89.18 images/sec.

## Fuse next-step embedding+LN into argmax kernel; skip empty GEMM M-tiles; size argmax

During greedy decoding, the argmax/update kernel now also computes the next step's token+position embedding and layer-0 LayerNorm into dedicated buffers. This removes the separate embed_ln launch at the start of each decode step. The first embedding is launched once after prefill. The change also adds a smaller argmax unroll variant for small candidate counts, and a flag that makes the pipelined bf16 GEMM skip M half-tiles beyond M. Together these cut per-step kernel count and wasted work, at the cost of extra buffers and more complicated state handling.

After: 88.91 images/sec. No clear change (-0.3%).

```diff
diff --git a/include/rgrg_hip.h b/include/rgrg_hip.h
--- a/include/rgrg_hip.h
+++ b/include/rgrg_hip.h
@@ -131,6 +131,11 @@
                                  int tile, int fp16, void* stream);
 int rgrg_debug_linear_bf16_argmax(const uint16_t* A16, const uint16_t* Wb, const float* shift, int M, int N, int K,
                                   float* cand_val, int* cand_idx, int fp16, void* stream);
+int rgrg_debug_argmax_update(const float* cand_val, const int* cand_idx, int NT, long long* ids, int ld_ids, int* finished,
+                             int* step, int* done_len, int* sync, int S, int sized, const float* wte, const float* gain,
+                             const float* bias, float* x, uint16_t* xn16, float* stats, int fp16, void* stream);
+int rgrg_debug_decoder_step_state(rgrg_decoder* d, int S, float* x, uint16_t* xn16, float* stats, float* x_emb, uint16_t* xn16_emb,
+                                  float* stat_emb);
 int rgrg_debug_ln_fold16(const float* w, const float* gain, const float* beta, const float* bias, uint16_t* wb, float* colsum,
                          float* shift, int N, int K, int fp16, void* stream);
 int rgrg_debug_linear_bf16_ln(const uint16_t* A16, const uint16_t* Wb, const float* shift, const float* R, float* Y,
diff --git a/rgrg_amd/_hip.py b/rgrg_amd/_hip.py
--- a/rgrg_amd/_hip.py
+++ b/rgrg_amd/_hip.py
@@ -10,7 +10,7 @@
 _i, _f, _p = C.c_int, C.c_float, C.c_void_p
 
 ACT_NONE, ACT_RELU, ACT_GELU_NEW = 0, 1, 2
-ABI_VERSION = 25
+ABI_VERSION = 26
 
 
 class RgrgHipError(RuntimeError):
@@ -76,6 +76,8 @@
     "rgrg_debug_linear_bf16_tile": (_i, [_p, _p, _p, _p, _p, _i, _i, _i, _i, _i, _i, _i, _i, _i, _p]),
     "rgrg_debug_linear_bf16_train": (_i, [_p, _p, _p, _p, _p, _p, _p, _p, _i, _i, _i, _i, _i, _i, _i, _p]),
     "rgrg_debug_linear_bf16_argmax": (_i, [_p, _p, _p, _i, _i, _i, _p, _p, _i, _p]),
+    "rgrg_debug_argmax_update": (_i, [_p, _p, _i, _p, _i, _p, _p, _p, _p, _i, _i, _p, _p, _p, _p, _p, _p, _i, _p]),
+    "rgrg_debug_decoder_step_state": (_i, [_p, _i, _p, _p, _p, _p, _p, _p]),
     "rgrg_debug_ln_fold16": (_i, [_p, _p, _p, _p, _p, _p, _p, _i, _i, _i, _p]),
     "rgrg_debug_linear_bf16_ln": (_i, [_p, _p, _p, _p, _p, _p, _p, _p, _p, _i, _i, _i, _i, _i, _i, _p]),
     "rgrg_debug_linear_bf16_ln_kp": (_i, [_p, _p, _p, _p, _p, _p, _p, _p, _p, _p, _i, _i, _i, _i, _i, _i, _i, _p]),
diff --git a/rgrg_amd/csrc/decoder.hip b/rgrg_amd/csrc/decoder.hip
--- a/rgrg_amd/csrc/decoder.hip
+++ b/rgrg_amd/csrc/decoder.hip
@@ -253,16 +253,18 @@
 }
 
 
-__global__ __launch_bounds__(256) void embed_ln_kernel(const float* __restrict__ wte, const long long* __restrict__ ids,
-                                                       int ld_ids, const int* __restrict__ step, const float* __restrict__ g,
-                                                       const float* __restrict__ b, float* __restrict__ x,
-                                                       float* __restrict__ xn, int D, const int* __restrict__ tok_override,
-                                                       unsigned short* __restrict__ xn16, int f16, const int* __restrict__ pos_override,
-                                                       float* __restrict__ stats) {
-    __shared__ float sh[4];
-    const int s = blockIdx.x, tid = threadIdx.x;
-    const int t = pos_override ? pos_override[s] : *step;
-    const long long tok = tok_override ? (long long)tok_override[s] : ids[(size_t)s * ld_ids + *step];
+struct EmbedOut {
+    const float *wte, *g, *b;
+    float *x, *xn;
+    unsigned short* xn16;
+    float* stats;
+    int D, f16;
+};
+__device__ __forceinline__ void embed_ln_row(const EmbedOut& e, int s, long long tok, int t, float* sh) {
+    const int tid = threadIdx.x, D = e.D, f16 = e.f16;
+    const float *wte = e.wte, *g = e.g, *b = e.b;
+    float *x = e.x, *xn = e.xn, *stats = e.stats;
+    unsigned short* xn16 = e.xn16;
     const f32x4 v = reinterpret_cast<const f32x4*>(wte + (size_t)tok * D)[tid] + reinterpret_cast<const f32x4*>(wte + (size_t)t * D)[tid];
     reinterpret_cast<f32x4*>(x + (size_t)s * D)[tid] = v;
     if (stats) {
@@ -275,6 +277,18 @@
     const f32x4 o = ln_row(v, g, b, sh, D);
     if (xn16) store_16x4(xn16 + (size_t)s * D + 4 * tid, o, f16);
     else reinterpret_cast<f32x4*>(xn + (size_t)s * D)[tid] = o;
+}
+__global__ __launch_bounds__(256) void embed_ln_kernel(const float* __restrict__ wte, const long long* __restrict__ ids,
+                                                       int ld_ids, const int* __restrict__ step, const float* __restrict__ g,
+                                                       const float* __restrict__ b, float* __restrict__ x,
+                                                       float* __restrict__ xn, int D, const int* __restrict__ tok_override,
+                                                       unsigned short* __restrict__ xn16, int f16, const int* __restrict__ pos_override,
+                                                       float* __restrict__ stats) {
+    __shared__ float sh[4];
+    const int s = blockIdx.x;
+    const int t = pos_override ? pos_override[s] : *step;
+    const long long tok = tok_override ? (long long)tok_override[s] : ids[(size_t)s * ld_ids + *step];
+    embed_ln_row(EmbedOut{wte, g, b, x, xn, xn16, stats, D, f16}, s, tok, t, sh);
 }
 
 __global__ __launch_bounds__(256) void ln_rows_kernel(const float* __restrict__ x, const float* __restrict__ g,
@@ -648,13 +662,17 @@
     }
 }
 
-constexpr int ARGMAX_U = 13;
+constexpr int ARGMAX_U_MAX = 13;
+template <int ARGMAX_U, bool EMBED>
 __global__ __launch_bounds__(256) void argmax_update_kernel(const float* __restrict__ cand_val, const int* __restrict__ cand_idx,
                                                             int NT, long long* __restrict__ ids, int ld_ids,
                                                             int* __restrict__ finished, int* __restrict__ step,
-                                                            int* __restrict__ done_len, int* __restrict__ sync, int S) {
+                                                            int* __restrict__ done_len, int* __restrict__ sync, int S,
+                                                            const EmbedOut emb) {
     __shared__ float bv[4];
     __shared__ int bi[4];
+    __shared__ float esh[4];
+    __shared__ int etok;
     const int row = blockIdx.x, tid = threadIdx.x, lane = tid & 63, wave = tid >> 6;
     const int t = *step;
     const float* cv = cand_val + (size_t)row * NT;
@@ -688,8 +706,28 @@
         for (int w = 1; w < 4; ++w)
             if (bv[w] > best || (bv[w] == best && bi[w] < idx)) { best = bv[w]; idx = bi[w]; }
         const StepBook bk{ids, ld_ids, finished, step, done_len, sync, S};
-        record_step_token(bk, row, t, idx == 0x7fffffff ? 0 : idx);
-    }
+        const int tok = record_step_token(bk, row, t, idx == 0x7fffffff ? 0 : idx);
+        if constexpr (EMBED) etok = tok;
+    }
+    if constexpr (EMBED) {
+        __syncthreads();
+        embed_ln_row(emb, row, (long long)etok, t + 1, esh);
+    }
+}
+static int launch_argmax(const float* cand_val, const int* cand_idx, int NT, const StepBook& bk, bool sized, hipStream_t st,
+                         const EmbedOut* emb) {
+#define ARGMAX_LAUNCH(U_, E_)                                                                                                  \
+    hipLaunchKernelGGL((argmax_update_kernel<U_, E_>), dim3(bk.S), dim3(256), 0, st, cand_val, cand_idx, NT, bk.ids, bk.ld_ids, \
+                       bk.finished, bk.step, bk.done_len, bk.sync, bk.S, emb ? *emb : EmbedOut{})
+    if (sized && NT <= 256) { if (emb) ARGMAX_LAUNCH(1, true); else ARGMAX_LAUNCH(1, false); }
+    else { if (emb) ARGMAX_LAUNCH(ARGMAX_U_MAX, true); else ARGMAX_LAUNCH(ARGMAX_U_MAX, false); }
+#undef ARGMAX_LAUNCH
+    RGRG_LAUNCH_CHECK();
+    return RGRG_OK;
+}
+static int launch_argmax_update(rgrg_decoder* d, int NT, int S, hipStream_t st, const EmbedOut* emb = nullptr) {
+    return launch_argmax(d->cand_val, d->cand_idx, NT, StepBook{d->ids, d->max_len, d->finished, d->step, d->done_len, d->sync, S},
+                         (d->step_tail & 2) != 0, st, emb);
 }
 
 __global__ __launch_bounds__(256) void logits_candidates_kernel(const float* __restrict__ logits, int ld, int V, int NT,
@@ -1109,10 +1147,7 @@
     h.Xf = cur; h.part = d->part; h.Y = d->logits; h.ldy = d->ld_logits; h.act = RGRG_ACT_NONE;
     if ((rc = direct_linear(d, d->lm_head, h, DX_COMBINE4, S, count, !beam))) return rc;
     if (beam) return RGRG_OK;
-    hipLaunchKernelGGL(argmax_update_kernel, dim3(S), dim3(256), 0, st, d->cand_val, d->cand_idx, d->lm_head.NT, d->ids,
-                       d->max_len, d->finished, d->step, d->done_len, d->sync, S);
-    RGRG_LAUNCH_CHECK();
-    return RGRG_OK;
+    return launch_argmax_update(d, d->lm_head.NT, S, st);
 }
 
 static int range_bounds(int S, int want, int (&bounds)[MAX_CHAINS + 1]) {
@@ -1171,6 +1206,13 @@
 static bool step_qkv_cache(const rgrg_decoder* d, int S, bool plain) {
     const KvFormat f = kv_format(d, S);
     return d->qkv_cache && plain && step_ln_fold(d, S) && (f == KV_BF16 || f == KV_F16) && d->kp_gemms != 1 && d->kp_gemms != 3 && !d->key_mask_cur;
+}
+static bool step_embed_fused(const rgrg_decoder* d, int S, bool plain) {
+    return (d->step_tail & 4) && plain && !d->pos_override_cur && !d->key_mask_cur && d->x_emb && d->xn16_emb && d->stat_emb &&
+           lm_head_cand_path(d, S);
+}
+static EmbedOut step_embed_out(const rgrg_decoder* d, bool fold) {
+    return EmbedOut{d->wte, d->layers[0].ln1_g, d->layers[0].ln1_b, d->x_emb, nullptr, d->xn16_emb, fold ? d->stat_emb : nullptr, d->D, d->f16()};
 }
 static GemmLnFold cons_kv_cache(const rgrg_decoder* d, const GemmLnFold& cons, int l, int r0) {
     GemmLnFold f = cons;
@@ -1195,8 +1237,7 @@
     GemmLnFold prod{}, cons{};
     prod.Yb16 = xn16; prod.stats_out = d->ln_stat;
     cons.ln_stats = d->ln_stat; cons.ln_colsum = &cons_tag;
-    const GemmLnFold* pf = fold ? &prod : nullptr;
-    const GemmLnFold* cf = fold ? &cons : nullptr;
+    const bool ef = d->embed_fused_cur && step_embed_fused(d, S, !beam && !tok_override && !src);
     auto run_rows = [&](int r0, int rows) -> int {
         hipStream_t rs = d->stream;
         const size_t o = (size_t)r0 * D;
@@ -1209,22 +1250,30 @@
         prod_r.Yb16 = xn16r; prod_r.stats_out = statr; cons_r.ln_stats = statr;
         const GemmLnFold* pfr = fold ? &prod_r : nullptr;
         const GemmLnFold* cfr = fold ? &cons_r : nullptr;
-        hipLaunchKernelGGL(embed_ln_kernel, dim3(rows), dim3(256), 0, rs, d->wte, d->ids + (size_t)r0 * d->max_len, d->max_len, d->step,
-                           d->layers[0].ln1_g, d->layers[0].ln1_b, x, xn, D, tok_override ? tok_override + r0 : nullptr, xn16r, d->f16(),
-                           d->pos_override_cur ? d->pos_override_cur + r0 : nullptr, fold ? statr : (float*)nullptr);
-        RGRG_LAUNCH_CHECK();
         int rc2;
-        if ((rc2 = trace_mark(d, r0, 1000))) return rc2;
+        const float* x0 = ef ? d->x_emb + o : x;
+        const unsigned short* xn16_0 = ef ? d->xn16_emb + o : xn16r;
+        GemmLnFold cons_0 = cons_r;
+        if (ef) cons_0.ln_stats = d->stat_emb + (size_t)r0 * 32;
+        if (!ef) {
+            hipLaunchKernelGGL(embed_ln_kernel, dim3(rows), dim3(256), 0, rs, d->wte, d->ids + (size_t)r0 * d->max_len, d->max_len, d->step,
+                               d->layers[0].ln1_g, d->layers[0].ln1_b, x, xn, D, tok_override ? tok_override + r0 : nullptr, xn16r, d->f16(),
+                               d->pos_override_cur ? d->pos_override_cur + r0 : nullptr, fold ? statr : (float*)nullptr);
+            RGRG_LAUNCH_CHECK();
+            if ((rc2 = trace_mark(d, r0, 1000))) return rc2;
+        }
         for (int l = 0; l < d->n_layer; ++l) {
             const LayerW& w = d->layers[l];
             const float* ng = (l + 1 < d->n_layer) ? d->layers[l + 1].ln1_g : d->lnf_g;
             const float* nb = (l + 1 < d->n_layer) ? d->layers[l + 1].ln1_b : d->lnf_b;
-            const GemmLnFold cons_kv = qc ? cons_kv_cache(d, cons_r, l, r0) : cons_r;
-            if ((rc2 = linear(d, w.c_attn, xn, nullptr, d->qkv + 3 * o, rows, 3 * D, RGRG_ACT_NONE, count, xn16r, nullptr, qc ? &cons_kv : cfr))) return rc2;
+            const GemmLnFold& cons_l = l ? cons_r : cons_0;
+            const GemmLnFold cons_kv = qc ? cons_kv_cache(d, cons_l, l, r0) : cons_l;
+            if ((rc2 = linear(d, w.c_attn, xn, nullptr, d->qkv + 3 * o, rows, 3 * D, RGRG_ACT_NONE, count, l ? xn16r : xn16_0, nullptr,
+                              fold ? &cons_kv : nullptr))) return rc2;
             if ((rc2 = trace_mark(d, r0, l * 8 + 0))) return rc2;
             if ((rc2 = launch_attention(d, l, rows, src ? src + (size_t)r0 * d->T : nullptr, att16r, 0, r0, qc))) return rc2;
             if ((rc2 = trace_mark(d, r0, l * 8 + 1))) return rc2;
-            if ((rc2 = linear(d, w.attn_proj, d->att + o, x, x, rows, D, RGRG_ACT_NONE, count, att16r, nullptr, pfr))) return rc2;
+            if ((rc2 = linear(d, w.attn_proj, d->att + o, l ? x : x0, x, rows, D, RGRG_ACT_NONE, count, att16r, nullptr, pfr))) return rc2;
             if ((rc2 = trace_mark(d, r0, l * 8 + 2))) return rc2;
             if (!fold) {
                 if ((rc2 = launch_ln_rows(x, w.ln2_g, w.ln2_b, xn, D, xn16r, d->f16(), rows, rs))) return rc2;
@@ -1246,9 +1295,8 @@
         ce.cand_val = d->cand_val; ce.cand_idx = d->cand_idx;
         if ((rc = linear(d, d->lm_head, d->xn, nullptr, nullptr, S, d->ld_logits, RGRG_ACT_NONE, count, xn16, nullptr, &ce))) return rc;
         if ((rc = trace_mark(d, 0, 1002))) return rc;
-        hipLaunchKernelGGL(argmax_update_kernel, dim3(S), dim3(256), 0, st, d->cand_val, d->cand_idx, (d->lm_head.N + 255) / 256, d->ids,
-                           d->max_len, d->finished, d->step, d->done_len, d->sync, S);
-        RGRG_LAUNCH_CHECK();
+        const EmbedOut emb = step_embed_out(d, fold);
+        if ((rc = launch_argmax_update(d, (d->lm_head.N + 255) / 256, S, st, ef ? &emb : nullptr))) return rc;
         return trace_mark(d, 0, 1003);
     }
     if ((rc = linear(d, d->lm_head, d->xn, nullptr, d->logits, S, d->ld_logits, RGRG_ACT_NONE, count, xn16))) return rc;
@@ -1257,10 +1305,7 @@
     hipLaunchKernelGGL(logits_candidates_kernel, dim3(4, S), dim3(256), 0, st, d->logits, d->ld_logits, d->V,
                        cand_nt, d->cand_val, d->cand_idx);
     RGRG_LAUNCH_CHECK();
-    hipLaunchKernelGGL(argmax_update_kernel, dim3(S), dim3(256), 0, st, d->cand_val, d->cand_idx, cand_nt, d->ids,
-                       d->max_len, d->finished, d->step, d->done_len, d->sync, S);
-    RGRG_LAUNCH_CHECK();
-    return RGRG_OK;
+    return launch_argmax_update(d, cand_nt, S, st);
 }
 
 int enqueue_prefill(rgrg_decoder* d, const float* feats, int S, int row_mul) {
@@ -1324,6 +1369,7 @@
     if (const char* e = getenv("RGRG_GEMM_KP")) d->kp_gemms = atoi(e);
     if (const char* e = getenv("RGRG_W16_FUSED")) d->w16_fused = atoi(e) != 0;
     if (const char* e = getenv("RGRG_QKV_CACHE")) d->qkv_cache = atoi(e) != 0;
+    if (const char* e = getenv("RGRG_STEP_TAIL")) d->step_tail = atoi(e) & 7;
     if (const char* e = getenv("RGRG_DECODE_CHAINS")) {
         const int v = atoi(e);
         d->chains = (v >= -MAX_CHAINS && v <= MAX_CHAINS && v != 0 && v != -1) ? v : 1;
@@ -1455,6 +1501,12 @@
                     int use_graph, int64_t* out_ids, int out_ld, float* out_logprobs, int* out_len) {
     int rc = enqueue_prefill(d, feats, S);
     if (rc) return rc;
+    if (d->embed_fused_cur && step_embed_fused(d, S, true)) {
+        const EmbedOut e = step_embed_out(d, step_ln_fold(d, S));
+        hipLaunchKernelGGL(embed_ln_kernel, dim3(S), dim3(256), 0, d->stream, e.wte, d->ids, d->max_len, d->step, e.g, e.b, e.x, e.xn, e.D,
+                           (const int*)nullptr, e.xn16, e.f16, (const int*)nullptr, e.stats);
+        RGRG_LAUNCH_CHECK();
+    }
 
     hipGraphExec_t exec = nullptr;
     if (use_graph) {
@@ -1518,7 +1570,10 @@
     RGRG_CHECK_ARG(limit >= 2 && limit <= d->max_len && out_ld >= limit);
     int rc = decode_begin(d, stream);
     if (rc) return rc;
-    if ((rc = run_decode_loop(d, feats, S, limit, 0, greedy_step, use_graph, out_ids, out_ld, nullptr, out_len))) return rc;
+    d->embed_fused_cur = true;
+    rc = run_decode_loop(d, feats, S, limit, 0, greedy_step, use_graph, out_ids, out_ld, nullptr, out_len);
+    d->embed_fused_cur = false;
+    if (rc) return rc;
     d->logits_stale_rows = lm_head_cand_path(d, S) ? S : 0;
     return RGRG_OK;
 }
@@ -1668,6 +1723,31 @@
     a.step = step_dev; a.out = out; a.out16 = out16; a.S = S; a.H = H; a.T = T_slots; a.src = src; a.kmask = kmask;
     a.fmt = KV_E4M3; a.f16 = fp16 ? 1 : 0; a.max_wgs = max_workgroups; a.st = as_stream(stream);
     return launch_attn_decode(a);
+}
+
+extern "C" int rgrg_debug_argmax_update(const float* cand_val, const int* cand_idx, int NT, long long* ids, int ld_ids, int* finished,
+                                        int* step, int* done_len, int* sync, int S, int sized, const float* wte, const float* gain,
+                                        const float* bias, float* x, uint16_t* xn16, float* stats, int fp16, void* stream) {
+    RGRG_CHECK_ARG(cand_val && cand_idx && NT > 0 && ids && ld_ids >= 2 && finished && step && done_len && sync && S > 0 && S < 65536);
+    RGRG_CHECK_ARG(!wte || (x && xn16 && (stats || (gain && bias))));
+    const EmbedOut e{wte, gain, bias, x, nullptr, xn16, stats, 1024, fp16 ? 1 : 0};
+    return launch_argmax(cand_val, cand_idx, NT, StepBook{ids, ld_ids, finished, step, done_len, sync, S}, sized != 0, as_stream(stream),
+                         wte ? &e : nullptr);
+}
+
+extern "C" int rgrg_debug_decoder_step_state(rgrg_decoder* d, int S, float* x, uint16_t* xn16, float* stats, float* x_emb, uint16_t* xn16_emb,
+                                             float* stat_emb) {
+    RGRG_CHECK_ARG(d && S > 0 && S <= d->max_seqs);
+    RGRG_CHECK_ARG((!xn16 || d->xn16) && (!stats || d->ln_stat) && (!x_emb || d->x_emb) && (!xn16_emb || d->xn16_emb) && (!stat_emb || d->stat_emb));
+    RGRG_HIP(hipStreamSynchronize(d->stream));
+    const size_t n = (size_t)S * d->D;
+    if (x) RGRG_HIP(hipMemcpy(x, d->x, n * 4, hipMemcpyDeviceToDevice));
+    if (xn16) RGRG_HIP(hipMemcpy(xn16, d->xn16, n * 2, hipMemcpyDeviceToDevice));
+    if (stats) RGRG_HIP(hipMemcpy(stats, d->ln_stat, (size_t)S * 32 * 4, hipMemcpyDeviceToDevice));
+    if (x_emb) RGRG_HIP(hipMemcpy(x_emb, d->x_emb, n * 4, hipMemcpyDeviceToDevice));
+    if (xn16_emb) RGRG_HIP(hipMemcpy(xn16_emb, d->xn16_emb, n * 2, hipMemcpyDeviceToDevice));
+    if (stat_emb) RGRG_HIP(hipMemcpy(stat_emb, d->stat_emb, (size_t)S * 32 * 4, hipMemcpyDeviceToDevice));
+    return RGRG_OK;
 }
 
 extern "C" int rgrg_debug_ln_fold16(const float* w, const float* gain, const float* beta, const float* bias, uint16_t* wb,
@@ -1718,6 +1798,12 @@
             if ((rc2 = dmalloc(d, (void**)&d->xn16, (size_t)d->rows * d->D * 2, false)) ||
                 (rc2 = dmalloc(d, (void**)&d->att16, (size_t)d->rows * d->D * 2, false)) ||
                 (rc2 = dmalloc(d, (void**)&d->ff16, (size_t)d->rows * 4 * d->D * 2, false)))
+                return rc2;
+        }
+        if ((d->step_tail & 4) && !d->x_emb) {
+            if ((rc2 = dmalloc(d, (void**)&d->x_emb, (size_t)d->rows * d->D * 4, false)) ||
+                (rc2 = dmalloc(d, (void**)&d->xn16_emb, (size_t)d->rows * d->D * 2, false)) ||
+                (rc2 = dmalloc(d, (void**)&d->stat_emb, (size_t)d->rows * 32 * sizeof(float), true)))
                 return rc2;
         }
         if ((rc2 = mk(d->lm_head))) return rc2;
diff --git a/rgrg_amd/csrc/decoder_internal.h b/rgrg_amd/csrc/decoder_internal.h
--- a/rgrg_amd/csrc/decoder_internal.h
+++ b/rgrg_amd/csrc/decoder_internal.h
@@ -159,6 +159,10 @@
     std::vector<TraceMark>* trace = nullptr;
     bool w16_fused = true;
     bool qkv_cache = true;
+    int step_tail = 7;
+    bool embed_fused_cur = false;
+    float *x_emb = nullptr, *stat_emb = nullptr;
+    unsigned short* xn16_emb = nullptr;
     int kp_gemms = 2;
     int gemm_launches_per_step = 0;
     const int* pos_override_cur = nullptr;
diff --git a/rgrg_amd/csrc/gemm_bf16.hip b/rgrg_amd/csrc/gemm_bf16.hip
--- a/rgrg_amd/csrc/gemm_bf16.hip
+++ b/rgrg_amd/csrc/gemm_bf16.hip
@@ -34,6 +34,7 @@
     unsigned* sk_cnt = nullptr;
     float* cand_val = nullptr;
     int* cand_idx = nullptr;
+    int skip_empty = 0;
     int dbg = 0;
 };
 
@@ -698,7 +699,7 @@
     float esh[NI];
 #pragma unroll
     for (int ni = 0; ni < NI; ++ni) esh[ni] = p.shift ? p.shift[min(n0 + wq * 64 + ni * 32 + (lane & 31), p.N - 1)] : 0.f;
-    const int dbg = __builtin_amdgcn_readfirstlane(p.dbg);
+    const int dbg = __builtin_amdgcn_readfirstlane(p.dbg | ((p.skip_empty && m0 + g * 128 >= p.M) ? 5 : 0));
     if (dbg) {
 #pragma unroll
         for (int ks = 0; ks < 4; ++ks)
@@ -1048,6 +1049,8 @@
         p.gm = o < 0 ? 0 : o > 0 ? o : (mtiles > 8 ? 8 : 0);
     }
     { const char* e = getenv("RGRG_PP_DBG"); p.dbg = e ? atoi(e) : 0; }
+    static const bool skip = [] { const char* e = getenv("RGRG_STEP_TAIL"); return !e || (atoi(e) & 1) != 0; }();
+    p.skip_empty = skip ? 1 : 0;
     if (p.f16) hipLaunchKernelGGL(gemm_bf16_pp_kernel<true>, dim3(mtiles * ntiles), dim3(512), PP_LDS, st, p, mtiles, ntiles);
     else hipLaunchKernelGGL(gemm_bf16_pp_kernel<false>, dim3(mtiles * ntiles), dim3(512), PP_LDS, st, p, mtiles, ntiles);
     RGRG_LAUNCH_CHECK();
diff --git a/rgrg_amd/csrc/runtime.hip b/rgrg_amd/csrc/runtime.hip
--- a/rgrg_amd/csrc/runtime.hip
+++ b/rgrg_amd/csrc/runtime.hip
@@ -14,7 +14,7 @@
 }
 
 extern "C" const char* rgrg_last_error(void) { return rgrg::g_err; }
-extern "C" int rgrg_abi_version(void) { return 25; }
+extern "C" int rgrg_abi_version(void) { return 26; }
 extern "C" int rgrg_device_arch(int dev, char* buf, int buflen) {
     RGRG_CHECK_ARG(buf && buflen > 1);
     hipDeviceProp_t prop;
```
